# nikvaessen/w2v2-speaker

Measured on AMD Instinct MI355X. Metric: utterances/sec (w2v2-base + mean+std + AAM-softmax training step, 3 s clips), higher is better.
Workload: dtype f16; 1 GPU; wav2vec2-base + AAM-softmax(5994), mean+std pooling, 3 s synthetic audio, bs=66 per GPU, CNN frozen, fwd+bwd+all-reduce+Adam (BASELINE configs[1]); global_batch=66, samples_per_utt=48000, parallelism=dp1, regularisation=True

## Files before the change

### include/w2v2_hip.h

```cpp
#ifndef W2V2_HIP_H
#define W2V2_HIP_H

#include <stddef.h>
#include <stdint.h>

#ifdef __cplusplus
extern "C" {
#endif

#define W2V2_F32 0
#define W2V2_BF16 1
#define W2V2_F16 2

int w2v2_version(void);
const char* w2v2_last_error(void);

typedef struct {
  const void* ptr;
  int64_t ld;
  int64_t seg_len, seg_stride;
  int64_t stride0, stride1;
  int32_t trans;
  int32_t _pad;
} w2v2_operand;

enum {
  W2V2_EPI_NONE = 0,
  W2V2_EPI_BIAS = 1,
  W2V2_EPI_BIAS_GELU = 2,
  W2V2_EPI_GELU_BWD = 3,
  W2V2_EPI_ADD = 4,
  W2V2_EPI_SCALE_RC = 5,
  W2V2_EPI_BIAS_GELU_GRAD = 6,
  W2V2_EPI_MUL = 7
};

typedef struct {
  int32_t M, N, K;
  int32_t batch, batch_inner;
  int32_t dtype_ab;
  int32_t dtype_c;
  int32_t epilogue;
  w2v2_operand A, B;
  void* C;
  int64_t ldc, c_stride0, c_stride1;
  void* aux;
  int64_t ldaux, aux_stride0, aux_stride1;
  const float* bias;
  int64_t bias_stride1;
  const float* row_scale;
  const float* col_scale;
  float alpha;
  int32_t split_k;
  int32_t accumulate;
  int32_t _pad;
  int32_t k_ext, n_ext_from;
  int64_t b_lo_offset;
} w2v2_gemm_desc;

int w2v2_gemm(const w2v2_gemm_desc* d, void* stream);
int w2v2_gemm_timed(const w2v2_gemm_desc* d, void* stream, int slot);
int w2v2_timer_read(int first_slot, int n, float* ms_out);
int w2v2_gemm_kernel_of(const w2v2_gemm_desc* d);
int w2v2_tune_gemm_kernel(int family);
int w2v2_tune_gemm_debug(int bits);
int w2v2_tune_gemm_f32_tile(int tile);
int w2v2_tune_gemm_ring_debug(int bits);
int w2v2_gemm_f32_last_kernel(void);

typedef struct {
  const void* dY; int64_t ld_dy;
  const void* X;  int64_t ld_x;
  float* dW;      int64_t ld_dw;
  float* dbias;
  int32_t n_out, n_in;
} w2v2_wgrad_problem;
int w2v2_wgrad_grouped(const w2v2_wgrad_problem* problems, int n, int tokens, int tokens_padded,
                       int dtype , void* stream);
int w2v2_wgrad_kernel_of(const w2v2_wgrad_problem* problems, int n);
int w2v2_tune_wgrad_kernel(int family);

int w2v2_conv0_workspace_floats(int N, int C, int k, int stride);
int w2v2_conv0_stats(const float* wav, const float* w , float* partial, float* mean_rstd,
                     int B, int N, int C, int k, int stride, float eps, void* stream);
int w2v2_conv0_stats_mfma(const float* wav, const float* w, float* partial, float* mean_rstd,
                          int B, int N, int C, int k, int stride, float eps, void* stream);
int w2v2_conv0_stats_len(const float* wav, const float* w, float* partial, float* mean_rstd, const int* frames,
                         int B, int N, int C, int k, int stride, float eps, void* stream);
int w2v2_conv0_stats_mfma_len(const float* wav, const float* w, float* partial, float* mean_rstd, const int* frames,
                              int B, int N, int C, int k, int stride, float eps, void* stream);
int w2v2_conv0_apply(const float* wav, const float* w, const float* mean_rstd, const float* gamma,
                     const float* beta, void* y, int dtype, int B, int N, int C, int k, int stride,
                     void* stream);
int w2v2_conv0_layernorm_gelu(const float* wav, const float* w, const float* bias, const float* gamma, const float* beta,
                              void* out, int B, int N, int C, int k, int stride, float eps, int dtype, void* stream);
int w2v2_conv0_layernorm_gelu_bwd_workspace_floats(int B, int N, int C, int k, int stride);
int w2v2_conv0_layernorm_gelu_bwd(const float* wav, const float* w, const float* bias, const float* gamma, const float* beta,
                                  const void* dy, float* dw, float* dbias, float* dgamma, float* dbeta, float* workspace,
                                  int B, int N, int C, int k, int stride, float eps, int dtype, void* stream);
int w2v2_conv0_bwd(const float* wav, const float* w, const float* mean_rstd, const float* gamma,
                   const float* beta, const void* dz, float* sums, float* dw, float* dgamma, float* dbeta,
                   int dtype, int B, int N, int C, int k, int stride, void* stream);
int w2v2_col2im(const void* col, void* dx, int B, int Lin, int Lout, int Cin, int k, int stride, int dtype,
                void* stream);
int w2v2_unpack_conv_grad(const float* gp, float* g, int Cout, int Cin, int k, void* stream);
int w2v2_pack_conv_weight(const float* w, void* out, int dtype, int Cout, int Cin, int k, void* stream);

int w2v2_layernorm_fwd(const void* x, void* r_inout, const float* gamma, const float* beta, void* y,
                       float* mean, float* rstd, int M, int H, float eps, float drop_p,
                       uint64_t seed, int dtype, void* stream);
int w2v2_layernorm_gelu_fwd(const void* x, const float* gamma, const float* beta, void* y, int M, int H, float eps,
                            int dtype, void* stream);
int w2v2_layernorm_gelu_bwd_workspace_floats(int M, int H);
int w2v2_layernorm_gelu_bwd(const void* dy, const void* z, const float* gamma, const float* beta, void* dz, float* dgamma,
                            float* dbeta, float* dbias, float* workspace, int M, int H, float eps, int dtype, void* stream);
int w2v2_layernorm_bwd_workspace_floats(int H);
int w2v2_layernorm_bwd(const void* dy, const void* s, const float* mean, const float* rstd,
                       const float* gamma, void* ds, void* d_r, float* dgamma, float* dbeta,
                       float* workspace, int M, int H, float drop_p, uint64_t seed, int dtype,
                       void* stream);
typedef struct {
  const float* partial;
  float* dgamma;
  float* dbeta;
} w2v2_ln_fold;
int w2v2_layernorm_bwd_fold(const w2v2_ln_fold* entries, int n, int M, int H, void* stream);

int w2v2_dropout(const void* x, void* y, int64_t n, float p, uint64_t seed, int dtype, void* stream);
int w2v2_gelu_bwd(const void* dy, const void* pre, void* dx, int64_t n, int dtype, void* stream);
#define W2V2_PARTIAL_ROWS 256
int w2v2_gelu_bwd_colsum(const void* dy, const void* pre, void* dx, float* colsum, float* partial, int M, int N, int dtype,
                         void* stream);
int w2v2_add(const void* x, const void* a, void* y, int64_t n, int dtype, void* stream);
int w2v2_colsum(const void* x, int64_t ld, float* out, int M, int N, int dtype, void* stream);
int w2v2_zero_ranges(float* base, const int64_t* table, int n_ranges, int blocks_per_range, void* stream);
int w2v2_mean(const float* x, float* out, int n, void* stream);
int w2v2_cast(const float* x, void* y, int64_t n, int dtype, void* stream);
int w2v2_transpose_many(const void* src, void* dst, const int64_t* table, int n, int blocks_per_matrix,
                        int dtype, void* stream);
int w2v2_mask_fill(void* h, const uint8_t* mask, const float* embed, int M, int H, int dtype,
                   void* stream);
int w2v2_mask_feature(void* h, const uint8_t* mask, int B, int T, int H, int dtype, void* stream);
int w2v2_mask_fill_bwd(void* dh, const uint8_t* mask, float* d_embed, float* partial, int M, int H, int dtype,
                       void* stream);
int w2v2_prepend_token(const void* x, void* y, float c, int B, int T, int H, int dtype, void* stream);
int w2v2_pair_assemble(const void* feat, void* y, const int* left_row, const int* left_frames, const int* right_row,
                       const int* right_frames, float cls_c, float sep_c, int B, int T, int H, int dtype, void* stream);

int w2v2_posconv_regroup(const void* x, void* xg, int B, int T, int H, int G, int K, int pad_left,
                         int dtype, void* stream);
int w2v2_posconv_regroup_len(const void* x, void* xg, const int* lens, int B, int T, int H, int G, int K, int pad_left,
                             int dtype, void* stream);
int w2v2_posconv_wgrad(const void* dY, const void* xg, float* dwf, int B, int T, int H, int G, int K,
                       int dtype , void* stream);
int w2v2_posconv_direct(const void* xg, const void* w, void* out, void* aux, const float* bias, int B, int T, int G,
                        int Cg, int K, int64_t ldc, int mode, int dtype, void* stream);
int64_t w2v2_weightnorm_scratch_floats(int H, int G, int K);
int w2v2_weightnorm_pack(const float* g, const float* v, float* sumsq , void* wf,
                         void* wb, int H, int G, int K, int dtype, void* stream);
int w2v2_weightnorm_bwd(const float* g, const float* v, const float* sumsq, const float* dwf,
                        float* dot , float* dg, float* dv, int H, int G, int K,
                        void* stream);

int w2v2_softmax_fwd(const float* s, void* p, void* p_drop, int64_t rows, int T, int64_t ld,
                     float drop_p, uint64_t seed, int dtype, void* stream);
int w2v2_softmax_bwd(const float* dp_drop, const void* p, void* ds, int64_t rows, int T, int64_t ld,
                     float drop_p, uint64_t seed, int dtype, void* stream);
int w2v2_softmax_fwd_len(const float* s, void* p, const int* lens, int B, int heads, int T, int64_t ld, int dtype,
                         void* stream);
int w2v2_attention_fwd(const void* qkv, void* ctx, float* lse, int B, int T, int heads, int d,
                       float scale, float drop_p, uint64_t seed, int dtype, void* stream);
int w2v2_attention_bwd(const void* qkv, const void* ctx, const void* dctx, const float* lse,
                       void* dqkv, float* delta , int B, int T, int heads,
                       int d, float scale, float drop_p, uint64_t seed, int dtype, void* stream);
int w2v2_attention_fwd_len(const void* qkv, void* ctx, float* lse, const int* lens, int B, int T, int heads, int d,
                           float scale, int dtype, void* stream);

int w2v2_pool_fwd(const void* x, float* out, int B, int T, int H, int mode, int dtype, void* stream);
int w2v2_pool_fwd_len(const void* x, float* out, const int* lens, int B, int T, int H, int mode, int dtype,
                      void* stream);
int w2v2_pool_bwd(const void* x, const float* out, const float* dout, void* dx, int B, int T, int H,
                  int mode, int dtype, void* stream);

int w2v2_asp_context(const void* x, float* ctx, int B, int T, int C, int dtype, void* stream);
int w2v2_asp_context_len(const void* x, float* ctx, const int* lens, int B, int T, int C, int dtype, void* stream);
int w2v2_asp_context_bias(const float* ctx, const float* w1 , const float* b1, float* cb ,
                          int B, int A, int C, void* stream);
int w2v2_asp_bn_workspace_floats(int M, int A);
int w2v2_asp_bn_stats(const void* a_pre, float* workspace, float* mean_rstd, float* running, int M, int A,
                      float eps, float momentum, int dtype, void* stream);
int w2v2_asp_bn_eval_stats(const float* running, float* mean_rstd, int A, float eps, void* stream);
int w2v2_asp_bn_tanh(const void* a_pre, const float* mean_rstd, const float* gamma, const float* beta, void* h,
                     int M, int A, int dtype, void* stream);
int w2v2_asp_bn_bwd(const void* dh, const void* a_pre, const float* mean_rstd, const float* gamma,
                    const float* beta, float* workspace, float* dgamma, float* dbeta, void* da, int M, int A,
                    int dtype, void* stream);
int w2v2_asp_pool_fwd(const void* x, const void* s, float* out, float* stats, int B, int T, int C, int dtype,
                      void* stream);
int w2v2_asp_pool_fwd_len(const void* x, const void* s, float* out, float* stats, const int* lens, int B, int T, int C,
                          int dtype, void* stream);
int w2v2_asp_pool_bwd(const void* x, const void* s, const float* out, const float* stats, const float* dout,
                      void* ds, void* dx, int B, int T, int C, int dtype, void* stream);
int w2v2_asp_context_bwd(const void* x, const float* ctx, const void* da, const float* w1, float* dw1, void* dx,
                         float* scratch, int B, int T, int C, int A, int dtype, void* stream);

int w2v2_bce_head_fwd_bwd(const float* emb, const float* w, const float* b, const int64_t* label, float* prob,
                          float* loss_rows, float* dlogit, float* demb, float* dw, float* db, int B, int H,
                          const float* loss_scale, void* stream);

int w2v2_bn_workspace_floats(int M, int C);
int w2v2_bn_fwd(const void* a, int64_t lda, float* workspace, float* mean_rstd, float* running, const float* gamma,
                const float* beta, void* y, int64_t ldy, int M, int C, float eps, float momentum, int relu, int train,
                int dtype, void* stream);
int w2v2_bn_colsum_rows(int M, int C);
int w2v2_bn_bwd(const void* dy, int64_t lddy, const void* a, int64_t lda, const float* mean_rstd, const float* gamma,
                float* workspace, float* dgamma, float* dbeta, void* da, int64_t ldda, int M, int C, int relu,
                float* colsum_partial, int dtype, void* stream);
int w2v2_bn_bwd_sum(const void* dy, int64_t lddy, const void* dy2, int64_t lddy2, const void* a, int64_t lda,
                    const float* mean_rstd, const float* gamma, float* workspace, float* dgamma, float* dbeta, void* da,
                    int64_t ldda, int M, int C, int relu, float* colsum_partial, int dtype, void* stream);
int w2v2_im2col_reflect(const void* x, int64_t ldx, void* col, int B, int T, int Cin, int k, int dilation, int dtype,
                        void* stream);
int w2v2_im2col_reflect_sum(const void* x, int64_t ldx, const void* x2, int64_t ldx2, void* col, int B, int T, int Cin,
                            int k, int dilation, int dtype, void* stream);
int w2v2_im2col_reflect_len(const void* x, int64_t ldx, void* col, const int* lens, int B, int T, int Cin, int k,
                            int dilation, int dtype, void* stream);
int w2v2_im2col_reflect_sum_len(const void* x, int64_t ldx, const void* x2, int64_t ldx2, void* col, const int* lens,
                                int B, int T, int Cin, int k, int dilation, int dtype, void* stream);
int w2v2_col2im_reflect(const void* dcol, void* dx, int64_t lddx, int B, int T, int Cin, int k, int dilation,
                        int accumulate, int dtype, void* stream);
int w2v2_add_strided(const void* a, int64_t lda, const void* b, int64_t ldb, void* y, int64_t ldy, int M, int C,
                     int dtype, void* stream);
int w2v2_se_scale(const void* x, const float* g, void* y, int B, int T, int C, int dtype, void* stream);
int w2v2_se_bwd_gate(const void* dout, const void* x, float* dg, int B, int T, int C, int dtype, void* stream);
int w2v2_se_bwd_x(const void* dout, const float* g, const float* ds, void* dx, int B, int T, int C, int dtype,
                  void* stream);
int w2v2_act_fwd(const float* x, float* y, int64_t n, int mode, void* stream);
int w2v2_act_bwd(const float* dy, const float* y, float* dx, int64_t n, int mode, void* stream);

#define W2V2_FBANK_TILE_FRAMES 16
int w2v2_fbank_db(const float* wav, const int* lens, const float* window, const float* fbank, float* db_out,
                  float* partial_max, int B, int N, int T, int n_mels, void* stream);
int w2v2_fbank_normalize(const float* db, const float* partial_max, const int* lens, void* out, int64_t ldo, int dtype,
                         int B, int T, int n_mels, void* stream);

int w2v2_skinny_linear_fwd(const float* x, const float* W, const float* bias, float* y, int B, int N, int K, int act,
                           void* stream);
int w2v2_skinny_linear_bwd_x(const float* dy, const float* y, const float* W, float* dx, int B, int N, int K, int act,
                             void* stream);
int w2v2_skinny_linear_bwd_w(const float* dy, const float* y, const float* x, float* dW, float* dbias, int B, int N,
                             int K, int act, int accumulate, void* stream);

int w2v2_row_invnorm(const void* x, int64_t ld, float* inv, int rows, int cols, int dtype,
                     void* stream);
int w2v2_aam_softmax_fwd_bwd(const float* cos, const int64_t* label, float* softmax,
                             float* loss_rows, void* dcos_w, void* dcos_x, const float* inv_x,
                             const float* inv_w, float* rowdot, float* colprod, int B, int C,
                             int64_t ldc, float margin, float scale, const float* loss_scale,
                             float* correct_rows, int easy_margin , int dtype, void* stream);
int w2v2_normalize_bwd(const float* g, const void* x, int64_t ldx, const float* inv,
                       const float* dot, float* dx, int rows, int cols, int x_dtype, int add,
                       void* stream);
int w2v2_aam_dw(const void* dcos_x, int64_t ldc, const void* emb, const float* colprod, const float* W,
                const float* inv_w, float* dW, int B, int C, int E, int dtype, void* stream);

int w2v2_adam_step(float* p, const float* g, float* m, float* v, void* pb, int pb_dtype, int64_t n, float lr,
                   float beta1, float beta2, float eps, float bias_corr1, float bias_corr2,
                   float grad_scale, const float* scaler_state, int step, int skip_slot, void* stream);

#define W2V2_OPTIM_ADAM 0
#define W2V2_OPTIM_SGD 1
int w2v2_optim_step(int algo, float* p, const float* g, float* m, float* v, void* pb, int pb_dtype, int64_t n, float lr,
                    float beta1, float beta2, float eps, float bias_corr1, float bias_corr2, float grad_scale,
                    float weight_decay, float momentum, float dampening, int nesterov, const float* norm_state,
                    const float* scaler_state, int step, int skip_slot, void* stream);

int w2v2_grad_norm_partials(int64_t n);
int w2v2_grad_norm(const float* g, int64_t n, float grad_scale, float* scaler_state, float max_norm, double* partials,
                   int n_partials, float* norm_state, void* stream);

int w2v2_grad_accumulate(float* acc, const float* g, int64_t n, int first, void* stream);

int w2v2_weight_residual(const float* p, void* lo, const int64_t* table, int n_ranges, int dtype, void* stream);
int w2v2_grad_scaler_check(const float* g, int64_t n, float* state, void* stream);
int w2v2_grad_scaler_update(float* state, float growth, float backoff, int growth_interval, int skipped_ranges,
                            void* stream);

typedef struct w2v2_comm w2v2_comm;
int w2v2_comm_unique_id(void* id_host_128);
int w2v2_comm_init(w2v2_comm** comm, const void* id_host_128, int rank, int world, int device);
int w2v2_comm_init_loopback(w2v2_comm** comm, int world, int device);
int w2v2_allreduce_async(w2v2_comm* comm, float* buf, int64_t n, void* stream);
int w2v2_broadcast_async(w2v2_comm* comm, void* buf, int64_t nbytes, int root, void* stream);
int w2v2_comm_destroy(w2v2_comm* comm);
int w2v2_traffic_probe(float* buf, int64_t n, int channels, int lds_bytes, float gbps, void* stream);

#ifdef __cplusplus
}
#endif
#endif
```

### w2v2_speaker_amd/_lib.py

```python
from __future__ import annotations

import ctypes as C
import os

from . import _build

F32, BF16, F16 = 0, 1, 2
EPI_NONE, EPI_BIAS, EPI_BIAS_GELU, EPI_GELU_BWD, EPI_ADD, EPI_SCALE_RC, EPI_BIAS_GELU_GRAD, EPI_MUL = range(8)
OPTIM_ADAM, OPTIM_SGD = 0, 1

c_i32, c_i64, c_u64, c_f32, c_vp = C.c_int32, C.c_int64, C.c_uint64, C.c_float, C.c_void_p


class Operand(C.Structure):
    _fields_ = [("ptr", c_vp), ("ld", c_i64), ("seg_len", c_i64), ("seg_stride", c_i64),
                ("stride0", c_i64), ("stride1", c_i64), ("trans", c_i32), ("_pad", c_i32)]


class GemmDesc(C.Structure):
    _fields_ = [("M", c_i32), ("N", c_i32), ("K", c_i32), ("batch", c_i32), ("batch_inner", c_i32),
                ("dtype_ab", c_i32), ("dtype_c", c_i32), ("epilogue", c_i32),
                ("A", Operand), ("B", Operand),
                ("C", c_vp), ("ldc", c_i64), ("c_stride0", c_i64), ("c_stride1", c_i64),
                ("aux", c_vp), ("ldaux", c_i64), ("aux_stride0", c_i64), ("aux_stride1", c_i64),
                ("bias", c_vp), ("bias_stride1", c_i64), ("row_scale", c_vp), ("col_scale", c_vp),
                ("alpha", c_f32), ("split_k", c_i32), ("accumulate", c_i32), ("_pad", c_i32),
                ("k_ext", c_i32), ("n_ext_from", c_i32), ("b_lo_offset", c_i64)]


class LnFold(C.Structure):
    _fields_ = [("partial", c_vp), ("dgamma", c_vp), ("dbeta", c_vp)]


class WgradProblem(C.Structure):
    _fields_ = [("dY", c_vp), ("ld_dy", c_i64), ("X", c_vp), ("ld_x", c_i64), ("dW", c_vp), ("ld_dw", c_i64),
                ("dbias", c_vp), ("n_out", c_i32), ("n_in", c_i32)]


_SIGS = {
    "w2v2_version": (c_i32, []),
    "w2v2_last_error": (C.c_char_p, []),
    "w2v2_gemm": (c_i32, [C.POINTER(GemmDesc), c_vp]),
    "w2v2_gemm_kernel_of": (c_i32, [c_vp]),
    "w2v2_gemm_timed": (c_i32, [C.POINTER(GemmDesc), c_vp, c_i32]),
    "w2v2_timer_read": (c_i32, [c_i32, c_i32, c_vp]),
    "w2v2_tune_gemm_kernel": (c_i32, [c_i32]),
    "w2v2_tune_gemm_debug": (c_i32, [c_i32]),
    "w2v2_tune_gemm_f32_tile": (c_i32, [c_i32]),
    "w2v2_tune_gemm_ring_debug": (c_i32, [c_i32]),
    "w2v2_gemm_f32_last_kernel": (c_i32, []),
    "w2v2_zero_ranges": (c_i32, [c_vp, c_vp, c_i32, c_i32, c_vp]),
    "w2v2_mean": (c_i32, [c_vp, c_vp, c_i32, c_vp]),
    "w2v2_wgrad_grouped": (c_i32, [C.POINTER(WgradProblem), c_i32, c_i32, c_i32, c_i32, c_vp]),
    "w2v2_wgrad_kernel_of": (c_i32, [C.POINTER(WgradProblem), c_i32]),
    "w2v2_tune_wgrad_kernel": (c_i32, [c_i32]),
    "w2v2_conv0_workspace_floats": (c_i32, [c_i32, c_i32, c_i32, c_i32]),
    "w2v2_conv0_stats": (c_i32, [c_vp, c_vp, c_vp, c_vp, c_i32, c_i32, c_i32, c_i32, c_i32, c_f32, c_vp]),
    "w2v2_conv0_stats_mfma": (c_i32, [c_vp, c_vp, c_vp, c_vp, c_i32, c_i32, c_i32, c_i32, c_i32, c_f32, c_vp]),
    "w2v2_conv0_stats_len": (c_i32, [c_vp, c_vp, c_vp, c_vp, c_vp, c_i32, c_i32, c_i32, c_i32, c_i32, c_f32, c_vp]),
    "w2v2_conv0_stats_mfma_len": (c_i32, [c_vp, c_vp, c_vp, c_vp, c_vp, c_i32, c_i32, c_i32, c_i32, c_i32, c_f32,
                                          c_vp]),
    "w2v2_conv0_apply": (c_i32, [c_vp, c_vp, c_vp, c_vp, c_vp, c_vp, c_i32, c_i32, c_i32, c_i32, c_i32,
                                 c_i32, c_vp]),
    "w2v2_pack_conv_weight": (c_i32, [c_vp, c_vp, c_i32, c_i32, c_i32, c_i32, c_vp]),
    "w2v2_conv0_bwd": (c_i32, [c_vp] * 10 + [c_i32] * 6 + [c_vp]),
    "w2v2_col2im": (c_i32, [c_vp, c_vp, c_i32, c_i32, c_i32, c_i32, c_i32, c_i32, c_i32, c_vp]),
    "w2v2_unpack_conv_grad": (c_i32, [c_vp, c_vp, c_i32, c_i32, c_i32, c_vp]),
    "w2v2_conv0_layernorm_gelu": (c_i32, [c_vp, c_vp, c_vp, c_vp, c_vp, c_vp, c_i32, c_i32, c_i32, c_i32, c_i32, c_f32, c_i32, c_vp]),
    "w2v2_layernorm_gelu_fwd": (c_i32, [c_vp, c_vp, c_vp, c_vp, c_i32, c_i32, c_f32, c_i32, c_vp]),
    "w2v2_layernorm_gelu_bwd_workspace_floats": (c_i32, [c_i32, c_i32]),
    "w2v2_layernorm_gelu_bwd": (c_i32, [c_vp] * 9 + [c_i32, c_i32, c_f32, c_i32, c_vp]),
    "w2v2_conv0_layernorm_gelu_bwd_workspace_floats": (c_i32, [c_i32] * 5),
    "w2v2_conv0_layernorm_gelu_bwd": (c_i32, [c_vp] * 11 + [c_i32] * 5 + [c_f32, c_i32, c_vp]),
    "w2v2_layernorm_fwd": (c_i32, [c_vp, c_vp, c_vp, c_vp, c_vp, c_vp, c_vp, c_i32, c_i32, c_f32, c_f32,
                                   c_u64, c_i32, c_vp]),
    "w2v2_layernorm_bwd_workspace_floats": (c_i32, [c_i32]),
    "w2v2_layernorm_bwd": (c_i32, [c_vp, c_vp, c_vp, c_vp, c_vp, c_vp, c_vp, c_vp, c_vp, c_vp, c_i32, c_i32,
                                   c_f32, c_u64, c_i32, c_vp]),
    "w2v2_layernorm_bwd_fold": (c_i32, [C.POINTER(LnFold), c_i32, c_i32, c_i32, c_vp]),
    "w2v2_dropout": (c_i32, [c_vp, c_vp, c_i64, c_f32, c_u64, c_i32, c_vp]),
    "w2v2_gelu_bwd_colsum": (c_i32, [c_vp, c_vp, c_vp, c_vp, c_vp, c_i32, c_i32, c_i32, c_vp]),
    "w2v2_gelu_bwd": (c_i32, [c_vp, c_vp, c_vp, c_i64, c_i32, c_vp]),
    "w2v2_add": (c_i32, [c_vp, c_vp, c_vp, c_i64, c_i32, c_vp]),
    "w2v2_colsum": (c_i32, [c_vp, c_i64, c_vp, c_i32, c_i32, c_i32, c_vp]),
    "w2v2_cast": (c_i32, [c_vp, c_vp, c_i64, c_i32, c_vp]),
    "w2v2_transpose_many": (c_i32, [c_vp, c_vp, c_vp, c_i32, c_i32, c_i32, c_vp]),
    "w2v2_mask_feature": (c_i32, [c_vp, c_vp, c_i32, c_i32, c_i32, c_i32, c_vp]),
    "w2v2_mask_fill": (c_i32, [c_vp, c_vp, c_vp, c_i32, c_i32, c_i32, c_vp]),
    "w2v2_mask_fill_bwd": (c_i32, [c_vp, c_vp, c_vp, c_vp, c_i32, c_i32, c_i32, c_vp]),
    "w2v2_prepend_token": (c_i32, [c_vp, c_vp, c_f32, c_i32, c_i32, c_i32, c_i32, c_vp]),
    "w2v2_pair_assemble": (c_i32, [c_vp, c_vp, c_vp, c_vp, c_vp, c_vp, c_f32, c_f32, c_i32, c_i32, c_i32, c_i32, c_vp]),
    "w2v2_posconv_regroup": (c_i32, [c_vp, c_vp, c_i32, c_i32, c_i32, c_i32, c_i32, c_i32, c_i32, c_vp]),
    "w2v2_posconv_regroup_len": (c_i32, [c_vp, c_vp, c_vp, c_i32, c_i32, c_i32, c_i32, c_i32, c_i32, c_i32, c_vp]),
    "w2v2_posconv_direct": (c_i32, [c_vp, c_vp, c_vp, c_vp, c_vp, c_i32, c_i32, c_i32, c_i32, c_i32, c_i64, c_i32, c_i32, c_vp]),
    "w2v2_posconv_wgrad": (c_i32, [c_vp, c_vp, c_vp, c_i32, c_i32, c_i32, c_i32, c_i32, c_i32, c_vp]),
    "w2v2_weightnorm_scratch_floats": (c_i64, [c_i32, c_i32, c_i32]),
    "w2v2_weightnorm_pack": (c_i32, [c_vp, c_vp, c_vp, c_vp, c_vp, c_i32, c_i32, c_i32, c_i32, c_vp]),
    "w2v2_weightnorm_bwd": (c_i32, [c_vp, c_vp, c_vp, c_vp, c_vp, c_vp, c_vp, c_i32, c_i32, c_i32, c_vp]),
    "w2v2_softmax_fwd": (c_i32, [c_vp, c_vp, c_vp, c_i64, c_i32, c_i64, c_f32, c_u64, c_i32, c_vp]),
    "w2v2_softmax_bwd": (c_i32, [c_vp, c_vp, c_vp, c_i64, c_i32, c_i64, c_f32, c_u64, c_i32, c_vp]),
    "w2v2_softmax_fwd_len": (c_i32, [c_vp, c_vp, c_vp, c_i32, c_i32, c_i32, c_i64, c_i32, c_vp]),
    "w2v2_attention_fwd": (c_i32, [c_vp, c_vp, c_vp, c_i32, c_i32, c_i32, c_i32, c_f32, c_f32, c_u64,
                                   c_i32, c_vp]),
    "w2v2_attention_fwd_len": (c_i32, [c_vp, c_vp, c_vp, c_vp, c_i32, c_i32, c_i32, c_i32, c_f32, c_i32, c_vp]),
    "w2v2_attention_bwd": (c_i32, [c_vp, c_vp, c_vp, c_vp, c_vp, c_vp, c_i32, c_i32, c_i32, c_i32, c_f32,
                                   c_f32, c_u64, c_i32, c_vp]),
    "w2v2_pool_fwd": (c_i32, [c_vp, c_vp, c_i32, c_i32, c_i32, c_i32, c_i32, c_vp]),
    "w2v2_pool_fwd_len": (c_i32, [c_vp, c_vp, c_vp, c_i32, c_i32, c_i32, c_i32, c_i32, c_vp]),
    "w2v2_pool_bwd": (c_i32, [c_vp, c_vp, c_vp, c_vp, c_i32, c_i32, c_i32, c_i32, c_i32, c_vp]),
    "w2v2_bce_head_fwd_bwd": (c_i32, [c_vp] * 10 + [c_i32, c_i32, c_vp, c_vp]),
    "w2v2_bn_workspace_floats": (c_i32, [c_i32, c_i32]),
    "w2v2_bn_fwd": (c_i32, [c_vp, c_i64, c_vp, c_vp, c_vp, c_vp, c_vp, c_vp, c_i64, c_i32, c_i32, c_f32, c_f32, c_i32,
                            c_i32, c_i32, c_vp]),
    "w2v2_skinny_linear_fwd": (c_i32, [c_vp, c_vp, c_vp, c_vp, c_i32, c_i32, c_i32, c_i32, c_vp]),
    "w2v2_skinny_linear_bwd_x": (c_i32, [c_vp, c_vp, c_vp, c_vp, c_i32, c_i32, c_i32, c_i32, c_vp]),
    "w2v2_skinny_linear_bwd_w": (c_i32, [c_vp, c_vp, c_vp, c_vp, c_vp, c_i32, c_i32, c_i32, c_i32, c_i32, c_vp]),
    "w2v2_bn_bwd": (c_i32, [c_vp, c_i64, c_vp, c_i64, c_vp, c_vp, c_vp, c_vp, c_vp, c_vp, c_i64, c_i32, c_i32, c_i32,
                            c_vp, c_i32, c_vp]),
    "w2v2_bn_bwd_sum": (c_i32, [c_vp, c_i64, c_vp, c_i64, c_vp, c_i64, c_vp, c_vp, c_vp, c_vp, c_vp, c_vp, c_i64, c_i32,
                                c_i32, c_i32, c_vp, c_i32, c_vp]),
    "w2v2_bn_colsum_rows": (c_i32, [c_i32, c_i32]),
    "w2v2_im2col_reflect": (c_i32, [c_vp, c_i64, c_vp, c_i32, c_i32, c_i32, c_i32, c_i32, c_i32, c_vp]),
    "w2v2_im2col_reflect_sum": (c_i32, [c_vp, c_i64, c_vp, c_i64, c_vp, c_i32, c_i32, c_i32, c_i32, c_i32, c_i32, c_vp]),
    "w2v2_im2col_reflect_len": (c_i32, [c_vp, c_i64, c_vp, c_vp, c_i32, c_i32, c_i32, c_i32, c_i32, c_i32, c_vp]),
    "w2v2_im2col_reflect_sum_len": (c_i32, [c_vp, c_i64, c_vp, c_i64, c_vp, c_vp, c_i32, c_i32, c_i32, c_i32, c_i32, c_i32,
                                            c_vp]),
    "w2v2_col2im_reflect": (c_i32, [c_vp, c_vp, c_i64, c_i32, c_i32, c_i32, c_i32, c_i32, c_i32, c_i32, c_vp]),
    "w2v2_add_strided": (c_i32, [c_vp, c_i64, c_vp, c_i64, c_vp, c_i64, c_i32, c_i32, c_i32, c_vp]),
    "w2v2_se_scale": (c_i32, [c_vp, c_vp, c_vp, c_i32, c_i32, c_i32, c_i32, c_vp]),
    "w2v2_se_bwd_gate": (c_i32, [c_vp, c_vp, c_vp, c_i32, c_i32, c_i32, c_i32, c_vp]),
    "w2v2_se_bwd_x": (c_i32, [c_vp, c_vp, c_vp, c_vp, c_i32, c_i32, c_i32, c_i32, c_vp]),
    "w2v2_act_fwd": (c_i32, [c_vp, c_vp, c_i64, c_i32, c_vp]),
    "w2v2_act_bwd": (c_i32, [c_vp, c_vp, c_vp, c_i64, c_i32, c_vp]),
    "w2v2_fbank_db": (c_i32, [c_vp, c_vp, c_vp, c_vp, c_vp, c_vp, c_i32, c_i32, c_i32, c_i32, c_vp]),
    "w2v2_fbank_normalize": (c_i32, [c_vp, c_vp, c_vp, c_vp, c_i64, c_i32, c_i32, c_i32, c_i32, c_vp]),
    "w2v2_asp_context": (c_i32, [c_vp, c_vp, c_i32, c_i32, c_i32, c_i32, c_vp]),
    "w2v2_asp_context_len": (c_i32, [c_vp, c_vp, c_vp, c_i32, c_i32, c_i32, c_i32, c_vp]),
    "w2v2_asp_context_bias": (c_i32, [c_vp, c_vp, c_vp, c_vp, c_i32, c_i32, c_i32, c_vp]),
    "w2v2_asp_bn_workspace_floats": (c_i32, [c_i32, c_i32]),
    "w2v2_asp_bn_stats": (c_i32, [c_vp, c_vp, c_vp, c_vp, c_i32, c_i32, c_f32, c_f32, c_i32, c_vp]),
    "w2v2_asp_bn_eval_stats": (c_i32, [c_vp, c_vp, c_i32, c_f32, c_vp]),
    "w2v2_asp_bn_tanh": (c_i32, [c_vp, c_vp, c_vp, c_vp, c_vp, c_i32, c_i32, c_i32, c_vp]),
    "w2v2_asp_bn_bwd": (c_i32, [c_vp] * 9 + [c_i32, c_i32, c_i32, c_vp]),
    "w2v2_asp_pool_fwd": (c_i32, [c_vp, c_vp, c_vp, c_vp, c_i32, c_i32, c_i32, c_i32, c_vp]),
    "w2v2_asp_pool_fwd_len": (c_i32, [c_vp, c_vp, c_vp, c_vp, c_vp, c_i32, c_i32, c_i32, c_i32, c_vp]),
    "w2v2_asp_pool_bwd": (c_i32, [c_vp] * 7 + [c_i32, c_i32, c_i32, c_i32, c_vp]),
    "w2v2_asp_context_bwd": (c_i32, [c_vp] * 7 + [c_i32, c_i32, c_i32, c_i32, c_i32, c_vp]),
    "w2v2_row_invnorm": (c_i32, [c_vp, c_i64, c_vp, c_i32, c_i32, c_i32, c_vp]),
    "w2v2_aam_softmax_fwd_bwd": (c_i32, [c_vp, c_vp, c_vp, c_vp, c_vp, c_vp, c_vp, c_vp, c_vp, c_vp, c_i32,
                                         c_i32, c_i64, c_f32, c_f32, c_vp, c_vp, c_i32, c_i32, c_vp]),
    "w2v2_aam_dw": (c_i32, [c_vp, c_i64, c_vp, c_vp, c_vp, c_vp, c_vp, c_i32, c_i32, c_i32, c_i32, c_vp]),
    "w2v2_normalize_bwd": (c_i32, [c_vp, c_vp, c_i64, c_vp, c_vp, c_vp, c_i32, c_i32, c_i32, c_i32, c_vp]),
    "w2v2_adam_step": (c_i32, [c_vp, c_vp, c_vp, c_vp, c_vp, c_i32, c_i64, c_f32, c_f32, c_f32, c_f32, c_f32,
                               c_f32, c_f32, c_vp, c_i32, c_i32, c_vp]),
    "w2v2_optim_step": (c_i32, [c_i32, c_vp, c_vp, c_vp, c_vp, c_vp, c_i32, c_i64, c_f32, c_f32, c_f32, c_f32, c_f32,
                                c_f32, c_f32, c_f32, c_f32, c_f32, c_i32, c_vp, c_vp, c_i32, c_i32, c_vp]),
    "w2v2_grad_norm_partials": (c_i32, [c_i64]),
    "w2v2_grad_norm": (c_i32, [c_vp, c_i64, c_f32, c_vp, c_f32, c_vp, c_i32, c_vp, c_vp]),
    "w2v2_grad_accumulate": (c_i32, [c_vp, c_vp, c_i64, c_i32, c_vp]),
    "w2v2_weight_residual": (c_i32, [c_vp, c_vp, c_vp, c_i32, c_i32, c_vp]),
    "w2v2_comm_unique_id": (c_i32, [c_vp]),
    "w2v2_comm_init": (c_i32, [C.POINTER(c_vp), c_vp, c_i32, c_i32, c_i32]),
    "w2v2_comm_init_loopback": (c_i32, [C.POINTER(c_vp), c_i32, c_i32]),
    "w2v2_allreduce_async": (c_i32, [c_vp, c_vp, c_i64, c_vp]),
    "w2v2_broadcast_async": (c_i32, [c_vp, c_vp, c_i64, c_i32, c_vp]),
    "w2v2_comm_destroy": (c_i32, [c_vp]),
    "w2v2_traffic_probe": (c_i32, [c_vp, c_i64, c_i32, c_i32, c_f32, c_vp]),
    "w2v2_grad_scaler_check": (c_i32, [c_vp, c_i64, c_vp, c_vp]),
    "w2v2_grad_scaler_update": (c_i32, [c_vp, c_f32, c_f32, c_i32, c_i32, c_vp]),
}

EXPORTS = tuple(_SIGS)
_lib = None


def library_path() -> str:
    return _build.LIB


def load():
    global _lib
    if _lib is not None:
        return _lib
    path = _build.LIB
    alt = os.environ.get("W2V2_LIB_AB")
    if alt and os.path.exists(alt):
        path = alt
    elif _build.needs_build():
        try:
            _build.build_locked()
        except Exception as e:
            raise RuntimeError(f"libw2v2hip.so is missing or older than its sources and could not be built: {e}") from e
    lib = C.CDLL(path)
    for name, (res, args) in _SIGS.items():
        if path == alt and not hasattr(lib, name):
            continue
        fn = getattr(lib, name)
        fn.restype, fn.argtypes = res, args
    _lib = lib
    return lib


def check(rc: int, what: str = "") -> None:
    if rc != 0:
        msg = load().w2v2_last_error()
        raise RuntimeError(f"libw2v2hip {what} failed: {msg.decode() if msg else rc}")
```

### w2v2_speaker_amd/csrc/gemm.hip

```cpp
#include "gemm_common.h"

template <int R, bool TRANS>
struct Stager {
  static constexpr int NV = TRANS ? 4 : (R / 32);
  uint4 v[NV];

  __device__ __forceinline__ void load(const OpDev& o, const bf16_t* __restrict__ base, int r0,
                                       int rbound, int k0, int kend, int tid,
                                       const int64_t* __restrict__ rowoff) {
    if constexpr (!TRANS) {
#pragma unroll
      for (int j = 0; j < NV; ++j) {
        const int c = tid + 256 * j;
        const int row = c >> 3, kc = c & 7;
        const int k = k0 + kc * 8;
        uint4 val = make_uint4(0, 0, 0, 0);
        if (r0 + row < rbound && k < kend) {
          const bf16_t* p = base + rowoff[j] + k;
          if (o.vec_ok && k + 8 <= kend) {
            val = *reinterpret_cast<const uint4*>(p);
          } else {
            bf16_t t[8];
#pragma unroll
            for (int e = 0; e < 8; ++e) t[e] = (k + e < kend) ? p[e] : (bf16_t)0;
            val.x = t[0] | ((uint32_t)t[1] << 16); val.y = t[2] | ((uint32_t)t[3] << 16);
            val.z = t[4] | ((uint32_t)t[5] << 16); val.w = t[6] | ((uint32_t)t[7] << 16);
          }
        }
        v[j] = val;
      }
    } else {
      const int nblk = R * 2;
      const int mb = tid % (R / 8), kb = tid / (R / 8);
#pragma unroll
      for (int i = 0; i < 4; ++i) {
        uint4 val = make_uint4(0, 0, 0, 0);
        const int k = k0 + kb * 4 + i;
        const int in0 = r0 + mb * 8;
        if (tid < nblk && k < kend && in0 < rbound) {
          const bf16_t* p = base + outer_off(o, k) + in0;
          if (o.vec_ok && in0 + 8 <= rbound) {
            val = *reinterpret_cast<const uint4*>(p);
          } else {
            bf16_t t[8];
#pragma unroll
            for (int e = 0; e < 8; ++e) t[e] = (in0 + e < rbound) ? p[e] : (bf16_t)0;
            val.x = t[0] | ((uint32_t)t[1] << 16); val.y = t[2] | ((uint32_t)t[3] << 16);
            val.z = t[4] | ((uint32_t)t[5] << 16); val.w = t[6] | ((uint32_t)t[7] << 16);
          }
        }
        v[i] = val;
      }
    }
  }

  __device__ __forceinline__ void store(bf16_t* __restrict__ lds, int tid) const {
    if constexpr (!TRANS) {
#pragma unroll
      for (int j = 0; j < NV; ++j) {
        const int c = tid + 256 * j;
        const int row = c >> 3, kc = c & 7;
        *reinterpret_cast<uint4*>(lds + row * 64 + ((kc ^ swz_rs(row)) << 3)) = v[j];
      }
    } else {
      const int nblk = R * 2;
      if (tid >= nblk) return;
      const int mb = tid % (R / 8), kb = tid / (R / 8);
      const uint32_t w[4][4] = {{v[0].x, v[0].y, v[0].z, v[0].w},
                                {v[1].x, v[1].y, v[1].z, v[1].w},
                                {v[2].x, v[2].y, v[2].z, v[2].w},
                                {v[3].x, v[3].y, v[3].z, v[3].w}};
#pragma unroll
      for (int mi = 0; mi < 8; ++mi) {
        const int d = mi >> 1;
        uint2 o2;
        if (mi & 1) {
          o2.x = (w[0][d] >> 16) | (w[1][d] & 0xffff0000u);
          o2.y = (w[2][d] >> 16) | (w[3][d] & 0xffff0000u);
        } else {
          o2.x = (w[0][d] & 0xffffu) | (w[1][d] << 16);
          o2.y = (w[2][d] & 0xffffu) | (w[3][d] << 16);
        }
        const int row = mb * 8 + mi;
        const int chunk = kb >> 1, half = kb & 1;
        *reinterpret_cast<uint2*>(lds + row * 64 + ((chunk ^ swz_rs(row)) << 3) + half * 4) = o2;
      }
    }
  }
};

template <typename TE, int FM, int FN, bool TA, bool TB, typename TC>
__global__ __launch_bounds__(256) void gemm16_regstage_kernel(const GemmArgs g) {
  constexpr int BM = 32 * FM, BN = 32 * FN;
  extern __shared__ __attribute__((aligned(16))) char smem_raw[];
  bf16_t* As = reinterpret_cast<bf16_t*>(smem_raw);
  bf16_t* Bs = As + 2 * BM * 64;

  const int tid = threadIdx.x;
  const int lane = tid & 63, wave = tid >> 6;
  const int wm = wave >> 1, wn = wave & 1;

  const int ntile = g.tiles_m * g.tiles_n;
  const int tile = xcd_remap(blockIdx.x, ntile);
  const int tm = tile / g.tiles_n, tn = tile - tm * g.tiles_n;
  const int m0 = tm * BM, n0 = tn * BN;
  const int z = blockIdx.z;
  const int z0 = z / g.batch_inner, z1 = z - z0 * g.batch_inner;
  const int split = blockIdx.y;
  const int kbeg = split * g.k_per_split;
  const int kend = min(g.K, kbeg + g.k_per_split);

  const bf16_t* Ab = reinterpret_cast<const bf16_t*>(g.A.ptr) + z0 * g.a_s0 + z1 * g.a_s1;
  const bf16_t* Bb = reinterpret_cast<const bf16_t*>(g.B.ptr) + z0 * g.b_s0 + z1 * g.b_s1;

  int64_t arow[TA ? 1 : (BM / 32)], brow[TB ? 1 : (BN / 32)];
  if constexpr (!TA) {
#pragma unroll
    for (int j = 0; j < BM / 32; ++j) {
      const int row = (tid + 256 * j) >> 3;
      arow[j] = (m0 + row < g.M) ? outer_off(g.A, m0 + row) : 0;
    }
  }
  if constexpr (!TB) {
#pragma unroll
    for (int j = 0; j < BN / 32; ++j) {
      const int row = (tid + 256 * j) >> 3;
      brow[j] = (n0 + row < g.N) ? outer_off(g.B, n0 + row) : 0;
    }
  }

  f32x4 acc[FM][FN];
#pragma unroll
  for (int i = 0; i < FM; ++i)
#pragma unroll
    for (int j = 0; j < FN; ++j) acc[i][j] = f32x4{0.f, 0.f, 0.f, 0.f};

  Stager<BM, TA> sa;
  Stager<BN, TB> sb;
  const int nk = (kend - kbeg + 63) / 64;
  if (nk > 0) {
    sa.load(g.A, Ab, m0, g.M, kbeg, kend, tid, arow);
    sb.load(g.B, Bb, n0, g.N, kbeg, kend, tid, brow);
    sa.store(As, tid);
    sb.store(Bs, tid);
  }
  __syncthreads();

  const int frow = lane & 15, fk = lane >> 4;
  for (int kt = 0; kt < nk; ++kt) {
    const int cur = kt & 1;
    if (kt + 1 < nk) {
      const int k0 = kbeg + (kt + 1) * 64;
      sa.load(g.A, Ab, m0, g.M, k0, kend, tid, arow);
      sb.load(g.B, Bb, n0, g.N, k0, kend, tid, brow);
    }
    const bf16_t* Ac = As + cur * BM * 64;
    const bf16_t* Bc = Bs + cur * BN * 64;
#pragma unroll
    for (int kk = 0; kk < 2; ++kk) {
      frag8_t af[FM], bfr[FN];
#pragma unroll
      for (int i = 0; i < FM; ++i) {
        const int row = wm * (16 * FM) + i * 16 + frow;
        af[i] = *reinterpret_cast<const frag8_t*>(Ac + row * 64 + (((kk * 4 + fk) ^ swz_rs(row)) << 3));
      }
#pragma unroll
      for (int j = 0; j < FN; ++j) {
        const int row = wn * (16 * FN) + j * 16 + frow;
        bfr[j] = *reinterpret_cast<const frag8_t*>(Bc + row * 64 + (((kk * 4 + fk) ^ swz_rs(row)) << 3));
      }
#pragma unroll
      for (int i = 0; i < FM; ++i)
#pragma unroll
        for (int j = 0; j < FN; ++j)
          acc[i][j] = mfma16<TE>(bfr[j], af[i], acc[i][j]);
    }
    if (kt + 1 < nk) {
      sa.store(As + (cur ^ 1) * BM * 64, tid);
      sb.store(Bs + (cur ^ 1) * BN * 64, tid);
    }
    __syncthreads();
  }

  tile_epilogue<TC, FM, FN>(g, acc, reinterpret_cast<float*>(smem_raw), m0, n0, wm, wn, z0, z1, split);
}


template <typename TE, int FM, int FN, typename TC>
__global__ __launch_bounds__(256) void gemm16_dma_128_kernel(const GemmArgs g) {
  constexpr int BM = 32 * FM, BN = 32 * FN;
  constexpr int NA = BM / 32, NB = BN / 32;
  extern __shared__ __attribute__((aligned(16))) char smem_raw[];
  bf16_t* As = reinterpret_cast<bf16_t*>(smem_raw);
  bf16_t* Bs = As + 2 * BM * 64;

  const int tid = threadIdx.x;
  const int lane = tid & 63;
  const int wave = __builtin_amdgcn_readfirstlane(tid >> 6);
  const int wm = wave >> 1, wn = wave & 1;

  const int ntile = g.tiles_m * g.tiles_n;
  const int tile = xcd_remap(blockIdx.x, ntile);
  const int tm = tile / g.tiles_n, tn = tile - tm * g.tiles_n;
  const int m0 = tm * BM, n0 = tn * BN;
  const int z = blockIdx.z;
  const int z0 = z / g.batch_inner, z1 = z - z0 * g.batch_inner;
  const int split = blockIdx.y;
  const int kbeg = split * g.k_per_split;
  const int kend = min(g.K, kbeg + g.k_per_split);
  const int nk = (kend - kbeg) >> 6;

  const bf16_t* Ab = reinterpret_cast<const bf16_t*>(g.A.ptr) + z0 * g.a_s0 + z1 * g.a_s1;
  const bf16_t* Bb = reinterpret_cast<const bf16_t*>(g.B.ptr) + z0 * g.b_s0 + z1 * g.b_s1;

  const int c8 = lane & 7, r8 = lane >> 3;
  const bf16_t* ap[NA];
  const bf16_t* bp[NB];
#pragma unroll
  for (int j = 0; j < NA; ++j) {
    const int row = (wave * NA + j) * 8 + r8;
    const int grow = min(m0 + row, g.M - 1);
    ap[j] = Ab + outer_off(g.A, grow) + kbeg + ((c8 ^ swz(row)) << 3);
  }
#pragma unroll
  for (int j = 0; j < NB; ++j) {
    const int row = (wave * NB + j) * 8 + r8;
    const int grow = min(n0 + row, g.N - 1);
    bp[j] = Bb + outer_off(g.B, grow) + kbeg + ((c8 ^ swz(row)) << 3);
  }

  f32x4 acc[FM][FN];
#pragma unroll
  for (int i = 0; i < FM; ++i)
#pragma unroll
    for (int j = 0; j < FN; ++j) acc[i][j] = f32x4{0.f, 0.f, 0.f, 0.f};

  auto stage = [&](int buf, int kt) {
    bf16_t* ad = As + buf * BM * 64 + wave * NA * 8 * 64;
    bf16_t* bd = Bs + buf * BN * 64 + wave * NB * 8 * 64;
#pragma unroll
    for (int j = 0; j < NA; ++j) w2v2_dma16(ap[j] + kt * 64, ad + j * 8 * 64);
#pragma unroll
    for (int j = 0; j < NB; ++j) w2v2_dma16(bp[j] + kt * 64, bd + j * 8 * 64);
  };
  auto landed = [&]() {
    asm volatile("s_waitcnt vmcnt(0)" ::: "memory");
    __syncthreads();
  };
  const int frow = lane & 15, fk = lane >> 4;
  auto compute = [&](int buf) {
    const bf16_t* Ac = As + buf * BM * 64;
    const bf16_t* Bc = Bs + buf * BN * 64;
#pragma unroll
    for (int kk = 0; kk < 2; ++kk) {
      frag8_t af[FM], bfr[FN];
#pragma unroll
      for (int i = 0; i < FM; ++i) {
        const int row = wm * (16 * FM) + i * 16 + frow;
        af[i] = *reinterpret_cast<const frag8_t*>(Ac + row * 64 + (((kk * 4 + fk) ^ swz(row)) << 3));
      }
#pragma unroll
      for (int j = 0; j < FN; ++j) {
        const int row = wn * (16 * FN) + j * 16 + frow;
        bfr[j] = *reinterpret_cast<const frag8_t*>(Bc + row * 64 + (((kk * 4 + fk) ^ swz(row)) << 3));
      }
#pragma unroll
      for (int i = 0; i < FM; ++i)
#pragma unroll
        for (int j = 0; j < FN; ++j)
          acc[i][j] = mfma16<TE>(bfr[j], af[i], acc[i][j]);
    }
  };

  if (nk > 0) stage(0, 0);
  w2v2_vmcnt0_visible();
  __syncthreads();
  for (int kt = 0; kt < nk; kt += 2) {
    if (kt + 1 < nk) stage(1, kt + 1);
    compute(0);
    landed();
    if (kt + 1 < nk) {
      if (kt + 2 < nk) stage(0, kt + 2);
      compute(1);
      landed();
    }
  }

  tile_epilogue<TC, FM, FN>(g, acc, reinterpret_cast<float*>(smem_raw), m0, n0, wm, wn, z0, z1, split);
}

const W2v2Switches& w2v2_switches() {
  static const W2v2Switches sw = [] {
    W2v2Switches s;
    auto env_int = [](const char* name, int dflt) { const char* e = getenv(name); return e ? atoi(e) : dflt; };
    auto env_on = [](const char* name, bool dflt) { const char* e = getenv(name); return e ? e[0] != '0' : dflt; };
    s.no_glds = getenv("W2V2_NO_GLDS") != nullptr;
    s.glds3 = getenv("W2V2_NO_GLDS3") == nullptr;
    s.tile256 = getenv("W2V2_NO_GEMM_PH") == nullptr;
    s.persistent = getenv("W2V2_G3_NONPERSISTENT") == nullptr;
    s.g3n = env_int("W2V2_G3N", 512);
    s.defer = getenv("W2V2_NO_DEFER") == nullptr;
    s.wt_stores = env_on("W2V2_EPI_WT", true);
    s.late_dma = env_on("W2V2_PH_LATE", false);
    s.reserve_cus = env_int("W2V2_RESERVE_CUS", 0);
    s.f32_no_dma = env_on("W2V2_F32_NO_DMA", false);
    s.wgrad_ring = getenv("W2V2_WGRAD_V1") == nullptr;
    s.wgrad_ring4 = getenv("W2V2_NO_WGRAD4") == nullptr;
    s.wgrad_phased = getenv("W2V2_NO_WGRAD_PH") == nullptr;
    return s;
  }();
  return sw;
}

int w2v2_device_cus() {
  static const int ncu = [] {
    int dev = 0, v = 0;
    (void)hipGetDevice(&dev);
    return (hipDeviceGetAttribute(&v, hipDeviceAttributeMultiprocessorCount, dev) == hipSuccess && v > 0) ? v : 256;
  }();
  return ncu;
}
int w2v2_gemm_device_cus() {
  const int ncu = w2v2_device_cus(), r = w2v2_switches().reserve_cus;
  return (r > 0 && r < ncu) ? ncu - r : ncu;
}

static int g_w2v2_force = 0;
extern "C" int w2v2_tune_gemm_kernel(int family) {
  const int old = g_w2v2_force;
  if (family == 0 || family == 1 || family == 2 || family == 4) g_w2v2_force = family;
  return old;
}

struct GemmRoute {
  int family;
  bool narrow;
  dim3 grid;
  int f32_rows;
};

static bool aligned16(const void* p) { return (reinterpret_cast<uintptr_t>(p) & 15) == 0; }

static int gemm_route(const w2v2_gemm_desc* d, int force, GemmArgs& a, GemmRoute& r) {
  W2V2_REQUIRE(d != nullptr, "w2v2_gemm: null descriptor");
  W2V2_REQUIRE(d->M > 0 && d->N > 0 && d->K >= 0 && d->batch > 0, "w2v2_gemm: bad shape M=%d N=%d K=%d batch=%d",
               d->M, d->N, d->K, d->batch);
  W2V2_REQUIRE(d->A.ptr && d->B.ptr && d->C, "w2v2_gemm: null operand");
  W2V2_REQUIRE(d->dtype_ab == W2V2_F32 || d->dtype_ab == W2V2_BF16 || d->dtype_ab == W2V2_F16,
               "w2v2_gemm: bad dtype_ab %d", d->dtype_ab);
  W2V2_REQUIRE(d->dtype_c == W2V2_F32 || d->dtype_c == d->dtype_ab, "w2v2_gemm: dtype_c %d must be f32 or dtype_ab (%d)",
               d->dtype_c, d->dtype_ab);
  W2V2_REQUIRE(d->epilogue >= 0 && d->epilogue <= W2V2_EPI_MUL, "w2v2_gemm: bad epilogue %d", d->epilogue);
  const int split = d->split_k > 1 ? d->split_k : 1;
  const int atomic = (split > 1 || d->accumulate) ? 1 : 0;
  if (atomic) {
    W2V2_REQUIRE(d->dtype_c == W2V2_F32, "w2v2_gemm: split_k/accumulate need an f32 C");
    W2V2_REQUIRE(d->epilogue == W2V2_EPI_NONE || (split == 1) || d->epilogue == W2V2_EPI_BIAS,
                 "w2v2_gemm: split_k supports EPI_NONE/EPI_BIAS only");
  }
  if (d->epilogue == W2V2_EPI_BIAS || d->epilogue == W2V2_EPI_BIAS_GELU || d->epilogue == W2V2_EPI_BIAS_GELU_GRAD)
    W2V2_REQUIRE(d->bias != nullptr, "w2v2_gemm: bias epilogue without bias");
  if (d->epilogue == W2V2_EPI_GELU_BWD || d->epilogue == W2V2_EPI_ADD || d->epilogue == W2V2_EPI_MUL ||
      d->epilogue == W2V2_EPI_BIAS_GELU_GRAD)
    W2V2_REQUIRE(d->aux != nullptr, "w2v2_gemm: epilogue %d needs aux", d->epilogue);
  if (d->epilogue == W2V2_EPI_SCALE_RC)
    W2V2_REQUIRE(d->row_scale && d->col_scale, "w2v2_gemm: EPI_SCALE_RC needs row/col scales");

  const bool f32 = d->dtype_ab == W2V2_F32;
  const int oal = f32 ? 4 : 8;
  a.M = d->M; a.N = d->N; a.K = d->K;
  a.epilogue = d->epilogue; a.split_k = split; a.atomic = atomic;
  a.tiles_m = a.tiles_n = 0;
  a.batch_inner = d->batch_inner > 0 ? d->batch_inner : 1;
  auto cvt = [&](const w2v2_operand& o) {
    OpDev v;
    v.ptr = o.ptr; v.ld = o.ld; v.seg_len = o.seg_len; v.seg_stride = o.seg_stride; v.trans = o.trans ? 1 : 0;
    v.vec_ok = aligned16(o.ptr) && (o.ld % oal == 0) && (o.seg_stride % oal == 0) && (o.stride0 % oal == 0) &&
               (o.stride1 % oal == 0);
    return v;
  };
  a.A = cvt(d->A);
  a.B = cvt(d->B);
  a.a_s0 = d->A.stride0; a.a_s1 = d->A.stride1; a.b_s0 = d->B.stride0; a.b_s1 = d->B.stride1;
  a.C = d->C; a.ldc = d->ldc; a.c_s0 = d->c_stride0; a.c_s1 = d->c_stride1;
  a.aux = d->aux; a.ldaux = d->ldaux; a.aux_s0 = d->aux_stride0; a.aux_s1 = d->aux_stride1;
  a.bias = d->bias; a.bias_s1 = d->bias_stride1;
  a.row_scale = d->row_scale; a.col_scale = d->col_scale;
  a.alpha = d->alpha;
  a.k_ext = d->k_ext; a.n_ext_from = d->n_ext_from; a.b_lo_off = d->b_lo_offset;
  a.defer_ok = 0;
  a.wt_stores = 1;
  a.late_dma = 0;
  a.xcd_tiles = 0;
  a.dbg_bits = 0;
  const int cal = d->dtype_c == W2V2_F32 ? 4 : 8;
  a.c_vec_ok = aligned16(d->C) && (d->ldc % cal == 0) && (d->c_stride0 % cal == 0) && (d->c_stride1 % cal == 0);
  a.aux_vec_ok = d->aux && aligned16(d->aux) && (d->ldaux % cal == 0) && (d->aux_stride0 % cal == 0) &&
                 (d->aux_stride1 % cal == 0);
  r.family = 0; r.narrow = false; r.grid = dim3(1); r.f32_rows = 0;

  const int bk = f32 ? 32 : 64;
  a.k_per_split = (int)(cdiv(cdiv(d->K, split), bk) * bk);
  if (a.k_per_split == 0) a.k_per_split = bk;
  if (f32) {
    r.f32_rows = w2v2_gemm_f32_dma_rows(a, d->M, d->N, d->K, split, d->batch);
    r.family = r.f32_rows > 0 ? 10 : 9;
    return 0;
  }

  const W2v2Switches& sw = w2v2_switches();
  const int64_t ncu = w2v2_gemm_device_cus();
  const bool glds = !a.A.trans && !a.B.trans && a.A.vec_ok && a.B.vec_ok && (d->K % 64 == 0) && d->K >= 64 && !sw.no_glds;
  r.narrow = d->N <= 64 || (glds && cdiv(d->M, 128) * cdiv(d->N, 128) * split * d->batch * 2 <= ncu);
  a.tiles_m = (int)cdiv(d->M, 128); a.tiles_n = (int)cdiv(d->N, r.narrow ? 64 : 128);
  r.grid = dim3(a.tiles_m * a.tiles_n, split, d->batch);

  const bool ring_ok = glds && split == 1 && !atomic;
  auto extent = [](const w2v2_operand& o, int64_t rows, int64_t K) -> int64_t {
    return (o.seg_len > 0 ? (rows / o.seg_len + 1) * o.seg_stride + o.seg_len * o.ld : rows * o.ld) + K;
  };
  const bool fits32 = extent(d->A, d->M, d->K) < (int64_t(1) << 31) && extent(d->B, d->N, d->K) < (int64_t(1) << 31);
  const bool phased_ok = ring_ok && d->k_ext == 0 && d->batch == 1 && fits32 && (d->dtype_c == W2V2_F32 || lines_ok(a));
  bool ring, phased;
  if (force != 0 && ring_ok && d->k_ext == 0 && d->batch == 1) {
    ring = force >= 2;
    phased = force == 4 && phased_ok;
  } else {
    ring = ring_ok && (d->k_ext != 0 || (d->N >= sw.g3n && d->M >= 1024 && sw.glds3));
    phased = false;
    if (ring && phased_ok && d->N >= 512 && sw.tile256) {
      const int64_t t4 = cdiv(d->M, 256) * cdiv(d->N, 256), t3 = cdiv(d->M, 256) * cdiv(d->N, 128);
      const double fill4 = (double)t4 / (double)(cdiv(t4, ncu) * ncu), fill3 = (double)t3 / (double)(cdiv(t3, ncu) * ncu);
      phased = fill4 * 1.25 >= fill3 && t4 * 2 >= ncu && (double)d->N / (double)(cdiv(d->N, 256) * 256) >= 0.9;
    }
  }
  if (d->k_ext != 0)
    W2V2_REQUIRE(ring && d->k_ext == d->K && d->n_ext_from >= 0 && d->n_ext_from % 128 == 0 && d->b_lo_offset % 8 == 0,
                 "w2v2_gemm: two-term weights (k_ext) need k_ext == K, n_ext_from %% 128 == 0 and K-contiguous 16-byte "
                 "aligned operands with K %% 64 == 0 (M=%d N=%d K=%d)", d->M, d->N, d->K);
  r.family = phased ? 4 : ring ? 2 : glds ? 1 : 3;
  a.wt_stores = sw.wt_stores;
  a.late_dma = sw.late_dma;
  if (r.family == 2)
    a.defer_ok = sw.defer && d->dtype_c != W2V2_F32 && lines_ok(a) && (d->N % 128 == 0) &&
                 d->epilogue != W2V2_EPI_BIAS_GELU && d->epilogue != W2V2_EPI_BIAS_GELU_GRAD;
  return 0;
}

extern "C" int w2v2_gemm_kernel_of(const w2v2_gemm_desc* d) {
  GemmArgs a;
  GemmRoute r;
  return gemm_route(d, g_w2v2_force, a, r) != 0 ? -1 : r.family;
}

template <typename TE, int FM, int FN, typename TC>
static int launch_glds(const GemmArgs& a, dim3 grid, hipStream_t st) {
  constexpr size_t lds = (size_t)2 * (32 * FM + 32 * FN) * 64 * sizeof(bf16_t);
  return w2v2_launch_lds<&gemm16_dma_128_kernel<TE, FM, FN, TC>>("gemm16_dma_128_kernel", grid, dim3(256), lds, st, a);
}

template <typename TE, int FM, int FN, typename TC>
static int launch_regstage(const GemmArgs& a, dim3 grid, hipStream_t st) {
  constexpr size_t lds = (size_t)2 * (32 * FM + 32 * FN) * 64 * sizeof(bf16_t);
#define W2V2_LAUNCH(TA_, TB_) \
  return w2v2_launch_lds<&gemm16_regstage_kernel<TE, FM, FN, TA_, TB_, TC>>("gemm16_regstage_kernel", grid, dim3(256), lds, st, a)
  if (!a.A.trans && !a.B.trans) W2V2_LAUNCH(false, false);
  else if (!a.A.trans && a.B.trans) W2V2_LAUNCH(false, true);
  else if (a.A.trans && !a.B.trans) W2V2_LAUNCH(true, false);
  else W2V2_LAUNCH(true, true);
#undef W2V2_LAUNCH
}

template <typename TE, typename TC>
static int launch_128(const GemmArgs& a, const GemmRoute& r, hipStream_t st) {
  if (r.family == 1) return r.narrow ? launch_glds<TE, 4, 2, TC>(a, r.grid, st) : launch_glds<TE, 4, 4, TC>(a, r.grid, st);
  return r.narrow ? launch_regstage<TE, 4, 2, TC>(a, r.grid, st) : launch_regstage<TE, 4, 4, TC>(a, r.grid, st);
}

extern "C" int w2v2_gemm(const w2v2_gemm_desc* d, void* stream) {
  GemmArgs a;
  GemmRoute r;
  if (gemm_route(d, g_w2v2_force, a, r) != 0) return -1;
  hipStream_t st = as_stream(stream);
  const bool c32 = d->dtype_c == W2V2_F32;
  int rc;
  switch (r.family) {
    case 4: rc = w2v2_launch_phased_256x256(a, d->dtype_ab, d->dtype_c, d->M, d->N, d->batch, st); break;
    case 2: rc = w2v2_launch_ring_256x128(a, d->dtype_ab, d->dtype_c, d->M, d->N, d->batch, w2v2_switches().persistent, st); break;
    case 9: case 10: rc = w2v2_launch_gemm_f32(a, d->M, d->N, d->K, a.split_k, d->batch, r.f32_rows, st); break;
    default:
      if (d->dtype_ab == W2V2_BF16) rc = c32 ? launch_128<bf16_t, float>(a, r, st) : launch_128<bf16_t, bf16_t>(a, r, st);
      else rc = c32 ? launch_128<f16_t, float>(a, r, st) : launch_128<f16_t, f16_t>(a, r, st);
      break;
  }
  if (rc != 0) return rc;
  W2V2_CHECK_LAUNCH("w2v2_gemm");
  return 0;
}

#include <vector>
W2v2PendingTimer& w2v2_pending_timer() {
  static thread_local W2v2PendingTimer t = {nullptr, nullptr, false};
  return t;
}
static std::vector<std::pair<hipEvent_t, hipEvent_t>> g_timer_slots;
extern "C" int w2v2_gemm_timed(const w2v2_gemm_desc* d, void* stream, int slot) {
  W2V2_REQUIRE(slot >= 0 && slot < (1 << 16), "w2v2_gemm_timed: slot %d out of range", slot);
  while ((int)g_timer_slots.size() <= slot) {
    hipEvent_t a, b;
    if (hipEventCreate(&a) != hipSuccess || hipEventCreate(&b) != hipSuccess) W2V2_FAIL("w2v2_gemm_timed: hipEventCreate failed");
    g_timer_slots.push_back({a, b});
  }
  W2v2PendingTimer& pt = w2v2_pending_timer();
  pt.start = g_timer_slots[slot].first;
  pt.stop = g_timer_slots[slot].second;
  pt.armed = true;
  const int rc = w2v2_gemm(d, stream);
  const bool unused = pt.armed;
  pt.armed = false;
  if (rc != 0) return rc;
  if (unused)
    W2V2_FAIL("w2v2_gemm_timed: this product does not run on the 256x128 ring or the phased 256x256 kernel");
  return 0;
}
extern "C" int w2v2_timer_read(int first_slot, int n, float* ms_out) {
  W2V2_REQUIRE(first_slot >= 0 && n >= 0 && first_slot + n <= (int)g_timer_slots.size() && ms_out, "w2v2_timer_read: bad range");
  for (int i = 0; i < n; ++i) {
    auto& e = g_timer_slots[first_slot + i];
    if (hipEventSynchronize(e.second) != hipSuccess || hipEventElapsedTime(ms_out + i, e.first, e.second) != hipSuccess)
      W2V2_FAIL("w2v2_timer_read: slot %d was never launched", first_slot + i);
  }
  return 0;
}
```

### w2v2_speaker_amd/csrc/gemm_common.h

```cpp
#pragma once
#include "common.h"
#include <hip/hip_ext.h>
#include <type_traits>
#include <stdlib.h>

typedef __attribute__((ext_vector_type(4))) float f32x4;

struct OpDev {
  const void* ptr;
  int64_t ld, seg_len, seg_stride;
  int trans;
  int vec_ok;
};

struct GemmArgs {
  int M, N, K;
  int epilogue, split_k, atomic;
  int tiles_m, tiles_n;
  int k_per_split;
  OpDev A, B;
  int64_t a_s0, a_s1, b_s0, b_s1;
  int batch_inner;
  void* C;
  int64_t ldc, c_s0, c_s1;
  void* aux;
  int64_t ldaux, aux_s0, aux_s1;
  const float* bias;
  int64_t bias_s1;
  const float* row_scale;
  const float* col_scale;
  float alpha;
  int c_vec_ok;
  int aux_vec_ok;
  int defer_ok;
  int wt_stores;
  int late_dma;
  int k_ext, n_ext_from;
  int64_t b_lo_off;
  int xcd_tiles;
  int dbg_bits;
};

__device__ __forceinline__ int64_t outer_off(const OpDev& o, int64_t idx) {
  if (o.seg_len > 0) {
    const int64_t q = idx / o.seg_len;
    return q * o.seg_stride + (idx - q * o.seg_len) * o.ld;
  }
  return idx * o.ld;
}

__device__ __forceinline__ int swz(int row) { return ((row ^ (row >> 1)) & 3) | (row & 4); }
__device__ __forceinline__ int swz_b(int row) { return swz((((row >> 4) & 3) << 2) | (row & 3)); }
__device__ __forceinline__ int swz_rs(int row) { return (row & 7) ^ ((row >> 3) & 1); }

template <typename TC>
__device__ __forceinline__ void epilogue_store4(const GemmArgs& g, TC* __restrict__ C,
                                                const TC* __restrict__ aux_in, TC* __restrict__ aux_out,
                                                const float* __restrict__ bias, int m, int n0,
                                                const float acc[4], bool lead) {
  if (m >= g.M) return;
  const float rs = (g.epilogue == W2V2_EPI_SCALE_RC) ? g.row_scale[m] : 1.0f;
  float out[4];
  float pre[4];
#pragma unroll
  for (int j = 0; j < 4; ++j) {
    const int n = n0 + j;
    float v = acc[j] * g.alpha;
    pre[j] = 0.f;
    if (n < g.N) {
      switch (g.epilogue) {
        case W2V2_EPI_BIAS:
          if (lead) v += bias[n];
          break;
        case W2V2_EPI_BIAS_GELU:
          v += bias[n];
          pre[j] = v;
          v = gelu_f(v);
          break;
        case W2V2_EPI_BIAS_GELU_GRAD:
          v += bias[n];
          gelu_both_f(v, v, pre[j]);
          break;
        case W2V2_EPI_GELU_BWD:
          v *= gelu_grad_f(to_f32<TC>(aux_in[(int64_t)m * g.ldaux + n]));
          break;
        case W2V2_EPI_MUL:
          v *= to_f32<TC>(aux_in[(int64_t)m * g.ldaux + n]);
          break;
        case W2V2_EPI_ADD:
          v += to_f32<TC>(aux_in[(int64_t)m * g.ldaux + n]);
          break;
        case W2V2_EPI_SCALE_RC:
          v *= rs * g.col_scale[n];
          break;
        default:
          break;
      }
    }
    out[j] = v;
  }
  TC* crow = C + (int64_t)m * g.ldc;
  if (g.atomic) {
    if constexpr (sizeof(TC) == 4) {
#pragma unroll
      for (int j = 0; j < 4; ++j)
        if (n0 + j < g.N) unsafeAtomicAdd(reinterpret_cast<float*>(crow) + n0 + j, out[j]);
    }
    return;
  }
  if (g.c_vec_ok && n0 + 4 <= g.N) {
    if constexpr (sizeof(TC) == 4) {
      *reinterpret_cast<float4*>(crow + n0) = make_float4(out[0], out[1], out[2], out[3]);
    } else {
      uint2 w;
      w.x = pack2<TC>(out[0], out[1]);
      w.y = pack2<TC>(out[2], out[3]);
      *reinterpret_cast<uint2*>(crow + n0) = w;
    }
  } else {
#pragma unroll
    for (int j = 0; j < 4; ++j)
      if (n0 + j < g.N) crow[n0 + j] = from_f32<TC>(out[j]);
  }
  if ((g.epilogue == W2V2_EPI_BIAS_GELU || g.epilogue == W2V2_EPI_BIAS_GELU_GRAD) && aux_out != nullptr) {
    TC* arow = aux_out + (int64_t)m * g.ldaux;
#pragma unroll
    for (int j = 0; j < 4; ++j)
      if (n0 + j < g.N) arow[n0 + j] = from_f32<TC>(pre[j]);
  }
}

template <typename TC, int EPI, bool DEFER = false>
__device__ __forceinline__ void epilogue_row8_impl(const GemmArgs& g, TC* __restrict__ Cz, TC* __restrict__ auxz,
                                                   int m, int n, float (&v)[8], const float (&cv)[8],
                                                   const float (&ax)[8], bool lead, uint4* dout = nullptr) {
  const bool full = n + 8 <= g.N;
  float pre[8];
  float rs = 1.0f;
  if constexpr (EPI == W2V2_EPI_SCALE_RC) rs = g.row_scale[m];
#pragma unroll
  for (int e = 0; e < 8; ++e) {
    float x = v[e] * g.alpha;
    if constexpr (EPI == W2V2_EPI_BIAS) { if (lead) x += cv[e]; }
    if constexpr (EPI == W2V2_EPI_BIAS_GELU) { x += cv[e]; pre[e] = x; x = gelu_f(x); }
    if constexpr (EPI == W2V2_EPI_BIAS_GELU_GRAD) { x += cv[e]; gelu_both_f(x, x, pre[e]); }
    if constexpr (EPI == W2V2_EPI_GELU_BWD) x *= gelu_grad_f(ax[e]);
    if constexpr (EPI == W2V2_EPI_MUL) x *= ax[e];
    if constexpr (EPI == W2V2_EPI_ADD) x += ax[e];
    if constexpr (EPI == W2V2_EPI_SCALE_RC) x *= rs * cv[e];
    v[e] = x;
  }
  TC* cp = Cz + (int64_t)m * g.ldc + n;
  if constexpr (DEFER) {
    if constexpr (sizeof(TC) == 2)
      *dout = make_uint4(pack2<TC>(v[0], v[1]), pack2<TC>(v[2], v[3]), pack2<TC>(v[4], v[5]), pack2<TC>(v[6], v[7]));
    return;
  }
  if (g.atomic) {
    if constexpr (sizeof(TC) == 4) {
#pragma unroll
      for (int e = 0; e < 8; ++e) if (n + e < g.N) unsafeAtomicAdd(reinterpret_cast<float*>(cp) + e, v[e]);
    }
  } else if (full && g.c_vec_ok) {
    Vec8<TC> t;
#pragma unroll
    for (int e = 0; e < 8; ++e) t.v[e] = v[e];
    t.store(cp);
  } else {
#pragma unroll
    for (int e = 0; e < 8; ++e) if (n + e < g.N) cp[e] = from_f32<TC>(v[e]);
  }
  if constexpr (EPI == W2V2_EPI_BIAS_GELU || EPI == W2V2_EPI_BIAS_GELU_GRAD) {
    if (auxz != nullptr) {
      TC* ap = auxz + (int64_t)m * g.ldaux + n;
      if (full && g.aux_vec_ok) {
        Vec8<TC> t;
#pragma unroll
        for (int e = 0; e < 8; ++e) t.v[e] = pre[e];
        t.store(ap);
      } else {
#pragma unroll
        for (int e = 0; e < 8; ++e) if (n + e < g.N) ap[e] = from_f32<TC>(pre[e]);
      }
    }
  }
}

template <typename TC, int EPI, int NIT, int NTHREADS, int BN>
__device__ __forceinline__ void epilogue_pass(const GemmArgs& g, const float* __restrict__ stage,
                                              TC* __restrict__ Cz, TC* __restrict__ auxz, int mbase, int n0,
                                              const float (&cv)[8], bool lead) {
  constexpr int PITCH = BN + 4, CPR = BN / 8;
  const int tid = threadIdx.x;
  const int ch = tid % CPR;
  const int n = n0 + ch * 8;
  if (n >= g.N) return;
  float ax[NIT][8];
  if constexpr (EPI == W2V2_EPI_GELU_BWD || EPI == W2V2_EPI_ADD || EPI == W2V2_EPI_MUL) {
#pragma unroll
    for (int it = 0; it < NIT; ++it) {
      const int r = (tid + NTHREADS * it) / CPR;
      const int m = mbase + r;
#pragma unroll
      for (int e = 0; e < 8; ++e) ax[it][e] = 0.f;
      if (m < g.M) {
        const TC* ap = auxz + (int64_t)m * g.ldaux + n;
        if (n + 8 <= g.N && g.aux_vec_ok) {
          Vec8<TC> t;
          t.load(ap);
#pragma unroll
          for (int e = 0; e < 8; ++e) ax[it][e] = t.v[e];
        } else {
#pragma unroll
          for (int e = 0; e < 8; ++e) if (n + e < g.N) ax[it][e] = to_f32<TC>(ap[e]);
        }
      }
    }
  }
#pragma unroll
  for (int it = 0; it < NIT; ++it) {
    const int r = (tid + NTHREADS * it) / CPR;
    const int m = mbase + r;
    if (m >= g.M) continue;
    const float4 lo = *reinterpret_cast<const float4*>(stage + r * PITCH + ch * 8);
    const float4 hi = *reinterpret_cast<const float4*>(stage + r * PITCH + ch * 8 + 4);
    float v[8] = {lo.x, lo.y, lo.z, lo.w, hi.x, hi.y, hi.z, hi.w};
    if constexpr (EPI == W2V2_EPI_GELU_BWD || EPI == W2V2_EPI_ADD || EPI == W2V2_EPI_MUL)
      epilogue_row8_impl<TC, EPI>(g, Cz, auxz, m, n, v, cv, ax[it], lead);
    else
      epilogue_row8_impl<TC, EPI>(g, Cz, auxz, m, n, v, cv, cv, lead);
  }
}

__device__ __forceinline__ void load_col8(const GemmArgs& g, const float* __restrict__ bias, int n, float (&cv)[8]) {
  const float* src = (g.epilogue == W2V2_EPI_SCALE_RC) ? g.col_scale : bias;
#pragma unroll
  for (int e = 0; e < 8; ++e) cv[e] = 0.f;
  if (src == nullptr || n >= g.N) return;
  if (n + 8 <= g.N && ((reinterpret_cast<uintptr_t>(src + n) & 15) == 0)) {
    const float4 a = *reinterpret_cast<const float4*>(src + n), b = *reinterpret_cast<const float4*>(src + n + 4);
    cv[0] = a.x; cv[1] = a.y; cv[2] = a.z; cv[3] = a.w; cv[4] = b.x; cv[5] = b.y; cv[6] = b.z; cv[7] = b.w;
  } else {
#pragma unroll
    for (int e = 0; e < 8; ++e) if (n + e < g.N) cv[e] = src[n + e];
  }
}

template <typename TC, int EPI, int FM, int I0, bool DEFER = false, int NR = 4>
__device__ __forceinline__ void epilogue_direct4(const GemmArgs& g, TC* __restrict__ Cz, TC* __restrict__ auxz,
                                                 f32x4 (&acc)[FM][4], int m, int n, const float (&cv0)[8],
                                                 const float (&cv1)[8], uint4 (&pend)[8]) {
  float ax[NR][16];
  if constexpr (EPI == W2V2_EPI_GELU_BWD || EPI == W2V2_EPI_ADD || EPI == W2V2_EPI_MUL) {
#pragma unroll
    for (int i = 0; i < NR; ++i) {
      const int mi = m + 16 * (I0 + i);
#pragma unroll
      for (int e = 0; e < 16; ++e) ax[i][e] = 0.f;
      if (mi < g.M) {
        const TC* ap = auxz + (int64_t)mi * g.ldaux + n;
#pragma unroll
        for (int h = 0; h < 2; ++h) {
          if (n + 8 * h + 8 <= g.N && g.aux_vec_ok) {
            Vec8<TC> t;
            t.load(ap + 8 * h);
#pragma unroll
            for (int e = 0; e < 8; ++e) ax[i][8 * h + e] = t.v[e];
          } else {
#pragma unroll
            for (int e = 0; e < 8; ++e) if (n + 8 * h + e < g.N) ax[i][8 * h + e] = to_f32<TC>(ap[8 * h + e]);
          }
        }
      }
    }
  }
#pragma unroll
  for (int i = 0; i < NR; ++i) {
    const int mi = m + 16 * (I0 + i);
    if (mi >= g.M) continue;
#pragma unroll
    for (int h = 0; h < 2; ++h) {
      if (n + 8 * h >= g.N) continue;
      float v[8];
#pragma unroll
      for (int e = 0; e < 8; ++e) v[e] = acc[I0 + i][2 * h + (e >> 2)][e & 3];
      float a8[8];
#pragma unroll
      for (int e = 0; e < 8; ++e) a8[e] = (EPI == W2V2_EPI_GELU_BWD || EPI == W2V2_EPI_ADD || EPI == W2V2_EPI_MUL) ? ax[i][8 * h + e] : 0.f;
      if constexpr (DEFER && FM == 4)
        epilogue_row8_impl<TC, EPI, true>(g, Cz, auxz, mi, n + 8 * h, v, h ? cv1 : cv0, a8, true, &pend[i * 2 + h]);
      else
        epilogue_row8_impl<TC, EPI>(g, Cz, auxz, mi, n + 8 * h, v, h ? cv1 : cv0, a8, true);
    }
  }
}
template <typename TC, int EPI, int FM, int NR = 4>
__device__ __forceinline__ void epilogue_direct(const GemmArgs& g, TC* __restrict__ Cz, TC* __restrict__ auxz,
                                                f32x4 (&acc)[FM][4], int m, int n, const float (&cv0)[8],
                                                const float (&cv1)[8]) {
  if (n >= g.N) return;
  uint4 unused[8];
  if constexpr (NR == 4) {
    epilogue_direct4<TC, EPI, FM, 0>(g, Cz, auxz, acc, m, n, cv0, cv1, unused);
    if constexpr (FM > 4) epilogue_direct4<TC, EPI, FM, 4>(g, Cz, auxz, acc, m, n, cv0, cv1, unused);
  } else {
    static_assert(NR == 2 && FM == 8, "two-row batches are wired for the 128-row wave tiles");
    epilogue_direct4<TC, EPI, FM, 0, false, 2>(g, Cz, auxz, acc, m, n, cv0, cv1, unused);
    epilogue_direct4<TC, EPI, FM, 2, false, 2>(g, Cz, auxz, acc, m, n, cv0, cv1, unused);
    epilogue_direct4<TC, EPI, FM, 4, false, 2>(g, Cz, auxz, acc, m, n, cv0, cv1, unused);
    epilogue_direct4<TC, EPI, FM, 6, false, 2>(g, Cz, auxz, acc, m, n, cv0, cv1, unused);
  }
}

__host__ __device__ __forceinline__ bool lines_ok(const GemmArgs& g) {
  return g.c_vec_ok && !g.atomic && (g.N & 63) == 0 && (g.aux == nullptr || g.aux_vec_ok);
}

template <typename TC, int EPI, int FM, bool DEFER = false>
__device__ __forceinline__ void epilogue_lines(const GemmArgs& g, TC* __restrict__ Cz, TC* __restrict__ auxz,
                                               f32x4 (&acc)[FM][4], int mw, int nc, int lane, const float (&cv0)[8],
                                               const float (&cv1)[8], uint4* __restrict__ pend) {
  static_assert(sizeof(TC) == 2, "16-bit outputs only");
  constexpr bool READS_AUX = EPI == W2V2_EPI_GELU_BWD || EPI == W2V2_EPI_ADD || EPI == W2V2_EPI_MUL;
  constexpr bool WRITES_AUX = EPI == W2V2_EPI_BIAS_GELU || EPI == W2V2_EPI_BIAS_GELU_GRAD;
  if constexpr (!DEFER) {
    if (nc >= g.N) return;
  }
  const bool wt = g.wt_stores != 0;
  auto st16 = [wt](TC* p, uint4 v) {
    if (wt) store16_wt(p, v); else *reinterpret_cast<uint4*>(p) = v;
  };
  const int c = lane & 15;
  const bool lo = c < 8;
  const int ra = mw + (c & 7);
  const int ncs = nc + (lo ? 0 : 8);
  const int mo = mw + c;
#pragma unroll
  for (int i0 = 0; i0 < FM; i0 += 4) {
    uint4 la[4], lb[4];
    if constexpr (READS_AUX) {
#pragma unroll
      for (int i = 0; i < 4; ++i) {
        const int r = ra + 16 * (i0 + i);
        la[i] = lb[i] = make_uint4(0, 0, 0, 0);
        if (r < g.M) la[i] = *reinterpret_cast<const uint4*>(auxz + (int64_t)r * g.ldaux + ncs);
        if (r + 8 < g.M) lb[i] = *reinterpret_cast<const uint4*>(auxz + (int64_t)(r + 8) * g.ldaux + ncs);
      }
    }
#pragma unroll
    for (int i = 0; i < 4; ++i) {
      float ax[16];
      if constexpr (READS_AUX) {
        uint4 a0, a1;
        lines_to_halves(lo, la[i], lb[i], a0, a1);
        unpack8<TC>(a0, ax);
        unpack8<TC>(a1, ax + 8);
      }
      float rs = 1.0f;
      if constexpr (EPI == W2V2_EPI_SCALE_RC) rs = (mo + 16 * (i0 + i) < g.M) ? g.row_scale[mo + 16 * (i0 + i)] : 0.f;
      float v[16], pre[16];
#pragma unroll
      for (int e = 0; e < 16; ++e) {
        float x = acc[i0 + i][e >> 2][e & 3] * g.alpha;
        const float cve = e < 8 ? cv0[e] : cv1[e - 8];
        if constexpr (EPI == W2V2_EPI_BIAS) x += cve;
        if constexpr (EPI == W2V2_EPI_BIAS_GELU) { x += cve; pre[e] = x; x = gelu_f(x); }
        if constexpr (EPI == W2V2_EPI_BIAS_GELU_GRAD) { x += cve; gelu_both_f(x, x, pre[e]); }
        if constexpr (EPI == W2V2_EPI_GELU_BWD) x *= gelu_grad_f(ax[e]);
        if constexpr (EPI == W2V2_EPI_MUL) x *= ax[e];
        if constexpr (EPI == W2V2_EPI_ADD) x += ax[e];
        if constexpr (EPI == W2V2_EPI_SCALE_RC) x *= rs * cve;
        v[e] = x;
      }
      uint4 da, db;
      halves_to_lines(lo, pack8<TC>(v), pack8<TC>(v + 8), da, db);
      const int r = ra + 16 * (i0 + i);
      if constexpr (DEFER) {
        pend[2 * (i0 + i)] = da;
        pend[2 * (i0 + i) + 1] = db;
      } else {
        if (r < g.M) st16(Cz + (int64_t)r * g.ldc + ncs, da);
        if (r + 8 < g.M) st16(Cz + (int64_t)(r + 8) * g.ldc + ncs, db);
      }
      if constexpr (WRITES_AUX) {
        if (auxz != nullptr) {
          uint4 xa, xb;
          halves_to_lines(lo, pack8<TC>(pre), pack8<TC>(pre + 8), xa, xb);
          if (r < g.M) st16(auxz + (int64_t)r * g.ldaux + ncs, xa);
          if (r + 8 < g.M) st16(auxz + (int64_t)(r + 8) * g.ldaux + ncs, xb);
        }
      }
    }
  }
}

#define W2V2_EPI_DISPATCH(CALL)                                              \
  switch (g.epilogue) {                                                      \
    case W2V2_EPI_BIAS: { constexpr int EPI = W2V2_EPI_BIAS; CALL; } break;  \
    case W2V2_EPI_BIAS_GELU: { constexpr int EPI = W2V2_EPI_BIAS_GELU; CALL; } break; \
    case W2V2_EPI_GELU_BWD: { constexpr int EPI = W2V2_EPI_GELU_BWD; CALL; } break;   \
    case W2V2_EPI_ADD: { constexpr int EPI = W2V2_EPI_ADD; CALL; } break;    \
    case W2V2_EPI_SCALE_RC: { constexpr int EPI = W2V2_EPI_SCALE_RC; CALL; } break;   \
    case W2V2_EPI_BIAS_GELU_GRAD: { constexpr int EPI = W2V2_EPI_BIAS_GELU_GRAD; CALL; } break; \
    case W2V2_EPI_MUL: { constexpr int EPI = W2V2_EPI_MUL; CALL; } break;    \
    default: { constexpr int EPI = W2V2_EPI_NONE; CALL; } break;             \
  }

template <typename TC, int FM, int FN>
__device__ __forceinline__ void tile_epilogue(const GemmArgs& g, f32x4 (&acc)[FM][FN], float* __restrict__ stage,
                                              int m0, int n0, int wm, int wn, int z0, int z1, int split) {
  constexpr int BN = 32 * FN, ROWS = 16 * FM, PITCH = BN + 4, CPR = BN / 8;
  const int tid = threadIdx.x, lane = tid & 63;
  const int frow = lane & 15, fk = lane >> 4;
  TC* Cz = reinterpret_cast<TC*>(g.C) + z0 * g.c_s0 + z1 * g.c_s1;
  TC* auxz = g.aux ? reinterpret_cast<TC*>(g.aux) + z0 * g.aux_s0 + z1 * g.aux_s1 : nullptr;
  const float* bias = g.bias ? g.bias + z1 * g.bias_s1 : nullptr;
  float cv[8];
  load_col8(g, bias, n0 + (tid % CPR) * 8, cv);
#pragma unroll 1
  for (int pass = 0; pass < 2; ++pass) {
    __syncthreads();
    if (wm == pass) {
#pragma unroll
      for (int i = 0; i < FM; ++i)
#pragma unroll
        for (int j = 0; j < FN; ++j)
          *reinterpret_cast<float4*>(stage + (i * 16 + frow) * PITCH + wn * (16 * FN) + j * 16 + fk * 4) =
              make_float4(acc[i][j][0], acc[i][j][1], acc[i][j][2], acc[i][j][3]);
    }
    __syncthreads();
    W2V2_EPI_DISPATCH((epilogue_pass<TC, EPI, (ROWS * CPR) / 256, 256, BN>(g, stage, Cz, auxz, m0 + pass * ROWS, n0, cv,
                                                                        split == 0)));
  }
}

template <int NP>
__device__ __forceinline__ void tile_ptrs(const OpDev& o, const bf16_t* base, int t0, int TR, int bound, int row0,
                                          int step, const int* col, const bf16_t** out) {
  bool fast = t0 + TR <= bound;
  int64_t seg_base = 0;
  int first = t0;
  if (o.seg_len > 0) {
    const int sl = (int)o.seg_len;
    const int q0 = t0 / sl, q1 = (t0 + TR - 1) / sl;
    fast = fast && q0 == q1;
    seg_base = (int64_t)q0 * o.seg_stride;
    first = t0 - q0 * sl;
  }
  if (fast) {
    const bf16_t* p0 = base + seg_base + (int64_t)(first + row0) * o.ld;
#pragma unroll
    for (int j = 0; j < NP; ++j) out[j] = p0 + (int64_t)(j * step) * o.ld + col[j];
  } else {
#pragma unroll
    for (int j = 0; j < NP; ++j) out[j] = base + outer_off(o, min(t0 + row0 + j * step, bound - 1)) + col[j];
  }
}

__device__ __forceinline__ int xcd_remap(int bid, int nwg) {
  const int q = nwg >> 3, r = nwg & 7, xcd = bid & 7, loc = bid >> 3;
  return (xcd < r ? xcd * (q + 1) : r * (q + 1) + (xcd - r) * q) + loc;
}


typedef __attribute__((address_space(1))) const void gvoid_t;
typedef __attribute__((address_space(3))) void lvoid_t;

template <int N> __device__ __forceinline__ void wait_vmcnt() {
  static_assert(N >= 0 && N < 64, "vmcnt is a 6-bit counter");
  asm volatile("s_waitcnt vmcnt(%0)" ::"n"(N) : "memory");
}

int w2v2_gemm_device_cus();
int w2v2_launch_ring_256x128(const GemmArgs& a, int dtype_ab, int dtype_c, int M, int N, int batch, bool persistent,
                             hipStream_t st);
int w2v2_launch_phased_256x256(const GemmArgs& a, int dtype_ab, int dtype_c, int M, int N, int batch, hipStream_t st);
int w2v2_launch_gemm_f32(GemmArgs a, int M, int N, int K, int split, int batch, int dma_rows, hipStream_t st);
int w2v2_gemm_f32_dma_rows(const GemmArgs& a, int M, int N, int K, int split, int batch);
int w2v2_launch_gemm_f32_dma(const GemmArgs& a, int M, int N, int split, int batch, int fi, int nst, hipStream_t st);
bool w2v2_gemm_f32_dma_has_dbg(const GemmArgs& a, int fi);
```

### w2v2_speaker_amd/csrc/heads.hip

```cpp
#include "common.h"
#include <stdlib.h>

template <typename T>
__global__ __launch_bounds__(256) void row_invnorm_kernel(const T* __restrict__ x, int64_t ld, float* __restrict__ inv,
                                                          int rows, int cols) {
  const int lane = threadIdx.x & 63;
  const int row = blockIdx.x * 4 + (threadIdx.x >> 6);
  if (row >= rows) return;
  const T* xr = x + (int64_t)row * ld;
  float s = 0.f;
  if constexpr (sizeof(T) == 4) {
    if ((cols & 3) == 0 && (ld & 3) == 0 && (reinterpret_cast<uintptr_t>(x) & 15) == 0) {
      const float4* x4 = reinterpret_cast<const float4*>(xr);
      float s1 = 0.f, s2 = 0.f, s3 = 0.f;
      for (int c = lane; c < (cols >> 2); c += 64) {
        const float4 v = x4[c];
        s = fmaf(v.x, v.x, s); s1 = fmaf(v.y, v.y, s1); s2 = fmaf(v.z, v.z, s2); s3 = fmaf(v.w, v.w, s3);
      }
      s = (s + s1) + (s2 + s3);
    } else {
      for (int c = lane; c < cols; c += 64) { const float v = to_f32<T>(xr[c]); s = fmaf(v, v, s); }
    }
  } else {
    for (int c = lane; c < cols; c += 64) { const float v = to_f32<T>(xr[c]); s = fmaf(v, v, s); }
  }
  s = wave_sum(s);
  if (lane == 0) inv[row] = 1.0f / fmaxf(sqrtf(s), 1e-12f);
}

extern "C" int w2v2_row_invnorm(const void* x, int64_t ld, float* inv, int rows, int cols, int dtype, void* stream) {
  W2V2_REQUIRE(x && inv && rows > 0 && cols > 0 && ld >= cols, "row_invnorm: bad arguments");
  dim3 grid((unsigned)cdiv(rows, 4));
  W2V2_DISPATCH_ACT(dtype, "row_invnorm",
    hipLaunchKernelGGL(row_invnorm_kernel<AT>, grid, dim3(256), 0, as_stream(stream), (const AT*)x, ld, inv, rows, cols););
  W2V2_CHECK_LAUNCH("row_invnorm");
  return 0;
}

__device__ __forceinline__ float block_reduce(float v, float* sh, bool is_max) {
  v = is_max ? wave_max(v) : wave_sum(v);
  const int lane = threadIdx.x & 63, wave = threadIdx.x >> 6;
  __syncthreads();
  if (lane == 0) sh[wave] = v;
  __syncthreads();
  const float a = sh[0], b = sh[1], c = sh[2], d = sh[3];
  return is_max ? fmaxf(fmaxf(a, b), fmaxf(c, d)) : (a + b + c + d);
}

template <int NW>
__device__ __forceinline__ float block_reduce_n(float v, float* sh, bool is_max) {
  v = is_max ? wave_max(v) : wave_sum(v);
  const int lane = threadIdx.x & 63, wave = threadIdx.x >> 6;
  __syncthreads();
  if (lane == 0) sh[wave] = v;
  __syncthreads();
  float r = sh[0];
#pragma unroll
  for (int w = 1; w < NW; ++w) r = is_max ? fmaxf(r, sh[w]) : r + sh[w];
  return r;
}

template <int NW>
__device__ __forceinline__ void block_reduce_sum2(float& a, float& b, float* sha, float* shb) {
  a = wave_sum(a);
  b = wave_sum(b);
  const int lane = threadIdx.x & 63, wave = threadIdx.x >> 6;
  __syncthreads();
  if (lane == 0) { sha[wave] = a; shb[wave] = b; }
  __syncthreads();
  float ra = sha[0], rb = shb[0];
#pragma unroll
  for (int w = 1; w < NW; ++w) { ra += sha[w]; rb += shb[w]; }
  a = ra;
  b = rb;
}

constexpr int AAM_ROW_THREADS = 1024;
template <typename T>
__global__ __launch_bounds__(AAM_ROW_THREADS) void aam_row_kernel(const float* __restrict__ cosv, const int64_t* __restrict__ label,
                                                      float* __restrict__ softmax, float* __restrict__ loss_rows,
                                                      T* __restrict__ dcos_w, T* __restrict__ dcos_x,
                                                      const float* __restrict__ inv_x,
                                                      const float* __restrict__ inv_w, float* __restrict__ rowdot,
                                                      float* __restrict__ colprod, int B, int C, int64_t ldc,
                                                      float margin, float scale, const float* __restrict__ loss_scale,
                                                      float* __restrict__ correct_rows, int easy_margin) {
  constexpr int NT = AAM_ROW_THREADS, NW = NT / 64;
  __shared__ float sh[NW], sh2[NW];
  __shared__ int shi[NW];
  const int b = blockIdx.x;
  const int64_t yl = label[b];
  const bool bad_label = yl < 0 || yl >= C;
  const int y = bad_label ? 0 : (int)yl;
  const float* cr = cosv + (int64_t)b * ldc;
  const bool plain = margin < 0.f;
  float zy, dphi = 1.0f, sc = plain ? 1.0f : scale;
  {
    const float cy = cr[y];
    if (plain) {
      zy = cy;
    } else {
      const float cos_m = cosf(margin), sin_m = sinf(margin);
      const float th = cosf(3.14159265358979323846f - margin);
      const float mm = sinf(3.14159265358979323846f - margin) * margin;
      const float sine = sqrtf(fminf(fmaxf(1.0f - cy * cy, 0.f), 1.f));
      float phi = cy * cos_m - sine * sin_m;
      if (easy_margin ? (cy > 0.f) : (cy - th > 0.f)) {
        dphi = cos_m + sin_m * cy / fmaxf(sine, 1e-12f);
      } else {
        phi = easy_margin ? cy : cy - mm;
        dphi = 1.0f;
      }
      zy = phi * scale;
    }
  }
  float mx = -INFINITY;
  int amax = 0;
  for (int c = threadIdx.x; c < C; c += NT) {
    const float z = c == y ? zy : cr[c] * sc;
    if (z > mx) { mx = z; amax = c; }
  }
  const float mine = mx;
  mx = block_reduce_n<NW>(mx, sh, true);
  if (correct_rows != nullptr) {
    int cand = (mine == mx) ? amax : 0x7fffffff;
#pragma unroll
    for (int o = 32; o > 0; o >>= 1) cand = min(cand, __shfl_xor(cand, o, 64));
    __syncthreads();
    if ((threadIdx.x & 63) == 0) shi[threadIdx.x >> 6] = cand;
    __syncthreads();
    if (threadIdx.x == 0) {
      int best = shi[0];
#pragma unroll
      for (int w = 1; w < NW; ++w) best = min(best, shi[w]);
      correct_rows[b] = (!bad_label && best == y) ? 1.0f : 0.0f;
    }
  }
  float sum = 0.f, sum_off = 0.f;
  for (int c = threadIdx.x; c < C; c += NT) {
    const float e = __expf((c == y ? zy : cr[c] * sc) - mx);
    sum += e;
    if (c != y) sum_off += e;
  }
  block_reduce_sum2<NW>(sum, sum_off, sh, sh2);
  const float inv = 1.0f / sum;
  if (threadIdx.x == 0) loss_rows[b] = bad_label ? __builtin_nanf("") : (mx + __logf(sum)) - zy;
  const float invB = bad_label ? 0.f : (loss_scale ? loss_scale[0] : 1.0f) / (float)B;
  float rd = 0.f;
  for (int c = threadIdx.x; c < C; c += NT) {
    const float cv = cr[c];
    const float p = __expf((c == y ? zy : cv * sc) - mx) * inv;
    softmax[(int64_t)b * ldc + c] = p;
    if (dcos_w != nullptr) {
      float g = (p - (c == y ? 1.0f : 0.0f)) * invB * sc;
      if (c == y) {
        if (p > 0.5f) g = -(sum_off * inv) * invB * sc;
        g *= dphi;
      }
      dcos_w[(int64_t)b * ldc + c] = from_f32<T>(inv_w ? g * inv_w[c] : g);
      if (dcos_x != nullptr) dcos_x[(int64_t)b * ldc + c] = from_f32<T>(inv_x ? g * inv_x[b] : g);
      if (colprod != nullptr) {
        rd = fmaf(g, cv, rd);
        colprod[(int64_t)b * C + c] = g * cv;
      }
    }
  }
  if (rowdot != nullptr && dcos_w != nullptr) {
    rd = block_reduce_n<NW>(rd, sh, false);
    if (threadIdx.x == 0) rowdot[b] = rd;
  }
}

extern "C" int w2v2_aam_softmax_fwd_bwd(const float* cos, const int64_t* label, float* softmax, float* loss_rows,
                                        void* dcos_w, void* dcos_x, const float* inv_x, const float* inv_w,
                                        float* rowdot, float* colprod, int B, int C, int64_t ldc, float margin,
                                        float scale, const float* loss_scale, float* correct_rows, int easy_margin,
                                        int dtype, void* stream) {
  W2V2_REQUIRE(cos && label && softmax && loss_rows && B > 0 && C > 0 && ldc >= C, "aam_softmax: bad arguments");
  W2V2_DISPATCH_ACT(dtype, "aam_softmax",
    hipLaunchKernelGGL(aam_row_kernel<AT>, dim3(B), dim3(AAM_ROW_THREADS), 0, as_stream(stream), cos, label, softmax,
                       loss_rows, (AT*)dcos_w, (AT*)dcos_x, inv_x, inv_w, rowdot, colprod, B, C, ldc, margin,
                       scale, loss_scale, correct_rows, easy_margin););
  W2V2_CHECK_LAUNCH("aam_softmax");
  return 0;
}

template <typename TX>
__global__ void normalize_bwd_kernel(const float* __restrict__ g, const TX* __restrict__ x, int64_t ldx,
                                     const float* __restrict__ inv, const float* __restrict__ dot,
                                     float* __restrict__ dx, int rows, int cols, int add) {
  const int64_t total = (int64_t)rows * cols;
  for (int64_t i = blockIdx.x * (int64_t)blockDim.x + threadIdx.x; i < total; i += (int64_t)gridDim.x * blockDim.x) {
    const int r = (int)(i / cols), c = (int)(i - (int64_t)r * cols);
    const float iv = inv[r];
    const float v = iv * (g[i] - to_f32<TX>(x[(int64_t)r * ldx + c]) * iv * dot[r]);
    dx[i] = add ? dx[i] + v : v;
  }
}

extern "C" int w2v2_normalize_bwd(const float* g, const void* x, int64_t ldx, const float* inv, const float* dot,
                                  float* dx, int rows, int cols, int x_dtype, int add, void* stream) {
  W2V2_REQUIRE(g && x && inv && dot && dx && rows > 0 && cols > 0 && ldx >= cols, "normalize_bwd: bad arguments");
  const int64_t total = (int64_t)rows * cols;
  int nb = (int)(cdiv(total, 256) > 4096 ? 4096 : cdiv(total, 256));
  W2V2_DISPATCH_ACT(x_dtype, "normalize_bwd",
    hipLaunchKernelGGL(normalize_bwd_kernel<AT>, dim3(nb), dim3(256), 0, as_stream(stream), g, (const AT*)x,
                       ldx, inv, dot, dx, rows, cols, add););
  W2V2_CHECK_LAUNCH("normalize_bwd");
  return 0;
}

constexpr int ADW_CB = 16, ADW_EC = 512, ADW_BC = 36;
typedef __attribute__((ext_vector_type(2))) float f32x2_t;
template <typename T>
__global__ __launch_bounds__(256) void aam_dw_kernel(const T* __restrict__ dcos_x, int64_t ldc, const T* __restrict__ emb,
                                                     const float* __restrict__ colprod, const float* __restrict__ W,
                                                     const float* __restrict__ inv_w, float* __restrict__ dW, int B,
                                                     int Cn, int E, int chunk) {
  extern __shared__ __attribute__((aligned(16))) char adw_raw[];
  T* es = reinterpret_cast<T*>(adw_raw);
  float* dc = reinterpret_cast<float*>(adw_raw + (size_t)ADW_BC * ADW_EC * sizeof(T));
  float* cdp = dc + ADW_BC * ADW_CB;
  float* cd = cdp + 16 * ADW_CB;
  const int c0 = blockIdx.x * ADW_CB, ecol0 = blockIdx.y * ADW_EC, tid = threadIdx.x;
  const int q = tid & 127, h = tid >> 7;
  const int e0 = ecol0 + 4 * q;
  f32x2_t acc[4][4];
#pragma unroll
  for (int j = 0; j < 4; ++j)
#pragma unroll
    for (int k = 0; k < 4; ++k) acc[j][k] = f32x2_t{0.f, 0.f};
  {
    const int k = tid % ADW_CB, bl = tid / ADW_CB;
    float s = 0.f;
    if (c0 + k < Cn)
      for (int b = bl; b < B; b += 256 / ADW_CB) s += colprod[(int64_t)b * Cn + c0 + k];
    cdp[bl * ADW_CB + k] = s;
  }
  constexpr int VPR = ADW_EC * sizeof(T) / 16;
  constexpr int EPV = 16 / sizeof(T);
  for (int b0 = 0; b0 < B; b0 += chunk) {
    const int nb = min(chunk, B - b0);
    __syncthreads();
    for (int i0 = tid; i0 < nb * VPR; i0 += 256 * 8) {
      uint4 v[8];
#pragma unroll
      for (int u = 0; u < 8; ++u) {
        const int i = i0 + 256 * u, r = i / VPR, vcol = i - r * VPR;
        v[u] = make_uint4(0, 0, 0, 0);
        if (i < nb * VPR && ecol0 + vcol * EPV < E)
          v[u] = *reinterpret_cast<const uint4*>(emb + (int64_t)(b0 + r) * E + ecol0 + vcol * EPV);
      }
#pragma unroll
      for (int u = 0; u < 8; ++u) {
        const int i = i0 + 256 * u, r = i / VPR, vcol = i - r * VPR;
        if (i < nb * VPR) *reinterpret_cast<uint4*>(es + (int64_t)r * ADW_EC + vcol * EPV) = v[u];
      }
    }
    {
      constexpr int NDV = (ADW_BC * ADW_CB + 255) / 256;
      float dv[NDV];
#pragma unroll
      for (int u = 0; u < NDV; ++u) {
        const int i = tid + 256 * u, r = i / ADW_CB, k = i - r * ADW_CB;
        dv[u] = (r < nb && c0 + k < Cn) ? to_f32<T>(dcos_x[(int64_t)(b0 + r) * ldc + c0 + k]) : 0.f;
      }
#pragma unroll
      for (int u = 0; u < NDV; ++u)
        if (tid + 256 * u < ADW_BC * ADW_CB) dc[tid + 256 * u] = dv[u];
    }
    __syncthreads();
#pragma unroll 4
    for (int r = 0; r < nb; ++r) {
      float x[4];
      if constexpr (sizeof(T) == 2) {
        const uint2 w = *reinterpret_cast<const uint2*>(es + r * ADW_EC + 4 * q);
        unpack2<T>(w.x, x[0], x[1]);
        unpack2<T>(w.y, x[2], x[3]);
      } else {
        const float4 w = *reinterpret_cast<const float4*>(es + r * ADW_EC + 4 * q);
        x[0] = w.x; x[1] = w.y; x[2] = w.z; x[3] = w.w;
      }
      const float4 d0 = *reinterpret_cast<const float4*>(dc + r * ADW_CB + h * 8);
      const float4 d1 = *reinterpret_cast<const float4*>(dc + r * ADW_CB + h * 8 + 4);
      const f32x2_t d[4] = {{d0.x, d0.y}, {d0.z, d0.w}, {d1.x, d1.y}, {d1.z, d1.w}};
#pragma unroll
      for (int j = 0; j < 4; ++j)
#pragma unroll
        for (int k = 0; k < 4; ++k) acc[j][k] = __builtin_elementwise_fma(d[k], f32x2_t{x[j], x[j]}, acc[j][k]);
    }
  }
  __syncthreads();
  if (tid < ADW_CB) {
    float s = 0.f;
    for (int l = 0; l < 256 / ADW_CB; ++l) s += cdp[l * ADW_CB + tid];
    cd[tid] = s;
  }
  __syncthreads();
  if (e0 >= E) return;
  float4 wv[8];
  float ivv[8];
#pragma unroll
  for (int k = 0; k < 8; ++k) {
    const int c = min(c0 + h * 8 + k, Cn - 1);
    wv[k] = *reinterpret_cast<const float4*>(W + (int64_t)c * E + e0);
    ivv[k] = inv_w[c];
  }
#pragma unroll
  for (int k = 0; k < 8; ++k) {
    const int c = c0 + h * 8 + k;
    const float iv = ivv[k], sc = iv * cd[h * 8 + k];
    const float w4[4] = {wv[k].x, wv[k].y, wv[k].z, wv[k].w};
    float o[4];
#pragma unroll
    for (int j = 0; j < 4; ++j) o[j] = iv * (acc[j][k >> 1][k & 1] - w4[j] * sc);
    if (c < Cn) *reinterpret_cast<float4*>(dW + (int64_t)c * E + e0) = make_float4(o[0], o[1], o[2], o[3]);
  }
}

extern "C" int w2v2_aam_dw(const void* dcos_x, int64_t ldc, const void* emb, const float* colprod, const float* W,
                           const float* inv_w, float* dW, int B, int Cn, int E, int dtype, void* stream) {
  W2V2_REQUIRE(dcos_x && emb && colprod && W && inv_w && dW && B > 0 && Cn > 0 && E > 0 && ldc >= Cn, "aam_dw: bad arguments");
  W2V2_REQUIRE(E % 8 == 0 && ((uintptr_t)emb | (uintptr_t)W | (uintptr_t)dW) % 16 == 0,
               "aam_dw: embedding dim %d must be a multiple of 8 and the operands 16-byte aligned (else: the GEMM path)", E);
  dim3 grid((unsigned)cdiv(Cn, ADW_CB), (unsigned)cdiv(E, ADW_EC));
  hipStream_t st = as_stream(stream);
  W2V2_DISPATCH_ACT(dtype, "aam_dw", {
    const size_t lds = (size_t)ADW_BC * ADW_EC * sizeof(AT) + (size_t)(ADW_BC * ADW_CB + 16 * ADW_CB + ADW_CB) * sizeof(float);
    const int nchunk = (int)cdiv(B, ADW_BC), chunk = (int)cdiv(B, nchunk);
    if (w2v2_launch_lds<&aam_dw_kernel<AT>>("aam_dw_kernel", grid, dim3(256), lds, st, (const AT*)dcos_x, ldc, (const AT*)emb,
                                            colprod, W, inv_w, dW, B, Cn, E, chunk) != 0)
      return -1;
  });
  W2V2_CHECK_LAUNCH("aam_dw");
  return 0;
}

__global__ __launch_bounds__(64) void bce_row_kernel(const float* __restrict__ emb, const float* __restrict__ w,
                                                     const float* __restrict__ b, const int64_t* __restrict__ label,
                                                     float* __restrict__ prob, float* __restrict__ loss_rows,
                                                     float* __restrict__ dlogit, float* __restrict__ demb, int B,
                                                     int H, const float* __restrict__ loss_scale) {
  const int row = blockIdx.x, lane = threadIdx.x;
  const float* e = emb + (int64_t)row * H;
  float s = 0.f;
  for (int h = lane; h < H; h += 64) s = fmaf(e[h], w[h], s);
  s = wave_sum(s) + b[0];
  const int64_t yl = label[row];
  const bool bad_label = yl != 0 && yl != 1;
  const float y = (float)yl;
  const float p = 1.0f / (1.0f + __expf(-s));
  const float l = fmaxf(s, 0.f) - s * y + log1pf(__expf(-fabsf(s)));
  const float dl = bad_label ? 0.f : (p - y) * (loss_scale ? loss_scale[0] : 1.0f) / (float)B;
  if (lane == 0) {
    prob[row] = p;
    loss_rows[row] = bad_label ? __builtin_nanf("") : l;
    if (dlogit != nullptr) dlogit[row] = dl;
  }
  if (demb != nullptr)
    for (int h = lane; h < H; h += 64) demb[(int64_t)row * H + h] = dl * w[h];
}
__global__ void bce_wgrad_kernel(const float* __restrict__ emb, const float* __restrict__ dlogit,
                                 float* __restrict__ dw, float* __restrict__ db, int B, int H) {
  const int h = blockIdx.x * blockDim.x + threadIdx.x;
  if (h < H) {
    float s = 0.f;
    for (int r = 0; r < B; ++r) s = fmaf(dlogit[r], emb[(int64_t)r * H + h], s);
    dw[h] = s;
  }
  if (h == 0) {
    float s = 0.f;
    for (int r = 0; r < B; ++r) s += dlogit[r];
    db[0] = s;
  }
}

extern "C" int w2v2_bce_head_fwd_bwd(const float* emb, const float* w, const float* b, const int64_t* label, float* prob,
                                     float* loss_rows, float* dlogit, float* demb, float* dw, float* db, int B, int H,
                                     const float* loss_scale, void* stream) {
  W2V2_REQUIRE(emb && w && b && label && prob && loss_rows && B > 0 && H > 0, "bce_head: bad arguments");
  W2V2_REQUIRE((dlogit == nullptr) == (demb == nullptr) && (demb == nullptr) == (dw == nullptr) &&
                   (dw == nullptr) == (db == nullptr),
               "bce_head: gradient outputs come together");
  hipStream_t st = as_stream(stream);
  hipLaunchKernelGGL(bce_row_kernel, dim3(B), dim3(64), 0, st, emb, w, b, label, prob, loss_rows, dlogit, demb, B, H,
                     loss_scale);
  if (dw != nullptr)
    hipLaunchKernelGGL(bce_wgrad_kernel, dim3((unsigned)cdiv(H, 256)), dim3(256), 0, st, emb, dlogit, dw, db, B, H);
  W2V2_CHECK_LAUNCH("bce_head");
  return 0;
}
```

### w2v2_speaker_amd/heads.py

```python
from __future__ import annotations

from typing import Optional

import torch

from . import ops
from .ops import EPI_BIAS, EPI_SCALE_RC, Gemm


class ClassifierHead:
    def __init__(self, kind: str, batch: int, embed_dim: int, classes: int, *, w_master: torch.Tensor,
                 w_operand: torch.Tensor, w_grad: Optional[torch.Tensor], bias: Optional[torch.Tensor] = None,
                 bias_grad: Optional[torch.Tensor] = None, emb: torch.Tensor, act_dtype: torch.dtype,
                 train: bool, margin: float = 0.2, scale: float = 30.0, loss_scale: Optional[torch.Tensor] = None,
                 easy_margin: bool = False):
        assert kind in ("aam", "ce")
        self.loss_scale = loss_scale
        self.kind, self.B, self.E, self.C, self.train = kind, batch, embed_dim, classes, train
        self.margin, self.scale, self.easy_margin = margin, scale, bool(easy_margin)
        self.w_master, self.w_grad, self.bias, self.bias_grad, self.emb = w_master, w_grad, bias, bias_grad, emb
        dev, f32 = emb.device, torch.float32
        B, E, Cn = batch, embed_dim, classes
        self.ldc = (Cn + 7) // 8 * 8
        self.emb_lp = torch.empty(B, E, dtype=act_dtype, device=dev) if act_dtype != f32 else emb
        self.logits = torch.zeros(B, self.ldc, dtype=f32, device=dev)
        self.softmax = torch.zeros(B, self.ldc, dtype=f32, device=dev)
        self.loss_rows = torch.empty(B, dtype=f32, device=dev)
        self.correct = torch.zeros(B, dtype=f32, device=dev)
        aam = kind == "aam"
        if aam:
            self.inv_x, self.inv_w = torch.empty(B, dtype=f32, device=dev), torch.empty(Cn, dtype=f32, device=dev)
            self.g_fwd = Gemm(B, Cn, E, self.emb_lp, w_operand, self.logits, lda=E, ldb=E, ldc=self.ldc,
                              epilogue=EPI_SCALE_RC, row_scale=self.inv_x, col_scale=self.inv_w)
        else:
            self.g_fwd = Gemm(B, Cn, E, self.emb_lp, w_operand, self.logits, lda=E, ldb=E, ldc=self.ldc,
                              epilogue=EPI_BIAS, bias=bias)
        if train:
            self.dcos_w = torch.zeros(B, self.ldc, dtype=act_dtype, device=dev)
            self.dcos_x = torch.zeros(B, self.ldc, dtype=act_dtype, device=dev) if aam else self.dcos_w
            self.rowdot = torch.empty(B, dtype=f32, device=dev)
            self._zbuf = torch.empty(Cn + B * E, dtype=f32, device=dev)
            self._ztab = torch.tensor([[0, Cn + B * E]], dtype=torch.int64, device=dev)
            self.coldot = self._zbuf[:Cn]
            self.G1 = self._zbuf[Cn:].view(B, E)
            self.colprod = torch.empty(B, Cn, dtype=f32, device=dev) if aam else None
            self.demb = torch.empty(B, E, dtype=f32, device=dev)
            S = max(1, min(16, Cn // 256))
            Kc = (Cn // S) // 8 * 8 if S > 1 else Cn
            rest = Cn - S * Kc
            self.dx_parts = torch.empty(S + (1 if rest else 0), B, E, dtype=f32, device=dev)
            self.g_dx = [Gemm(B, E, Kc, self.dcos_w, w_operand, self.dx_parts, lda=self.ldc, ldb=E, ldc=E, transB=True,
                              batch=S, batch_inner=S, a_strides=(0, Kc), b_strides=(0, Kc * E), c_strides=(0, B * E))]
            if rest:
                self.g_dx.append(Gemm(B, E, rest, self.dcos_w.view(-1)[S * Kc:], w_operand.view(-1)[S * Kc * E:],
                                      self.dx_parts[S], lda=self.ldc, ldb=E, ldc=E, transB=True))
            self.fused_dw = aam and E % 8 == 0
            if aam and not self.fused_dw:
                self.H1 = torch.empty(Cn, E, dtype=f32, device=dev)
                self.g_dw = Gemm(Cn, E, B, self.dcos_x, self.emb_lp, self.H1, lda=self.ldc, ldb=E, ldc=E,
                                 transA=True, transB=True)
            elif not aam:
                self.g_dw = Gemm(Cn, E, B, self.dcos_x, self.emb_lp, w_grad, lda=self.ldc, ldb=E, ldc=E,
                                 transA=True, transB=True, accumulate=True)

    def forward_backward(self, label: torch.Tensor):
        B, E, Cn = self.B, self.E, self.C
        assert label.dtype == torch.int64 and label.is_cuda and label.shape == (B,)
        aam, tr = self.kind == "aam", self.train
        if self.emb_lp is not self.emb:
            ops.cast(self.emb, self.emb_lp)
        if aam:
            ops.row_invnorm(self.emb, self.inv_x, B, E)
            ops.row_invnorm(self.w_master, self.inv_w, Cn, E)
        self.g_fwd()
        if tr:
            ops.zero_ranges(self._zbuf, self._ztab, blocks_per_range=16)
        ops.aam_softmax_fwd_bwd(self.logits, label, self.softmax, self.loss_rows,
                                self.dcos_w if tr else None, (self.dcos_x if aam else None) if tr else None,
                                self.inv_x if aam else None, self.inv_w if aam else None,
                                self.rowdot if (tr and aam) else None, self.colprod if (tr and aam) else None,
                                B, Cn, self.ldc, self.margin if aam else -1.0, self.scale, self.loss_scale if tr else None,
                                self.correct, easy_margin=self.easy_margin)
        loss = torch.empty((), dtype=torch.float32, device=self.loss_rows.device)
        ops.mean(self.loss_rows, loss)
        if tr:
            for g in self.g_dx:
                g()
            ops.colsum(self.dx_parts, self.G1.view(-1), self.dx_parts.shape[0], B * E)
            if aam:
                ops.normalize_bwd(self.G1, self.emb, self.inv_x, self.rowdot, self.demb, B, E)
                if self.fused_dw:
                    ops.aam_dw(self.dcos_x, self.emb_lp, self.colprod, self.w_master, self.inv_w, self.w_grad, B, Cn, E,
                               self.ldc)
                else:
                    self.g_dw()
                    ops.colsum(self.colprod, self.coldot, B, Cn)
                    ops.normalize_bwd(self.H1, self.w_master, self.inv_w, self.coldot, self.w_grad, Cn, E)
            else:
                self.demb.copy_(self.G1)
                self.g_dw()
                ops.colsum(self.dcos_w, self.bias_grad, B, Cn, self.ldc)
        return loss, self.softmax[:, :Cn]


class BceHead:

    def __init__(self, batch: int, embed_dim: int, *, w: torch.Tensor, b: torch.Tensor,
                 w_grad: Optional[torch.Tensor], b_grad: Optional[torch.Tensor], emb: torch.Tensor, train: bool,
                 loss_scale: Optional[torch.Tensor] = None):
        dev, f32 = emb.device, torch.float32
        self.loss_scale = loss_scale
        self.B, self.E, self.w, self.b, self.w_grad, self.b_grad, self.emb, self.train = (batch, embed_dim, w, b, w_grad,
                                                                                          b_grad, emb, train)
        self.prob = torch.empty(batch, dtype=f32, device=dev)
        self.loss_rows = torch.empty(batch, dtype=f32, device=dev)
        self.dlogit = torch.empty(batch, dtype=f32, device=dev) if train else None
        self.demb = torch.empty(batch, embed_dim, dtype=f32, device=dev) if train else None

    def forward_backward(self, label: torch.Tensor):
        assert label.dtype == torch.int64 and label.is_cuda and label.shape == (self.B,)
        tr = self.train
        ops.bce_head_fwd_bwd(self.emb, self.w.view(-1), self.b, label, self.prob, self.loss_rows,
                             self.dlogit if tr else None, self.demb if tr else None,
                             self.w_grad.view(-1) if tr else None, self.b_grad if tr else None, self.B, self.E,
                             self.loss_scale if tr else None)
        loss = torch.empty((), dtype=torch.float32, device=self.loss_rows.device)
        ops.mean(self.loss_rows, loss)
        return loss, self.prob



class FcStack:

    def __init__(self, store, batch: int, in_dim: int, hidden, x0: torch.Tensor, train: bool):
        dev, f32 = x0.device, torch.float32
        self.B, self.dims, self.train = batch, [in_dim] + list(hidden), train
        self.x = [x0] + [torch.empty(batch, h, dtype=f32, device=dev) for h in hidden]
        self.w = [store.p(f"fc_list.{i}.0.weight") for i in range(len(hidden))]
        self.b = [store.p(f"fc_list.{i}.0.bias") for i in range(len(hidden))]
        if train:
            self.dw = [store.g(f"fc_list.{i}.0.weight") for i in range(len(hidden))]
            self.db = [store.g(f"fc_list.{i}.0.bias") for i in range(len(hidden))]
            self.dx = [torch.empty(batch, d, dtype=f32, device=dev) for d in self.dims]

    def forward(self, upto: Optional[int] = None) -> torch.Tensor:
        n = len(self.w) if upto is None else upto + 1
        for i in range(n):
            ops.skinny_linear_fwd(self.x[i], self.w[i], self.b[i], self.x[i + 1], ops.ACT_RELU)
        return self.x[n]

    def backward(self, dout: torch.Tensor) -> torch.Tensor:
        n = len(self.w)
        self.dx[n].copy_(dout)
        for i in reversed(range(n)):
            ops.skinny_linear_bwd_w(self.dx[i + 1], self.x[i + 1], self.x[i], self.dw[i], self.db[i], ops.ACT_RELU, True)
            ops.skinny_linear_bwd_x(self.dx[i + 1], self.x[i + 1], self.w[i], self.dx[i], ops.ACT_RELU)
        return self.dx[0]
```

### w2v2_speaker_amd/ops.py

```python
from __future__ import annotations

import ctypes as C
from typing import Optional, Tuple

import torch

from . import _lib
from ._lib import (BF16, EPI_ADD, EPI_BIAS, EPI_BIAS_GELU, EPI_BIAS_GELU_GRAD, EPI_GELU_BWD, EPI_MUL, EPI_NONE, EPI_SCALE_RC, F16, F32,
                   GemmDesc)

POOL_MODES = {"mean+std": 0, "mean": 1, "max": 2, "first": 3, "first+cls": 3, "last": 4, "middle": 4, "quantile": 5}
POOL_WIDTH = {0: 2, 5: 5}
POOL_INDEX_BASE = 16


def lib():
    return _lib.load()


def dt(t: torch.Tensor) -> int:
    if t.dtype == torch.bfloat16:
        return BF16
    if t.dtype == torch.float16:
        return F16
    if t.dtype == torch.float32:
        return F32
    raise TypeError(f"unsupported dtype {t.dtype}")


def is16(dtype: torch.dtype) -> bool:
    return dtype in (torch.bfloat16, torch.float16)


def stream() -> int:
    return torch.cuda.current_stream().cuda_stream


def _p(t: Optional[torch.Tensor]):
    return None if t is None else t.data_ptr()


def _dev(*ts):
    for t in ts:
        if t is not None and not t.is_cuda:
            raise RuntimeError("w2v2_speaker_amd ops need tensors on the GPU (no CPU fallback exists)")


class Gemm:

    def __init__(self, M: int, N: int, K: int, A: torch.Tensor, B: torch.Tensor, Cmat: torch.Tensor, *,
                 lda: int, ldb: int, ldc: int, transA: bool = False, transB: bool = False,
                 batch: int = 1, batch_inner: int = 1,
                 a_strides: Tuple[int, int] = (0, 0), b_strides: Tuple[int, int] = (0, 0),
                 c_strides: Tuple[int, int] = (0, 0),
                 a_seg: Tuple[int, int] = (0, 0), b_seg: Tuple[int, int] = (0, 0),
                 epilogue: int = EPI_NONE, bias: Optional[torch.Tensor] = None, bias_stride1: int = 0,
                 aux: Optional[torch.Tensor] = None, ldaux: int = 0, aux_strides: Tuple[int, int] = (0, 0),
                 row_scale: Optional[torch.Tensor] = None, col_scale: Optional[torch.Tensor] = None,
                 alpha: float = 1.0, split_k: int = 1, accumulate: bool = False,
                 b_lo: Optional[torch.Tensor] = None, n_ext_from: int = 0):
        _dev(A, B, Cmat, bias, aux, row_scale, col_scale, b_lo)
        if dt(A) != dt(B):
            raise TypeError("GEMM operands must share a dtype")
        if aux is not None and aux.dtype != Cmat.dtype:
            raise TypeError("aux must have the dtype of C")
        for t in (bias, row_scale, col_scale):
            if t is not None and t.dtype != torch.float32:
                raise TypeError("bias / scales are f32")
        d = GemmDesc()
        d.M, d.N, d.K = M, N, K
        d.batch, d.batch_inner = batch, max(1, batch_inner)
        d.dtype_ab, d.dtype_c, d.epilogue = dt(A), dt(Cmat), epilogue
        d.A.ptr, d.A.ld, d.A.trans = A.data_ptr(), lda, int(transA)
        d.A.seg_len, d.A.seg_stride = a_seg
        d.A.stride0, d.A.stride1 = a_strides
        d.B.ptr, d.B.ld, d.B.trans = B.data_ptr(), ldb, int(transB)
        d.B.seg_len, d.B.seg_stride = b_seg
        d.B.stride0, d.B.stride1 = b_strides
        d.C, d.ldc = Cmat.data_ptr(), ldc
        d.c_stride0, d.c_stride1 = c_strides
        d.aux, d.ldaux = _p(aux), ldaux
        d.aux_stride0, d.aux_stride1 = aux_strides
        d.bias, d.bias_stride1 = _p(bias), bias_stride1
        d.row_scale, d.col_scale = _p(row_scale), _p(col_scale)
        d.alpha, d.split_k, d.accumulate = alpha, split_k, int(accumulate)
        d.k_ext, d.n_ext_from, d.b_lo_offset = 0, 0, 0
        if b_lo is not None:
            assert b_lo.dtype == B.dtype and (b_lo.data_ptr() - B.data_ptr()) % B.element_size() == 0
            d.k_ext, d.n_ext_from = K, n_ext_from
            d.b_lo_offset = (b_lo.data_ptr() - B.data_ptr()) // B.element_size()
        self.desc = d
        self._ref = C.byref(d)
        self._keep = (A, B, Cmat, bias, aux, row_scale, col_scale, b_lo)
        self._fn = lib().w2v2_gemm
        self.flops = 2.0 * M * N * K * batch
        esz = A.element_size()
        self.bytes = float(batch) * ((M * K + N * K) * esz + M * N * Cmat.element_size() * (2 if aux is not None else 1))
        lp = dt(A) != F32
        self.kernel_class = ("mfma16" if lp else "f32") + "_" + ("t" if transA else "n") + ("n" if transB else "t")
        self.narrow = N <= 64
        self.out_is_act = is16(Cmat.dtype)
        fam = lib().w2v2_gemm_kernel_of(self._ref)
        self.kernel_name = {4: "gemm16_phased_256x256_kernel", 2: "gemm16_ring_256x128_kernel", 1: "gemm16_dma_128_kernel",
                            3: "gemm16_regstage_kernel", 9: "gemm_f32_mfma_kernel",
                            10: "gemm_f32_dma_kernel"}.get(fam, "gemm16_regstage_kernel" if lp
                                                                                       else "gemm_f32_mfma_kernel")

    _prof = None
    _TIMED_KERNELS = ("gemm16_ring_256x128_kernel", "gemm16_phased_256x256_kernel")
    _log = None

    def key(self) -> dict:
        d = self.desc
        return {"kind": "gemm", "M": d.M, "N": d.N, "K": d.K, "batch": d.batch, "epi": d.epilogue,
                "two_term": int(d.k_ext != 0), "n_ext_from": d.n_ext_from, "aux": int(bool(d.aux)),
                "kernel": self.kernel_name, "flops": self.flops + 2.0 * d.M * max(0, d.N - d.n_ext_from) * d.k_ext,
                "alg_flops": self.flops, "bytes": self.bytes}

    @classmethod
    def profile_begin(cls, select) -> None:
        cls._prof = {"select": select, "events": [], "slots": []}

    @classmethod
    def profile_end(cls) -> dict:
        prof, cls._prof = cls._prof, None
        if not prof or not (prof["events"] or prof["slots"]):
            return {"launches": 0, "ms": 0.0, "flops": 0.0, "bytes": 0.0, "by_kernel": {}}
        torch.cuda.synchronize()
        out = {"launches": 0, "ms": 0.0, "flops": 0.0, "bytes": 0.0, "by_kernel": {}}
        timed = []
        if prof["slots"]:
            import ctypes
            buf = (ctypes.c_float * len(prof["slots"]))()
            _lib.check(lib().w2v2_timer_read(0, len(prof["slots"]), ctypes.cast(buf, ctypes.c_void_p)), "timer_read")
            timed = [(float(buf[i]),) + prof["slots"][i] for i in range(len(prof["slots"]))]
        for ms, f, nb, name in [(a.elapsed_time(b), f, nb, name) for a, b, f, nb, name in prof["events"]] + timed:
            k = out["by_kernel"].setdefault(name, {"launches": 0, "ms": 0.0, "flops": 0.0, "bytes": 0.0})
            for d in (out, k):
                d["launches"] += 1
                d["ms"] += ms
                d["flops"] += f
                d["bytes"] += nb
        return out

    def __call__(self) -> None:
        prof = Gemm._prof
        if Gemm._log is not None:
            Gemm._log.append(self.key())
        if (prof is not None and prof["select"](self) and self.kernel_name in Gemm._TIMED_KERNELS
                and hasattr(lib(), "w2v2_gemm_timed")):
            rc = lib().w2v2_gemm_timed(self._ref, stream(), len(prof["slots"]))
            prof["slots"].append((self.flops, self.bytes, self.kernel_name))
        elif prof is not None and prof["select"](self):
            e0, e1 = torch.cuda.Event(enable_timing=True), torch.cuda.Event(enable_timing=True)
            e0.record()
            rc = self._fn(self._ref, stream())
            e1.record()
            prof["events"].append((e0, e1, self.flops, self.bytes, self.kernel_name))
        else:
            rc = self._fn(self._ref, stream())
        if rc:
            _lib.check(rc, "gemm")


def gemm(*args, **kw) -> None:
    Gemm(*args, **kw)()


class WgradGroup:

    def __init__(self, problems, tokens: int, tokens_padded: int):
        n = len(problems)
        arr = (_lib.WgradProblem * n)()
        keep = []
        self.flops = 0.0
        for i, (dY, X, dW, db) in enumerate(problems):
            _dev(dY, X, dW, db)
            assert is16(dY.dtype) and X.dtype == dY.dtype and dW.dtype == torch.float32
            assert i == 0 or dY.dtype == problems[0][0].dtype, "one element type per grouped launch"
            assert dY.shape[0] >= tokens_padded and X.shape[0] >= tokens_padded
            q = arr[i]
            q.dY, q.ld_dy = dY.data_ptr(), dY.stride(0)
            q.X, q.ld_x = X.data_ptr(), X.stride(0)
            q.dW, q.ld_dw = dW.data_ptr(), dW.stride(0)
            q.dbias = _p(db)
            q.n_out, q.n_in = dW.shape
            keep.append((dY, X, dW, db))
            self.flops += 2.0 * tokens * dW.shape[0] * dW.shape[1]
        self._arr, self._keep, self._n = arr, keep, n
        self._tokens, self._tpad = tokens, tokens_padded
        self._dt = dt(problems[0][0])
        self._fn = lib().w2v2_wgrad_grouped
        self.kernel_name = self._KERNELS.get(lib().w2v2_wgrad_kernel_of(arr, n), "rejected")

    _KERNELS = {1: "wgrad_grouped_kernel", 2: "wgrad_grouped_ring_kernel", 3: "wgrad_grouped_ring4_kernel",
                4: "wgrad_grouped_phased_kernel"}

    def __call__(self) -> None:
        if Gemm._log is not None:
            Gemm._log.append({"kind": "wgrad", "problems": self._n, "tokens": self._tokens, "flops": self.flops,
                              "alg_flops": self.flops,
                              "kernel": self.kernel_name})
        rc = self._fn(self._arr, self._n, self._tokens, self._tpad, self._dt, stream())
        if rc:
            _lib.check(rc, "wgrad_grouped")


def conv0_workspace(B: int, N: int, C: int, k: int, stride: int, device) -> torch.Tensor:
    n = lib().w2v2_conv0_workspace_floats(N, C, k, stride)
    return torch.empty(B * n + B * C * 2, dtype=torch.float32, device=device)


def conv0_groupnorm_gelu(wav: torch.Tensor, w: torch.Tensor, gamma: torch.Tensor, beta: torch.Tensor,
                         out: torch.Tensor, work: torch.Tensor, k: int, stride: int, eps: float = 1e-5) -> None:
    _dev(wav, w, gamma, beta, out, work)
    B, N = wav.shape
    Cc = w.shape[0]
    mr = work[work.numel() - B * Cc * 2:]
    L = lib()
    stats = L.w2v2_conv0_stats_mfma if is16(out.dtype) else L.w2v2_conv0_stats
    _lib.check(stats(wav.data_ptr(), w.data_ptr(), work.data_ptr(), mr.data_ptr(), B, N, Cc, k, stride,
                     eps, stream()), "conv0_stats")
    _lib.check(L.w2v2_conv0_apply(wav.data_ptr(), w.data_ptr(), mr.data_ptr(), gamma.data_ptr(), beta.data_ptr(),
                                  out.data_ptr(), dt(out), B, N, Cc, k, stride, stream()), "conv0_apply")


def conv0_stats_len(wav, w, work, frames, k: int, stride: int, mfma: bool, eps: float = 1e-5) -> torch.Tensor:
    _dev(wav, w, work, frames)
    assert frames.dtype == torch.int32
    B, N = wav.shape
    Cc = w.shape[0]
    mr = work[work.numel() - B * Cc * 2:]
    fn = lib().w2v2_conv0_stats_mfma_len if mfma else lib().w2v2_conv0_stats_len
    _lib.check(fn(wav.data_ptr(), w.data_ptr(), work.data_ptr(), mr.data_ptr(), frames.data_ptr(), B, N, Cc, k, stride,
                  eps, stream()), "conv0_stats_len")
    return mr.view(B, Cc, 2)


def conv0_groupnorm_gelu_len(wav, w, gamma, beta, out, work, frames, k: int, stride: int, eps: float = 1e-5) -> None:
    _dev(wav, w, gamma, beta, out, work, frames)
    B, N = wav.shape
    Cc = w.shape[0]
    mr = conv0_stats_len(wav, w, work, frames, k, stride, is16(out.dtype), eps)
    _lib.check(lib().w2v2_conv0_apply(wav.data_ptr(), w.data_ptr(), mr.data_ptr(), gamma.data_ptr(), beta.data_ptr(),
                                      out.data_ptr(), dt(out), B, N, Cc, k, stride, stream()), "conv0_apply")


def conv0_layernorm_gelu(wav, w, bias, gamma, beta, out, k: int, stride: int, eps: float = 1e-5) -> None:
    _dev(wav, w, bias, gamma, beta, out)
    B, N = wav.shape
    _lib.check(lib().w2v2_conv0_layernorm_gelu(wav.data_ptr(), w.data_ptr(), _p(bias), gamma.data_ptr(), beta.data_ptr(),
                                               out.data_ptr(), B, N, out.shape[-1], k, stride, eps, dt(out), stream()),
               "conv0_layernorm_gelu")


def conv0_layernorm_gelu_bwd_workspace(B: int, N: int, C: int, k: int, stride: int, device) -> torch.Tensor:
    n = lib().w2v2_conv0_layernorm_gelu_bwd_workspace_floats(B, N, C, k, stride)
    return torch.empty(max(n, 1), dtype=torch.float32, device=device)


def conv0_layernorm_gelu_bwd(wav, w, bias, gamma, beta, dy, dw, dbias, dgamma, dbeta, work, k: int, stride: int,
                             eps: float = 1e-5) -> None:
    _dev(wav, w, bias, gamma, beta, dy, dw, dbias, dgamma, dbeta, work)
    B, N = wav.shape
    Cc = dy.shape[-1]
    if work.numel() < lib().w2v2_conv0_layernorm_gelu_bwd_workspace_floats(B, N, Cc, k, stride):
        raise ValueError("conv0_layernorm_gelu_bwd: workspace too small")
    _lib.check(lib().w2v2_conv0_layernorm_gelu_bwd(wav.data_ptr(), w.data_ptr(), _p(bias), gamma.data_ptr(), beta.data_ptr(),
                                                   dy.data_ptr(), dw.data_ptr(), _p(dbias), dgamma.data_ptr(),
                                                   dbeta.data_ptr(), work.data_ptr(), B, N, Cc, k, stride, eps, dt(dy),
                                                   stream()), "conv0_layernorm_gelu_bwd")


def conv0_bwd(wav, w, work, gamma, beta, dz, sums, dw, dgamma, dbeta, k: int, stride: int) -> None:
    _dev(wav, w, work, gamma, beta, dz, sums, dw, dgamma, dbeta)
    B, N = wav.shape
    Cc = w.shape[0]
    mr = work[work.numel() - B * Cc * 2:]
    _lib.check(lib().w2v2_conv0_bwd(wav.data_ptr(), w.data_ptr(), mr.data_ptr(), gamma.data_ptr(), beta.data_ptr(),
                                    dz.data_ptr(), sums.data_ptr(), dw.data_ptr(), dgamma.data_ptr(), dbeta.data_ptr(),
                                    dt(dz), B, N, Cc, k, stride, stream()), "conv0_bwd")


def col2im(col, dx, B: int, Lin: int, Lout: int, Cin: int, k: int, stride: int) -> None:
    _dev(col, dx)
    _lib.check(lib().w2v2_col2im(col.data_ptr(), dx.data_ptr(), B, Lin, Lout, Cin, k, stride, dt(col), stream()),
               "col2im")


def unpack_conv_grad(gp, g) -> None:
    _dev(gp, g)
    co, ci, k = g.shape
    _lib.check(lib().w2v2_unpack_conv_grad(gp.data_ptr(), g.data_ptr(), co, ci, k, stream()), "unpack_conv_grad")


def pack_conv_weight(w: torch.Tensor, out: torch.Tensor) -> None:
    _dev(w, out)
    co, ci, k = w.shape
    _lib.check(lib().w2v2_pack_conv_weight(w.data_ptr(), out.data_ptr(), dt(out), co, ci, k, stream()), "pack_conv")


def layernorm_fwd(x, r, gamma, beta, y, mean, rstd, eps: float, drop_p: float = 0.0, seed: int = 0) -> None:
    _dev(x, r, gamma, beta, y, mean, rstd)
    H = x.shape[-1]
    M = x.numel() // H
    _lib.check(lib().w2v2_layernorm_fwd(x.data_ptr(), _p(r), gamma.data_ptr(), beta.data_ptr(), y.data_ptr(),
                                        mean.data_ptr(), rstd.data_ptr(), M, H, eps, drop_p, seed, dt(x), stream()),
               "layernorm_fwd")


def layernorm_gelu_fwd(x, gamma, beta, y, eps: float) -> None:
    _dev(x, gamma, beta, y)
    H = x.shape[-1]
    _lib.check(lib().w2v2_layernorm_gelu_fwd(x.data_ptr(), gamma.data_ptr(), beta.data_ptr(), y.data_ptr(), x.numel() // H, H,
                                             eps, dt(x), stream()), "layernorm_gelu_fwd")


def layernorm_gelu_bwd_workspace(M: int, H: int, device) -> torch.Tensor:
    return torch.empty(max(lib().w2v2_layernorm_gelu_bwd_workspace_floats(M, H), 1), dtype=torch.float32, device=device)


def layernorm_gelu_bwd(dy, z, gamma, beta, dz, dgamma, dbeta, dbias, work, eps: float = 1e-5) -> None:
    _dev(dy, z, gamma, beta, dz, dgamma, dbeta, dbias, work)
    H = dy.shape[-1]
    M = dy.numel() // H
    if work.numel() < lib().w2v2_layernorm_gelu_bwd_workspace_floats(M, H):
        raise ValueError("layernorm_gelu_bwd: workspace too small")
    _lib.check(lib().w2v2_layernorm_gelu_bwd(dy.data_ptr(), z.data_ptr(), gamma.data_ptr(), beta.data_ptr(), dz.data_ptr(),
                                             dgamma.data_ptr(), dbeta.data_ptr(), _p(dbias), work.data_ptr(), M, H, eps,
                                             dt(dy), stream()), "layernorm_gelu_bwd")


_LN_WS = {}


def _ln_workspace(H: int, device) -> torch.Tensor:
    key = (H, str(device))
    if key not in _LN_WS:
        _LN_WS[key] = torch.empty(lib().w2v2_layernorm_bwd_workspace_floats(H), dtype=torch.float32, device=device)
    return _LN_WS[key]


def layernorm_bwd(dy, s, mean, rstd, gamma, ds, d_r, dgamma, dbeta, drop_p: float = 0.0, seed: int = 0,
                  defer_to: Optional["LnFoldGroup"] = None) -> None:
    _dev(dy, s, mean, rstd, gamma, ds, d_r, dgamma, dbeta)
    H = dy.shape[-1]
    M = dy.numel() // H
    if defer_to is not None and dgamma is not None:
        ws = defer_to.add(dgamma, dbeta, M, H)
        _lib.check(lib().w2v2_layernorm_bwd(dy.data_ptr(), s.data_ptr(), mean.data_ptr(), rstd.data_ptr(),
                                            gamma.data_ptr(), ds.data_ptr(), _p(d_r), None, None, ws.data_ptr(), M, H,
                                            drop_p, seed, dt(dy), stream()), "layernorm_bwd")
        return
    ws = _ln_workspace(H, dy.device) if dgamma is not None else None
    _lib.check(lib().w2v2_layernorm_bwd(dy.data_ptr(), s.data_ptr(), mean.data_ptr(), rstd.data_ptr(),
                                        gamma.data_ptr(), ds.data_ptr(), _p(d_r), _p(dgamma), _p(dbeta), _p(ws), M, H,
                                        drop_p, seed, dt(dy), stream()), "layernorm_bwd")


class LnFoldGroup:

    def __init__(self, H: int, device, slots: int = 8):
        n = lib().w2v2_layernorm_bwd_workspace_floats(H)
        self._ws = torch.empty(slots, n, dtype=torch.float32, device=device)
        self._arr = (_lib.LnFold * slots)()
        self._n, self._M, self._H, self._keep = 0, 0, H, []

    def add(self, dgamma, dbeta, M: int, H: int) -> torch.Tensor:
        if self._n == len(self._arr):
            self.fold()
        assert H == self._H and (self._n == 0 or M == self._M)
        e = self._arr[self._n]
        e.partial, e.dgamma, e.dbeta = self._ws[self._n].data_ptr(), dgamma.data_ptr(), dbeta.data_ptr()
        self._keep.append((dgamma, dbeta))
        self._M = M
        self._n += 1
        return self._ws[self._n - 1]

    def fold(self) -> None:
        if self._n:
            _lib.check(lib().w2v2_layernorm_bwd_fold(self._arr, self._n, self._M, self._H, stream()),
                       "layernorm_bwd_fold")
        self._n, self._keep = 0, []


def dropout_(x: torch.Tensor, p: float, seed: int) -> None:
    _dev(x)
    _lib.check(lib().w2v2_dropout(x.data_ptr(), x.data_ptr(), x.numel(), p, seed, dt(x), stream()), "dropout")


def gelu_bwd(dy, pre, dx) -> None:
    _dev(dy, pre, dx)
    _lib.check(lib().w2v2_gelu_bwd(dy.data_ptr(), pre.data_ptr(), dx.data_ptr(), dy.numel(), dt(dy), stream()),
               "gelu_bwd")


PARTIAL_ROWS = 256
_PARTIAL_WS = {}


def _partial_workspace(N: int, device, st: int) -> torch.Tensor:
    key = (N, str(device), st)
    if key not in _PARTIAL_WS:
        _PARTIAL_WS[key] = torch.empty(PARTIAL_ROWS * N, dtype=torch.float32, device=device)
    return _PARTIAL_WS[key]


def gelu_bwd_colsum(dy, pre, dx, colsum_out, M: int, N: int) -> None:
    _dev(dy, pre, dx, colsum_out)
    st = stream()
    ws = _partial_workspace(N, dy.device, st)
    _lib.check(lib().w2v2_gelu_bwd_colsum(dy.data_ptr(), pre.data_ptr(), dx.data_ptr(), colsum_out.data_ptr(),
                                          ws.data_ptr(), M, N, dt(dy), st), "gelu_bwd_colsum")


def add(x, a, y) -> None:
    _dev(x, a, y)
    _lib.check(lib().w2v2_add(x.data_ptr(), a.data_ptr(), y.data_ptr(), x.numel(), dt(x), stream()), "add")


def colsum(x: torch.Tensor, out: torch.Tensor, M: int, N: int, ld: Optional[int] = None) -> None:
    _dev(x, out)
    _lib.check(lib().w2v2_colsum(x.data_ptr(), ld if ld is not None else N, out.data_ptr(), M, N, dt(x), stream()),
               "colsum")


def zero_ranges(base: torch.Tensor, table: torch.Tensor, blocks_per_range: int = 8) -> None:
    _dev(base, table)
    assert base.dtype == torch.float32 and table.dtype == torch.int64
    _lib.check(lib().w2v2_zero_ranges(base.data_ptr(), table.data_ptr(), table.shape[0], blocks_per_range, stream()),
               "zero_ranges")


def mean(x: torch.Tensor, out: torch.Tensor) -> None:
    _dev(x, out)
    assert x.dtype == torch.float32 and out.dtype == torch.float32
    _lib.check(lib().w2v2_mean(x.data_ptr(), out.data_ptr(), x.numel(), stream()), "mean")


def cast(x: torch.Tensor, y: torch.Tensor) -> None:
    _dev(x, y)
    _lib.check(lib().w2v2_cast(x.data_ptr(), y.data_ptr(), x.numel(), dt(y), stream()), "cast")


def transpose_many(src, dst, table, n: int, blocks_per_matrix: int = 64) -> None:
    _dev(src, dst, table)
    _lib.check(lib().w2v2_transpose_many(src.data_ptr(), dst.data_ptr(), table.data_ptr(), n, blocks_per_matrix,
                                         dt(src), stream()), "transpose_many")


def mask_fill(h, mask_u8, embed) -> None:
    _dev(h, mask_u8, embed)
    H = h.shape[-1]
    _lib.check(lib().w2v2_mask_fill(h.data_ptr(), mask_u8.data_ptr(), embed.data_ptr(), h.numel() // H, H, dt(h),
                                    stream()), "mask_fill")


def mask_feature(h, mask_u8, B: int, T: int) -> None:
    _dev(h, mask_u8)
    H = h.shape[-1]
    assert mask_u8.dtype == torch.uint8 and mask_u8.numel() == B * H
    _lib.check(lib().w2v2_mask_feature(h.data_ptr(), mask_u8.data_ptr(), B, T, H, dt(h), stream()), "mask_feature")


def mask_fill_bwd(dh, mask_u8, d_embed) -> None:
    _dev(dh, mask_u8, d_embed)
    H = dh.shape[-1]
    st = stream()
    ws = _partial_workspace(H, dh.device, st)
    _lib.check(lib().w2v2_mask_fill_bwd(dh.data_ptr(), mask_u8.data_ptr(), d_embed.data_ptr(), ws.data_ptr(),
                                        dh.numel() // H, H, dt(dh), st), "mask_fill_bwd")


def prepend_token(x, y, c: float) -> None:
    _dev(x, y)
    B, T, H = x.shape
    _lib.check(lib().w2v2_prepend_token(x.data_ptr(), y.data_ptr(), c, B, T, H, dt(x), stream()), "prepend_token")


def pair_tables(left_row, left_frames, right_row, right_frames, rows: int, T: int) -> torch.Tensor:
    as_list = lambda x: x.reshape(-1).tolist() if isinstance(x, torch.Tensor) else list(x)
    cols = [[int(v) for v in as_list(x)] for x in (left_row, left_frames, right_row, right_frames)]
    if len({len(c) for c in cols}) != 1 or not cols[0]:
        raise ValueError("pair_assemble: the four tables need one entry per pair (at least one pair)")
    for b, (lr, ta, rr, tb) in enumerate(zip(*cols)):
        if ta < 1 or tb < 1:
            raise ValueError(f"pair_assemble: pair {b} has an empty side ({ta} + {tb} frames)")
        if ta + tb + 3 > T:
            raise ValueError(f"pair_assemble: pair {b} needs {ta + tb + 3} frames, the sequence has {T}")
        if lr < 0 or rr < 0 or lr + ta > rows or rr + tb > rows:
            raise ValueError(f"pair_assemble: pair {b} reads rows [{lr}, {lr + ta}) and [{rr}, {rr + tb}) of a feature "
                             f"matrix of {rows}")
    return torch.tensor(cols, dtype=torch.int32)


def pair_assemble(feat, y, left_row, left_frames, right_row, right_frames, cls_c: float, sep_c: float,
                  table: Optional[torch.Tensor] = None) -> torch.Tensor:
    _dev(feat, y)
    B, T, H = y.shape
    assert feat.dim() == 2 and feat.shape[1] == H and feat.dtype == y.dtype and feat.is_contiguous() and y.is_contiguous()
    host = pair_tables(left_row, left_frames, right_row, right_frames, feat.shape[0], T)
    if host.shape[1] != B:
        raise ValueError(f"pair_assemble: {host.shape[1]} pairs for a batch of {B}")
    if table is None:
        table = torch.empty(4, B, dtype=torch.int32, device=y.device)
    assert table.shape == (4, B) and table.dtype == torch.int32 and table.is_cuda and table.is_contiguous()
    table.copy_(host)
    _lib.check(lib().w2v2_pair_assemble(feat.data_ptr(), y.data_ptr(), table[0].data_ptr(), table[1].data_ptr(),
                                        table[2].data_ptr(), table[3].data_ptr(), cls_c, sep_c, B, T, H, dt(y), stream()),
               "pair_assemble")
    return host


def posconv_wgrad(dY, xg, dwf, B: int, T: int, H: int, G: int, K: int) -> None:
    _dev(dY, xg, dwf)
    assert is16(dY.dtype) and xg.dtype == dY.dtype and dwf.dtype == torch.float32
    _lib.check(lib().w2v2_posconv_wgrad(dY.data_ptr(), xg.data_ptr(), dwf.data_ptr(), B, T, H, G, K, dt(dY), stream()),
               "posconv_wgrad")


def posconv_direct(xg, w, out, aux, bias, B: int, T: int, G: int, Cg: int, K: int, ldc: int, mode: int) -> None:
    _dev(xg, w, out, aux, bias)
    assert is16(xg.dtype) and w.dtype == xg.dtype and out.dtype == xg.dtype
    _lib.check(lib().w2v2_posconv_direct(xg.data_ptr(), w.data_ptr(), out.data_ptr(), _p(aux), _p(bias), B, T, G, Cg, K,
                                         ldc, mode, dt(xg), stream()), "posconv_direct")
    if Gemm._log is not None:
        Gemm._log.append({"kind": "posconv", "flops": 2.0 * B * T * G * Cg * K * Cg, "alg_flops": 2.0 * B * T * G * Cg * K * Cg,
                          "kernel": "posconv_direct_kernel", "M": B * T, "N": Cg, "K": K * Cg, "mode": mode})


def posconv_regroup(x, xg, B: int, T: int, H: int, G: int, K: int, pad_left: int) -> None:
    _dev(x, xg)
    _lib.check(lib().w2v2_posconv_regroup(x.data_ptr(), xg.data_ptr(), B, T, H, G, K, pad_left, dt(x), stream()),
               "posconv_regroup")


def posconv_regroup_len(x, xg, lens, B: int, T: int, H: int, G: int, K: int, pad_left: int) -> None:
    _dev(x, xg, lens)
    _lib.check(lib().w2v2_posconv_regroup_len(x.data_ptr(), xg.data_ptr(), lens.data_ptr(), B, T, H, G, K, pad_left,
                                              dt(x), stream()), "posconv_regroup_len")


def weightnorm_scratch(H: int, G: int, K: int, device) -> torch.Tensor:
    return torch.empty(int(lib().w2v2_weightnorm_scratch_floats(H, G, K)), dtype=torch.float32, device=device)


def weightnorm_pack(g, v, sumsq, wf, wb, H: int, G: int, K: int) -> None:
    _dev(g, v, sumsq, wf, wb)
    _lib.check(lib().w2v2_weightnorm_pack(g.data_ptr(), v.data_ptr(), sumsq.data_ptr(), wf.data_ptr(),
                                          wb.data_ptr(), H, G, K, dt(wf), stream()), "weightnorm_pack")


def weightnorm_bwd(g, v, sumsq, dwf, dot, dg, dv, H: int, G: int, K: int) -> None:
    _dev(g, v, sumsq, dwf, dot, dg, dv)
    _lib.check(lib().w2v2_weightnorm_bwd(g.data_ptr(), v.data_ptr(), sumsq.data_ptr(), dwf.data_ptr(),
                                         dot.data_ptr(), dg.data_ptr(), dv.data_ptr(), H, G, K, stream()),
               "weightnorm_bwd")


def softmax_fwd(s, p, p_drop, rows: int, T: int, ld: int, drop_p: float, seed: int) -> None:
    _dev(s, p, p_drop)
    _lib.check(lib().w2v2_softmax_fwd(s.data_ptr(), p.data_ptr(), _p(p_drop), rows, T, ld, drop_p, seed, dt(p),
                                      stream()), "softmax_fwd")


def softmax_fwd_len(s, p, lens, B: int, heads: int, T: int, ld: int) -> None:
    _dev(s, p, lens)
    _lib.check(lib().w2v2_softmax_fwd_len(s.data_ptr(), p.data_ptr(), lens.data_ptr(), B, heads, T, ld, dt(p),
                                          stream()), "softmax_fwd_len")


def softmax_bwd(dp_drop, p, ds, rows: int, T: int, ld: int, drop_p: float, seed: int) -> None:
    _dev(dp_drop, p, ds)
    _lib.check(lib().w2v2_softmax_bwd(dp_drop.data_ptr(), p.data_ptr(), ds.data_ptr(), rows, T, ld, drop_p, seed,
                                      dt(p), stream()), "softmax_bwd")


def attention_fwd(qkv, ctx, lse, B: int, T: int, heads: int, d: int, scale: float, drop_p: float, seed: int) -> None:
    _dev(qkv, ctx, lse)
    _lib.check(lib().w2v2_attention_fwd(qkv.data_ptr(), ctx.data_ptr(), lse.data_ptr(), B, T, heads, d, scale,
                                        drop_p, seed, dt(qkv), stream()), "attention_fwd")


def attention_fwd_len(qkv, ctx, lse, lens, B: int, T: int, heads: int, d: int, scale: float) -> None:
    _dev(qkv, ctx, lse, lens)
    _lib.check(lib().w2v2_attention_fwd_len(qkv.data_ptr(), ctx.data_ptr(), lse.data_ptr(), lens.data_ptr(), B, T, heads,
                                            d, scale, dt(qkv), stream()), "attention_fwd_len")


def attention_bwd(qkv, ctx, dctx, lse, dqkv, delta, B: int, T: int, heads: int, d: int, scale: float,
                  drop_p: float, seed: int) -> None:
    _dev(qkv, ctx, dctx, lse, dqkv, delta)
    _lib.check(lib().w2v2_attention_bwd(qkv.data_ptr(), ctx.data_ptr(), dctx.data_ptr(), lse.data_ptr(),
                                        dqkv.data_ptr(), delta.data_ptr(), B, T, heads, d, scale, drop_p, seed,
                                        dt(qkv), stream()), "attention_bwd")


def pool_fwd(x, out, mode: int) -> None:
    _dev(x, out)
    B, T, H = x.shape
    _lib.check(lib().w2v2_pool_fwd(x.data_ptr(), out.data_ptr(), B, T, H, mode, dt(x), stream()), "pool_fwd")


def pool_fwd_len(x, out, lens, mode: int) -> None:
    _dev(x, out, lens)
    B, T, H = x.shape
    _lib.check(lib().w2v2_pool_fwd_len(x.data_ptr(), out.data_ptr(), lens.data_ptr(), B, T, H, mode, dt(x), stream()),
               "pool_fwd_len")


def pool_bwd(x, out, dout, dx, mode: int) -> None:
    _dev(x, out, dout, dx)
    B, T, H = x.shape
    _lib.check(lib().w2v2_pool_bwd(x.data_ptr(), out.data_ptr(), dout.data_ptr(), dx.data_ptr(), B, T, H, mode,
                                   dt(x), stream()), "pool_bwd")


def row_invnorm(x, inv, rows: int, cols: int, ld: Optional[int] = None) -> None:
    _dev(x, inv)
    _lib.check(lib().w2v2_row_invnorm(x.data_ptr(), ld if ld is not None else cols, inv.data_ptr(), rows, cols,
                                      dt(x), stream()), "row_invnorm")


def aam_softmax_fwd_bwd(cos, label, softmax, loss_rows, dcos_w, dcos_x, inv_x, inv_w, rowdot, colprod, B: int,
                        Cn: int, ldc: int, margin: float, scale: float, loss_scale=None, correct_rows=None,
                        easy_margin: bool = False) -> None:
    _dev(cos, label, softmax, loss_rows, dcos_w, dcos_x, inv_x, inv_w, rowdot, colprod, loss_scale, correct_rows)
    dty = dt(dcos_w) if dcos_w is not None else F32
    _lib.check(lib().w2v2_aam_softmax_fwd_bwd(cos.data_ptr(), label.data_ptr(), softmax.data_ptr(),
                                              loss_rows.data_ptr(), _p(dcos_w), _p(dcos_x), _p(inv_x), _p(inv_w),
                                              _p(rowdot), _p(colprod), B, Cn, ldc, margin, scale, _p(loss_scale),
                                              _p(correct_rows), int(easy_margin), dty, stream()),
               "aam_softmax")


def normalize_bwd(g, x, inv, dot, dx, rows: int, cols: int, ldx: Optional[int] = None, add_to: bool = False) -> None:
    _dev(g, x, inv, dot, dx)
    _lib.check(lib().w2v2_normalize_bwd(g.data_ptr(), x.data_ptr(), ldx if ldx is not None else cols, inv.data_ptr(),
                                        dot.data_ptr(), dx.data_ptr(), rows, cols, dt(x), int(add_to), stream()),
               "normalize_bwd")


def aam_dw(dcos_x, emb, colprod, w_master, inv_w, dw, B: int, Cn: int, E: int, ldc: int) -> None:
    _dev(dcos_x, emb, colprod, w_master, inv_w, dw)
    assert emb.dtype == dcos_x.dtype and dw.dtype == torch.float32 and w_master.dtype == torch.float32
    _lib.check(lib().w2v2_aam_dw(dcos_x.data_ptr(), ldc, emb.data_ptr(), colprod.data_ptr(), w_master.data_ptr(),
                                 inv_w.data_ptr(), dw.data_ptr(), B, Cn, E, dt(emb), stream()), "aam_dw")


def adam_step(p, g, m, v, pb, n: int, lr: float, beta1: float, beta2: float, eps: float, step: int,
              grad_scale: float = 1.0, scaler=None, skip_slot: int = 0) -> None:
    _dev(p, g, m, v, pb, scaler)
    bc1 = 1.0 - beta1 ** step
    bc2 = 1.0 - beta2 ** step
    _lib.check(lib().w2v2_adam_step(p.data_ptr(), g.data_ptr(), m.data_ptr(), v.data_ptr(), _p(pb),
                                    dt(pb) if pb is not None else BF16, n, lr, beta1, beta2, eps, bc1, bc2, grad_scale,
                                    _p(scaler), step, skip_slot, stream()), "adam_step")


def optim_step(algo: str, p, g, m, v, pb, n: int, lr: float, beta1: float = 0.9, beta2: float = 0.999, eps: float = 1e-8,
               step: int = 1, grad_scale: float = 1.0, scaler=None, skip_slot: int = 0, weight_decay: float = 0.0,
               momentum: float = 0.0, dampening: float = 0.0, nesterov: bool = False, norm_state=None) -> None:
    if algo not in ("adam", "sgd"):
        raise ValueError(f"optim_step: algo must be 'adam' or 'sgd', got {algo!r}")
    _dev(p, g, m, v, pb, scaler, norm_state)
    adam = algo == "adam"
    bc1 = 1.0 - beta1 ** step if adam else 1.0
    bc2 = 1.0 - beta2 ** step if adam else 1.0
    _lib.check(lib().w2v2_optim_step(_lib.OPTIM_ADAM if adam else _lib.OPTIM_SGD, p.data_ptr(), g.data_ptr(), _p(m), _p(v),
                                     _p(pb), dt(pb) if pb is not None else BF16, n, lr, beta1, beta2, eps, bc1, bc2,
                                     grad_scale, weight_decay, momentum, dampening, int(bool(nesterov)), _p(norm_state),
                                     _p(scaler), step, skip_slot, stream()), "optim_step")


def grad_norm_partials(n: int) -> int:
    return int(lib().w2v2_grad_norm_partials(n))


def grad_norm(g, n: int, norm_state, partials, grad_scale: float = 1.0, scaler=None, max_norm: float = 0.0) -> None:
    _dev(g, norm_state, partials, scaler)
    assert partials.dtype == torch.float64 and norm_state.dtype == torch.float32 and norm_state.numel() >= 2
    _lib.check(lib().w2v2_grad_norm(g.data_ptr(), n, grad_scale, _p(scaler), max_norm, partials.data_ptr(),
                                    partials.numel(), norm_state.data_ptr(), stream()), "grad_norm")


def grad_accumulate(acc, g, n: int, first: bool) -> None:
    _dev(acc, g)
    assert acc.dtype == torch.float32 and g.dtype == torch.float32 and acc.numel() >= n and g.numel() >= n
    _lib.check(lib().w2v2_grad_accumulate(acc.data_ptr(), g.data_ptr(), n, int(bool(first)), stream()), "grad_accumulate")


def weight_residual(p, lo, table) -> None:
    _dev(p, lo, table)
    _lib.check(lib().w2v2_weight_residual(p.data_ptr(), lo.data_ptr(), table.data_ptr(), table.shape[0], dt(lo), stream()),
               "weight_residual")


def grad_scaler_check(g, n: int, state) -> None:
    _dev(g, state)
    _lib.check(lib().w2v2_grad_scaler_check(g.data_ptr(), n, state.data_ptr(), stream()), "grad_scaler_check")


def grad_scaler_update(state, growth: float = 2.0, backoff: float = 0.5, growth_interval: int = 2000,
                       skipped_ranges: int = 0) -> None:
    _dev(state)
    assert skipped_ranges == 0 or state.numel() >= 8
    _lib.check(lib().w2v2_grad_scaler_update(state.data_ptr(), growth, backoff, growth_interval, skipped_ranges, stream()),
               "grad_scaler_update")


def asp_context(x, ctx, B: int, T: int, C: int) -> None:
    _dev(x, ctx)
    _lib.check(lib().w2v2_asp_context(x.data_ptr(), ctx.data_ptr(), B, T, C, dt(x), stream()), "asp_context")


def asp_context_len(x, ctx, lens, B: int, T: int, C: int) -> None:
    _dev(x, ctx, lens)
    _lib.check(lib().w2v2_asp_context_len(x.data_ptr(), ctx.data_ptr(), lens.data_ptr(), B, T, C, dt(x), stream()),
               "asp_context_len")


def asp_context_bias(ctx, w1, b1, cb, B: int, A: int, C: int) -> None:
    _dev(ctx, w1, b1, cb)
    _lib.check(lib().w2v2_asp_context_bias(ctx.data_ptr(), w1.data_ptr(), b1.data_ptr(), cb.data_ptr(), B, A, C,
                                           stream()), "asp_context_bias")


def asp_bn_workspace(M: int, A: int, device) -> torch.Tensor:
    return torch.empty(lib().w2v2_asp_bn_workspace_floats(M, A), dtype=torch.float32, device=device)


def asp_bn_stats(a_pre, work, mean_rstd, running, M: int, A: int, eps: float, momentum: float) -> None:
    _dev(a_pre, work, mean_rstd, running)
    _lib.check(lib().w2v2_asp_bn_stats(a_pre.data_ptr(), work.data_ptr(), mean_rstd.data_ptr(), _p(running), M, A, eps,
                                       momentum, dt(a_pre), stream()), "asp_bn_stats")


def asp_bn_eval_stats(running, mean_rstd, A: int, eps: float) -> None:
    _dev(running, mean_rstd)
    _lib.check(lib().w2v2_asp_bn_eval_stats(running.data_ptr(), mean_rstd.data_ptr(), A, eps, stream()),
               "asp_bn_eval_stats")


def asp_bn_tanh(a_pre, mean_rstd, gamma, beta, h, M: int, A: int) -> None:
    _dev(a_pre, mean_rstd, gamma, beta, h)
    _lib.check(lib().w2v2_asp_bn_tanh(a_pre.data_ptr(), mean_rstd.data_ptr(), gamma.data_ptr(), beta.data_ptr(),
                                      h.data_ptr(), M, A, dt(a_pre), stream()), "asp_bn_tanh")


def asp_bn_bwd(dh, a_pre, mean_rstd, gamma, beta, work, dgamma, dbeta, da, M: int, A: int) -> None:
    _dev(dh, a_pre, mean_rstd, gamma, beta, work, dgamma, dbeta, da)
    _lib.check(lib().w2v2_asp_bn_bwd(dh.data_ptr(), a_pre.data_ptr(), mean_rstd.data_ptr(),
                                     gamma.data_ptr(), beta.data_ptr(), work.data_ptr(), dgamma.data_ptr(), dbeta.data_ptr(),
                                     da.data_ptr(), M, A, dt(dh), stream()), "asp_bn_bwd")


def asp_pool_fwd(x, s, out, stats, B: int, T: int, C: int) -> None:
    _dev(x, s, out, stats)
    _lib.check(lib().w2v2_asp_pool_fwd(x.data_ptr(), s.data_ptr(), out.data_ptr(), stats.data_ptr(), B, T, C, dt(x),
                                       stream()), "asp_pool_fwd")


def asp_pool_fwd_len(x, s, out, stats, lens, B: int, T: int, C: int) -> None:
    _dev(x, s, out, stats, lens)
    _lib.check(lib().w2v2_asp_pool_fwd_len(x.data_ptr(), s.data_ptr(), out.data_ptr(), stats.data_ptr(), lens.data_ptr(),
                                           B, T, C, dt(x), stream()), "asp_pool_fwd_len")


def asp_pool_bwd(x, s, out, stats, dout, ds, dx, B: int, T: int, C: int) -> None:
    _dev(x, s, out, stats, dout, ds, dx)
    _lib.check(lib().w2v2_asp_pool_bwd(x.data_ptr(), s.data_ptr(), out.data_ptr(), stats.data_ptr(), dout.data_ptr(),
                                       ds.data_ptr(), dx.data_ptr(), B, T, C, dt(x), stream()), "asp_pool_bwd")


def asp_context_bwd(x, ctx, da, w1, dw1, dx, scratch, B: int, T: int, C: int, A: int) -> None:
    _dev(x, ctx, da, w1, dw1, dx, scratch)
    _lib.check(lib().w2v2_asp_context_bwd(x.data_ptr(), ctx.data_ptr(), da.data_ptr(), w1.data_ptr(), dw1.data_ptr(),
                                          dx.data_ptr(), scratch.data_ptr(), B, T, C, A, dt(x), stream()),
               "asp_context_bwd")


def bn_workspace(M: int, C: int, device) -> torch.Tensor:
    return torch.empty(lib().w2v2_bn_workspace_floats(M, C), dtype=torch.float32, device=device)


def bn_fwd(a, lda: int, work, mean_rstd, running, gamma, beta, y, ldy: int, M: int, C: int, eps: float,
           momentum: float, relu: bool, train: bool) -> None:
    _dev(a, work, mean_rstd, running, gamma, beta, y)
    _lib.check(lib().w2v2_bn_fwd(a.data_ptr(), lda, _p(work), mean_rstd.data_ptr(), _p(running), gamma.data_ptr(),
                                 beta.data_ptr(), y.data_ptr(), ldy, M, C, eps, momentum, int(relu), int(train), dt(a),
                                 stream()), "bn_fwd")


def bn_colsum_rows(M: int, C: int) -> int:
    return int(lib().w2v2_bn_colsum_rows(M, C))


def bn_bwd(dy, lddy: int, a, lda: int, mean_rstd, gamma, work, dgamma, dbeta, da, ldda: int, M: int, C: int,
           relu: bool, colsum_partial=None, dy2=None, lddy2: int = 0) -> None:
    _dev(dy, a, mean_rstd, gamma, work, dgamma, dbeta, da, colsum_partial, dy2)
    if dy2 is None:
        _lib.check(lib().w2v2_bn_bwd(dy.data_ptr(), lddy, a.data_ptr(), lda, mean_rstd.data_ptr(), gamma.data_ptr(),
                                     work.data_ptr(), dgamma.data_ptr(), dbeta.data_ptr(), da.data_ptr(), ldda, M, C,
                                     int(relu), _p(colsum_partial), dt(a), stream()), "bn_bwd")
    else:
        _lib.check(lib().w2v2_bn_bwd_sum(dy.data_ptr(), lddy, dy2.data_ptr(), lddy2, a.data_ptr(), lda,
                                         mean_rstd.data_ptr(), gamma.data_ptr(), work.data_ptr(), dgamma.data_ptr(),
                                         dbeta.data_ptr(), da.data_ptr(), ldda, M, C, int(relu), _p(colsum_partial),
                                         dt(a), stream()), "bn_bwd_sum")


def im2col_reflect(x, ldx: int, col, B: int, T: int, Cin: int, k: int, dilation: int, x2=None, ldx2: int = 0) -> None:
    _dev(x, col, x2)
    if x2 is None:
        _lib.check(lib().w2v2_im2col_reflect(x.data_ptr(), ldx, col.data_ptr(), B, T, Cin, k, dilation, dt(x), stream()),
                   "im2col_reflect")
    else:
        _lib.check(lib().w2v2_im2col_reflect_sum(x.data_ptr(), ldx, x2.data_ptr(), ldx2, col.data_ptr(), B, T, Cin, k,
                                                 dilation, dt(x), stream()), "im2col_reflect_sum")


def im2col_reflect_len(x, ldx: int, col, lens, B: int, T: int, Cin: int, k: int, dilation: int, x2=None,
                       ldx2: int = 0) -> None:
    _dev(x, col, lens, x2)
    if x2 is None:
        _lib.check(lib().w2v2_im2col_reflect_len(x.data_ptr(), ldx, col.data_ptr(), lens.data_ptr(), B, T, Cin, k,
                                                 dilation, dt(x), stream()), "im2col_reflect_len")
    else:
        _lib.check(lib().w2v2_im2col_reflect_sum_len(x.data_ptr(), ldx, x2.data_ptr(), ldx2, col.data_ptr(),
                                                     lens.data_ptr(), B, T, Cin, k, dilation, dt(x), stream()),
                   "im2col_reflect_sum_len")


def col2im_reflect(dcol, dx, lddx: int, B: int, T: int, Cin: int, k: int, dilation: int, accumulate: bool) -> None:
    _dev(dcol, dx)
    _lib.check(lib().w2v2_col2im_reflect(dcol.data_ptr(), dx.data_ptr(), lddx, B, T, Cin, k, dilation,
                                         int(accumulate), dt(dcol), stream()), "col2im_reflect")


def add_strided(a, lda: int, b, ldb: int, y, ldy: int, M: int, C: int) -> None:
    _dev(a, b, y)
    _lib.check(lib().w2v2_add_strided(a.data_ptr(), lda, _p(b), ldb, y.data_ptr(), ldy, M, C, dt(a), stream()),
               "add_strided")


def copy_strided(a, lda: int, y, ldy: int, M: int, C: int) -> None:
    add_strided(a, lda, None, 0, y, ldy, M, C)


FBANK_HOP, FBANK_WIN, FBANK_TILE_FRAMES = 160, 400, 16


def fbank_partial_max(B: int, T: int, device) -> torch.Tensor:
    return torch.empty(B, -(-T // FBANK_TILE_FRAMES), dtype=torch.float32, device=device)


def _fbank_f32(*ts) -> None:
    for t in ts:
        if t.dtype != torch.float32 or not t.is_contiguous():
            raise ValueError("fbank: wav, window, fbank, db and partial_max are contiguous f32 tensors")


def fbank_db(wav, lens, window, fbank, db, partial_max) -> None:
    _dev(wav, lens, window, fbank, db, partial_max)
    _fbank_f32(wav, window, fbank, db, partial_max)
    B, N = wav.shape
    T, n_mels = 1 + N // FBANK_HOP, fbank.shape[1]
    if (window.numel() != FBANK_WIN or fbank.shape[0] != FBANK_WIN // 2 + 1 or tuple(db.shape) != (B, T, n_mels)
            or partial_max.numel() < B * -(-T // FBANK_TILE_FRAMES)
            or (lens is not None and (lens.dtype != torch.int32 or lens.numel() != B))):
        raise ValueError(f"fbank_db: shapes wav {tuple(wav.shape)}, window {tuple(window.shape)}, fbank "
                         f"{tuple(fbank.shape)}, db {tuple(db.shape)}, partial_max {tuple(partial_max.shape)}")
    _lib.check(lib().w2v2_fbank_db(wav.data_ptr(), _p(lens), window.data_ptr(), fbank.data_ptr(), db.data_ptr(),
                                   partial_max.data_ptr(), B, N, T, n_mels, stream()), "fbank_db")


def fbank_normalize(db, partial_max, lens, out, ldo: int) -> None:
    _dev(db, partial_max, lens, out)
    _fbank_f32(db, partial_max)
    B, T, n_mels = db.shape
    if (out.dtype not in (torch.float32, torch.bfloat16) or ldo < n_mels or out.stride(-1) != 1
            or partial_max.numel() < B * -(-T // FBANK_TILE_FRAMES)
            or out.untyped_storage().nbytes() // out.element_size() - out.storage_offset() < (B * T - 1) * ldo + n_mels
            or (lens is not None and (lens.dtype != torch.int32 or lens.numel() != B))):
        raise ValueError(f"fbank_normalize: db {tuple(db.shape)}, out {tuple(out.shape)} {out.dtype} with row stride {ldo}")
    _lib.check(lib().w2v2_fbank_normalize(db.data_ptr(), partial_max.data_ptr(), _p(lens), out.data_ptr(), ldo, dt(out),
                                          B, T, n_mels, stream()), "fbank_normalize")


def se_scale(x, g, y, B: int, T: int, C: int) -> None:
    _dev(x, g, y)
    _lib.check(lib().w2v2_se_scale(x.data_ptr(), g.data_ptr(), y.data_ptr(), B, T, C, dt(x), stream()), "se_scale")


def se_bwd_gate(dout, x, dg, B: int, T: int, C: int) -> None:
    _dev(dout, x, dg)
    _lib.check(lib().w2v2_se_bwd_gate(dout.data_ptr(), x.data_ptr(), dg.data_ptr(), B, T, C, dt(x), stream()),
               "se_bwd_gate")


def se_bwd_x(dout, g, ds, dx, B: int, T: int, C: int) -> None:
    _dev(dout, g, ds, dx)
    _lib.check(lib().w2v2_se_bwd_x(dout.data_ptr(), g.data_ptr(), ds.data_ptr(), dx.data_ptr(), B, T, C, dt(dout),
                                   stream()), "se_bwd_x")


ACT_NONE, ACT_RELU, ACT_SIGMOID = 0, 1, 2


def skinny_linear_fwd(x, W, bias, y, act: int) -> None:
    _dev(x, W, bias, y)
    assert x.dtype == W.dtype == y.dtype == torch.float32 and x.is_contiguous() and W.is_contiguous() and y.is_contiguous()
    B, K = x.shape
    N = W.shape[0]
    assert W.numel() == N * K and y.shape == (B, N)
    _lib.check(lib().w2v2_skinny_linear_fwd(x.data_ptr(), W.data_ptr(), _p(bias), y.data_ptr(), B, N, K, act, stream()),
               "skinny_linear_fwd")


def skinny_linear_bwd_x(dy, y, W, dx, act: int) -> None:
    _dev(dy, y, W, dx)
    B, N = dy.shape
    K = dx.shape[1]
    assert W.numel() == N * K and dx.shape == (B, K) and dx.is_contiguous() and dy.is_contiguous()
    _lib.check(lib().w2v2_skinny_linear_bwd_x(dy.data_ptr(), _p(y), W.data_ptr(), dx.data_ptr(), B, N, K, act, stream()),
               "skinny_linear_bwd_x")


def skinny_linear_bwd_w(dy, y, x, dW, dbias, act: int, accumulate: bool) -> None:
    _dev(dy, y, x, dW, dbias)
    B, N = dy.shape
    K = x.shape[1]
    assert dW.numel() == N * K and x.shape == (B, K) and x.is_contiguous() and dy.is_contiguous()
    _lib.check(lib().w2v2_skinny_linear_bwd_w(dy.data_ptr(), _p(y), x.data_ptr(), dW.data_ptr(), _p(dbias), B, N, K, act,
                                              int(accumulate), stream()), "skinny_linear_bwd_w")


def act_fwd(x, y, mode: int) -> None:
    _dev(x, y)
    _lib.check(lib().w2v2_act_fwd(x.data_ptr(), y.data_ptr(), x.numel(), mode, stream()), "act_fwd")


def act_bwd(dy, y, dx, mode: int) -> None:
    _dev(dy, y, dx)
    _lib.check(lib().w2v2_act_bwd(dy.data_ptr(), y.data_ptr(), dx.data_ptr(), dy.numel(), mode, stream()), "act_bwd")


def bce_head_fwd_bwd(emb, w, b, label, prob, loss_rows, dlogit, demb, dw, db, B: int, H: int, loss_scale=None) -> None:
    _dev(emb, w, b, label, prob, loss_rows, dlogit, demb, dw, db, loss_scale)
    _lib.check(lib().w2v2_bce_head_fwd_bwd(emb.data_ptr(), w.data_ptr(), b.data_ptr(), label.data_ptr(), prob.data_ptr(),
                                           loss_rows.data_ptr(), _p(dlogit), _p(demb), _p(dw), _p(db), B, H,
                                           _p(loss_scale), stream()), "bce_head")
```

Before: 6440 utterances/sec.

## Fuse AAM-softmax head into cosine, loss-mean, and batched dx kernels

Adds a fused path for the AAM-softmax head. One kernel computes row norms of weights and embeddings, casts the embedding to 16-bit, and produces the normalized cosine logits with MFMA. The softmax kernel now also reduces the mean loss through a last-block ticket, and the split dx GEMMs become one batched launch whose last entry takes a shorter K, followed by a fold kernel that produces demb. The goal is fewer small launches and host-side ops in a head that runs on only 66 rows. The cost is more custom code and atomic ticket logic in place of library GEMMs.

```diff
diff --git a/include/w2v2_hip.h b/include/w2v2_hip.h
--- a/include/w2v2_hip.h
+++ b/include/w2v2_hip.h
@@ -53,7 +53,7 @@
   float alpha;
   int32_t split_k;
   int32_t accumulate;
-  int32_t _pad;
+  int32_t k_last;
   int32_t k_ext, n_ext_from;
   int64_t b_lo_offset;
 } w2v2_gemm_desc;
@@ -263,6 +263,15 @@
                        void* stream);
 int w2v2_aam_dw(const void* dcos_x, int64_t ldc, const void* emb, const float* colprod, const float* W,
                 const float* inv_w, float* dW, int B, int C, int E, int dtype, void* stream);
+int w2v2_aam_cos(const float* W, const float* emb, float* logits, int64_t ldc, float* inv_x, float* inv_w,
+                 void* emb_lp, int B, int C, int E, int dtype, void* stream);
+int w2v2_aam_softmax_fwd_bwd_mean(const float* cos, const int64_t* label, float* softmax, float* loss_rows,
+                                  void* dcos_w, void* dcos_x, const float* inv_x, const float* inv_w,
+                                  float* rowdot, float* colprod, int B, int C, int64_t ldc, float margin,
+                                  float scale, const float* loss_scale, float* correct_rows, int easy_margin,
+                                  float* loss_mean, unsigned* ticket, int dtype, void* stream);
+int w2v2_aam_fold_demb(const float* parts, int nparts, const float* emb, const float* inv_x, const float* rowdot,
+                       float* demb, int B, int E, void* stream);
 
 int w2v2_adam_step(float* p, const float* g, float* m, float* v, void* pb, int pb_dtype, int64_t n, float lr,
                    float beta1, float beta2, float eps, float bias_corr1, float bias_corr2,
diff --git a/w2v2_speaker_amd/_lib.py b/w2v2_speaker_amd/_lib.py
--- a/w2v2_speaker_amd/_lib.py
+++ b/w2v2_speaker_amd/_lib.py
@@ -24,7 +24,7 @@
                 ("C", c_vp), ("ldc", c_i64), ("c_stride0", c_i64), ("c_stride1", c_i64),
                 ("aux", c_vp), ("ldaux", c_i64), ("aux_stride0", c_i64), ("aux_stride1", c_i64),
                 ("bias", c_vp), ("bias_stride1", c_i64), ("row_scale", c_vp), ("col_scale", c_vp),
-                ("alpha", c_f32), ("split_k", c_i32), ("accumulate", c_i32), ("_pad", c_i32),
+                ("alpha", c_f32), ("split_k", c_i32), ("accumulate", c_i32), ("k_last", c_i32),
                 ("k_ext", c_i32), ("n_ext_from", c_i32), ("b_lo_offset", c_i64)]
 
 
@@ -150,6 +150,10 @@
     "w2v2_aam_softmax_fwd_bwd": (c_i32, [c_vp, c_vp, c_vp, c_vp, c_vp, c_vp, c_vp, c_vp, c_vp, c_vp, c_i32,
                                          c_i32, c_i64, c_f32, c_f32, c_vp, c_vp, c_i32, c_i32, c_vp]),
     "w2v2_aam_dw": (c_i32, [c_vp, c_i64, c_vp, c_vp, c_vp, c_vp, c_vp, c_i32, c_i32, c_i32, c_i32, c_vp]),
+    "w2v2_aam_cos": (c_i32, [c_vp, c_vp, c_vp, c_i64, c_vp, c_vp, c_vp, c_i32, c_i32, c_i32, c_i32, c_vp]),
+    "w2v2_aam_softmax_fwd_bwd_mean": (c_i32, [c_vp, c_vp, c_vp, c_vp, c_vp, c_vp, c_vp, c_vp, c_vp, c_vp, c_i32,
+                                              c_i32, c_i64, c_f32, c_f32, c_vp, c_vp, c_i32, c_vp, c_vp, c_i32, c_vp]),
+    "w2v2_aam_fold_demb": (c_i32, [c_vp, c_i32, c_vp, c_vp, c_vp, c_vp, c_i32, c_i32, c_vp]),
     "w2v2_normalize_bwd": (c_i32, [c_vp, c_vp, c_i64, c_vp, c_vp, c_vp, c_i32, c_i32, c_i32, c_i32, c_vp]),
     "w2v2_adam_step": (c_i32, [c_vp, c_vp, c_vp, c_vp, c_vp, c_i32, c_i64, c_f32, c_f32, c_f32, c_f32, c_f32,
                                c_f32, c_f32, c_vp, c_i32, c_i32, c_vp]),
diff --git a/w2v2_speaker_amd/csrc/gemm.hip b/w2v2_speaker_amd/csrc/gemm.hip
--- a/w2v2_speaker_amd/csrc/gemm.hip
+++ b/w2v2_speaker_amd/csrc/gemm.hip
@@ -108,7 +108,8 @@
   const int z0 = z / g.batch_inner, z1 = z - z0 * g.batch_inner;
   const int split = blockIdx.y;
   const int kbeg = split * g.k_per_split;
-  const int kend = min(g.K, kbeg + g.k_per_split);
+  const int Kz = (g.k_last > 0 && z == (int)gridDim.z - 1) ? g.k_last : g.K;
+  const int kend = min(Kz, kbeg + g.k_per_split);
 
   const bf16_t* Ab = reinterpret_cast<const bf16_t*>(g.A.ptr) + z0 * g.a_s0 + z1 * g.a_s1;
   const bf16_t* Bb = reinterpret_cast<const bf16_t*>(g.B.ptr) + z0 * g.b_s0 + z1 * g.b_s1;
@@ -393,6 +394,7 @@
   a.late_dma = 0;
   a.xcd_tiles = 0;
   a.dbg_bits = 0;
+  a.k_last = d->k_last;
   const int cal = d->dtype_c == W2V2_F32 ? 4 : 8;
   a.c_vec_ok = aligned16(d->C) && (d->ldc % cal == 0) && (d->c_stride0 % cal == 0) && (d->c_stride1 % cal == 0);
   a.aux_vec_ok = d->aux && aligned16(d->aux) && (d->ldaux % cal == 0) && (d->aux_stride0 % cal == 0) &&
@@ -403,6 +405,7 @@
   a.k_per_split = (int)(cdiv(cdiv(d->K, split), bk) * bk);
   if (a.k_per_split == 0) a.k_per_split = bk;
   if (f32) {
+    W2V2_REQUIRE(d->k_last == 0, "w2v2_gemm: k_last is for 16-bit operands");
     r.f32_rows = w2v2_gemm_f32_dma_rows(a, d->M, d->N, d->K, split, d->batch);
     r.family = r.f32_rows > 0 ? 10 : 9;
     return 0;
@@ -439,6 +442,10 @@
                  "w2v2_gemm: two-term weights (k_ext) need k_ext == K, n_ext_from %% 128 == 0 and K-contiguous 16-byte "
                  "aligned operands with K %% 64 == 0 (M=%d N=%d K=%d)", d->M, d->N, d->K);
   r.family = phased ? 4 : ring ? 2 : glds ? 1 : 3;
+  if (d->k_last != 0)
+    W2V2_REQUIRE(r.family == 3 && d->k_last > 0 && d->k_last < d->K && d->batch > 1 && split == 1 && !atomic,
+                 "w2v2_gemm: a shorter last batch entry (k_last=%d, K=%d, batch=%d) runs on the register-staged kernel "
+                 "only, unsplit and written", d->k_last, d->K, d->batch);
   a.wt_stores = sw.wt_stores;
   a.late_dma = sw.late_dma;
   if (r.family == 2)
diff --git a/w2v2_speaker_amd/csrc/gemm_common.h b/w2v2_speaker_amd/csrc/gemm_common.h
--- a/w2v2_speaker_amd/csrc/gemm_common.h
+++ b/w2v2_speaker_amd/csrc/gemm_common.h
@@ -39,6 +39,7 @@
   int64_t b_lo_off;
   int xcd_tiles;
   int dbg_bits;
+  int k_last;
 };
 
 __device__ __forceinline__ int64_t outer_off(const OpDev& o, int64_t idx) {
diff --git a/w2v2_speaker_amd/csrc/heads.hip b/w2v2_speaker_amd/csrc/heads.hip
--- a/w2v2_speaker_amd/csrc/heads.hip
+++ b/w2v2_speaker_amd/csrc/heads.hip
@@ -84,7 +84,8 @@
                                                       const float* __restrict__ inv_w, float* __restrict__ rowdot,
                                                       float* __restrict__ colprod, int B, int C, int64_t ldc,
                                                       float margin, float scale, const float* __restrict__ loss_scale,
-                                                      float* __restrict__ correct_rows, int easy_margin) {
+                                                      float* __restrict__ correct_rows, int easy_margin,
+                                                      float* __restrict__ loss_mean, unsigned* __restrict__ ticket) {
   constexpr int NT = AAM_ROW_THREADS, NW = NT / 64;
   __shared__ float sh[NW], sh2[NW];
   __shared__ int shi[NW];
@@ -144,7 +145,11 @@
   }
   block_reduce_sum2<NW>(sum, sum_off, sh, sh2);
   const float inv = 1.0f / sum;
-  if (threadIdx.x == 0) loss_rows[b] = bad_label ? __builtin_nanf("") : (mx + __logf(sum)) - zy;
+  if (threadIdx.x == 0) {
+    const float lr = bad_label ? __builtin_nanf("") : (mx + __logf(sum)) - zy;
+    if (loss_mean != nullptr) __hip_atomic_store(loss_rows + b, lr, __ATOMIC_RELAXED, __HIP_MEMORY_SCOPE_AGENT);
+    else loss_rows[b] = lr;
+  }
   const float invB = bad_label ? 0.f : (loss_scale ? loss_scale[0] : 1.0f) / (float)B;
   float rd = 0.f;
   for (int c = threadIdx.x; c < C; c += NT) {
@@ -169,6 +174,43 @@
     rd = block_reduce_n<NW>(rd, sh, false);
     if (threadIdx.x == 0) rowdot[b] = rd;
   }
+  if (loss_mean != nullptr && threadIdx.x < 64) {
+    unsigned t = 0;
+    if (threadIdx.x == 0) {
+      asm volatile("s_waitcnt vmcnt(0)" ::: "memory");
+      t = __hip_atomic_fetch_add(ticket, 1u, __ATOMIC_RELAXED, __HIP_MEMORY_SCOPE_AGENT);
+    }
+    t = __shfl(t, 0, 64);
+    if (t == gridDim.x - 1) {
+      float r[4];
+#pragma unroll
+      for (int w = 0; w < 4; ++w) {
+        float s = 0.f;
+        for (int i = 64 * w + (int)threadIdx.x; i < B; i += 256)
+          s += __hip_atomic_load(loss_rows + i, __ATOMIC_RELAXED, __HIP_MEMORY_SCOPE_AGENT);
+        r[w] = wave_sum(s);
+      }
+      if (threadIdx.x == 0) {
+        loss_mean[0] = (r[0] + r[1] + r[2] + r[3]) / (float)B;
+        __hip_atomic_store(ticket, 0u, __ATOMIC_RELAXED, __HIP_MEMORY_SCOPE_AGENT);
+      }
+    }
+  }
+}
+
+extern "C" int w2v2_aam_softmax_fwd_bwd_mean(const float* cos, const int64_t* label, float* softmax, float* loss_rows,
+                                             void* dcos_w, void* dcos_x, const float* inv_x, const float* inv_w,
+                                             float* rowdot, float* colprod, int B, int C, int64_t ldc, float margin,
+                                             float scale, const float* loss_scale, float* correct_rows, int easy_margin,
+                                             float* loss_mean, unsigned* ticket, int dtype, void* stream) {
+  W2V2_REQUIRE(cos && label && softmax && loss_rows && B > 0 && C > 0 && ldc >= C, "aam_softmax: bad arguments");
+  W2V2_REQUIRE((loss_mean == nullptr) == (ticket == nullptr), "aam_softmax: the mean and its ticket counter come together");
+  W2V2_DISPATCH_ACT(dtype, "aam_softmax",
+    hipLaunchKernelGGL(aam_row_kernel<AT>, dim3(B), dim3(AAM_ROW_THREADS), 0, as_stream(stream), cos, label, softmax,
+                       loss_rows, (AT*)dcos_w, (AT*)dcos_x, inv_x, inv_w, rowdot, colprod, B, C, ldc, margin,
+                       scale, loss_scale, correct_rows, easy_margin, loss_mean, ticket););
+  W2V2_CHECK_LAUNCH("aam_softmax");
+  return 0;
 }
 
 extern "C" int w2v2_aam_softmax_fwd_bwd(const float* cos, const int64_t* label, float* softmax, float* loss_rows,
@@ -176,13 +218,9 @@
                                         float* rowdot, float* colprod, int B, int C, int64_t ldc, float margin,
                                         float scale, const float* loss_scale, float* correct_rows, int easy_margin,
                                         int dtype, void* stream) {
-  W2V2_REQUIRE(cos && label && softmax && loss_rows && B > 0 && C > 0 && ldc >= C, "aam_softmax: bad arguments");
-  W2V2_DISPATCH_ACT(dtype, "aam_softmax",
-    hipLaunchKernelGGL(aam_row_kernel<AT>, dim3(B), dim3(AAM_ROW_THREADS), 0, as_stream(stream), cos, label, softmax,
-                       loss_rows, (AT*)dcos_w, (AT*)dcos_x, inv_x, inv_w, rowdot, colprod, B, C, ldc, margin,
-                       scale, loss_scale, correct_rows, easy_margin););
-  W2V2_CHECK_LAUNCH("aam_softmax");
-  return 0;
+  return w2v2_aam_softmax_fwd_bwd_mean(cos, label, softmax, loss_rows, dcos_w, dcos_x, inv_x, inv_w, rowdot, colprod, B, C,
+                                       ldc, margin, scale, loss_scale, correct_rows, easy_margin, nullptr, nullptr, dtype,
+                                       stream);
 }
 
 template <typename TX>
@@ -207,6 +245,226 @@
     hipLaunchKernelGGL(normalize_bwd_kernel<AT>, dim3(nb), dim3(256), 0, as_stream(stream), g, (const AT*)x,
                        ldx, inv, dot, dx, rows, cols, add););
   W2V2_CHECK_LAUNCH("normalize_bwd");
+  return 0;
+}
+
+constexpr int ACOS_CT = 32, ACOS_KT = 256, ACOS_PITCH = ACOS_KT + 8;
+template <int MT2> constexpr size_t acos_lds_bytes() {
+  return (size_t)(ACOS_CT + 32 * MT2) * ACOS_PITCH * 2 + (size_t)(ACOS_CT + 32 * MT2) * sizeof(float);
+}
+template <typename T, int MT2>
+__global__ __launch_bounds__(512) void aam_cos_kernel(const float* __restrict__ W, const float* __restrict__ emb,
+                                                      float* __restrict__ logits, int64_t ldc, float* __restrict__ inv_x,
+                                                      float* __restrict__ inv_w, T* __restrict__ emb_lp, int B, int C,
+                                                      int E) {
+  constexpr int RPW = 4 * MT2;
+  constexpr int NI = (2 * MT2 + 3) / 4;
+  extern __shared__ __attribute__((aligned(16))) char acos_raw[];
+  T* Ws = reinterpret_cast<T*>(acos_raw);
+  T* Xs = Ws + ACOS_CT * ACOS_PITCH;
+  float* s_invw = reinterpret_cast<float*>(Xs + 32 * MT2 * ACOS_PITCH);
+  float* s_invx = s_invw + ACOS_CT;
+  const int tid = threadIdx.x, lane = tid & 63;
+  const int wave = __builtin_amdgcn_readfirstlane(tid >> 6);
+  const int c0 = blockIdx.x * ACOS_CT;
+  const int nv = E >> 2;
+  const bool first = blockIdx.x == 0;
+  const float4* W4 = reinterpret_cast<const float4*>(W);
+  const float4* X4 = reinterpret_cast<const float4*>(emb);
+
+  int64_t wrow[4];
+#pragma unroll
+  for (int j = 0; j < 4; ++j) wrow[j] = (int64_t)min(c0 + wave * 4 + j, C - 1) * nv;
+  float ssw[4][4], ssx[RPW][4];
+#pragma unroll
+  for (int j = 0; j < 4; ++j)
+#pragma unroll
+    for (int e = 0; e < 4; ++e) ssw[j][e] = 0.f;
+#pragma unroll
+  for (int j = 0; j < RPW; ++j)
+#pragma unroll
+    for (int e = 0; e < 4; ++e) ssx[j][e] = 0.f;
+  f32x4_hw acc[NI];
+#pragma unroll
+  for (int i = 0; i < NI; ++i) acc[i] = f32x4_hw{0.f, 0.f, 0.f, 0.f};
+
+  constexpr bool XPRE = MT2 < 4;
+  constexpr int XH = XPRE ? RPW : RPW / 2;
+  float4 wv[4], xv[XH];
+  auto load_w = [&](int t) {
+    const int c = lane + 64 * t;
+#pragma unroll
+    for (int j = 0; j < 4; ++j) wv[j] = c < nv ? W4[wrow[j] + c] : make_float4(0.f, 0.f, 0.f, 0.f);
+  };
+  auto load_x = [&](int t, int jb) {
+    const int c = lane + 64 * t;
+#pragma unroll
+    for (int j = 0; j < XH; ++j) {
+      const int r = wave + 8 * (jb + j);
+      xv[j] = (c < nv && r < B) ? X4[(int64_t)r * nv + c] : make_float4(0.f, 0.f, 0.f, 0.f);
+    }
+  };
+  auto conv_x = [&](int t, int jb) {
+    const int c = lane + 64 * t;
+#pragma unroll
+    for (int j = 0; j < XH; ++j) {
+      const int r = wave + 8 * (jb + j);
+      float* ss = ssx[jb + j];
+      ss[0] = fmaf(xv[j].x, xv[j].x, ss[0]); ss[1] = fmaf(xv[j].y, xv[j].y, ss[1]);
+      ss[2] = fmaf(xv[j].z, xv[j].z, ss[2]); ss[3] = fmaf(xv[j].w, xv[j].w, ss[3]);
+      const uint2 p = make_uint2(pack2<T>(xv[j].x, xv[j].y), pack2<T>(xv[j].z, xv[j].w));
+      *reinterpret_cast<uint2*>(Xs + r * ACOS_PITCH + 4 * lane) = p;
+      if (first && emb_lp != nullptr && c < nv && r < B) *reinterpret_cast<uint2*>(emb_lp + (int64_t)r * E + 4 * c) = p;
+    }
+  };
+  const int cw = wave & 1, mg = wave >> 1;
+  const int frow = lane & 15, fk = lane >> 4;
+  const int nt = (E + ACOS_KT - 1) / ACOS_KT;
+  load_w(0);
+  if constexpr (XPRE) load_x(0, 0);
+  for (int t = 0; t < nt; ++t) {
+#pragma unroll
+    for (int j = 0; j < 4; ++j) {
+      ssw[j][0] = fmaf(wv[j].x, wv[j].x, ssw[j][0]); ssw[j][1] = fmaf(wv[j].y, wv[j].y, ssw[j][1]);
+      ssw[j][2] = fmaf(wv[j].z, wv[j].z, ssw[j][2]); ssw[j][3] = fmaf(wv[j].w, wv[j].w, ssw[j][3]);
+      *reinterpret_cast<uint2*>(Ws + (wave * 4 + j) * ACOS_PITCH + 4 * lane) =
+          make_uint2(pack2<T>(wv[j].x, wv[j].y), pack2<T>(wv[j].z, wv[j].w));
+    }
+    if constexpr (XPRE) {
+      conv_x(t, 0);
+    } else {
+      load_x(t, 0);
+      conv_x(t, 0);
+      load_x(t, XH);
+      conv_x(t, XH);
+    }
+    if (t + 1 < nt) {
+      load_w(t + 1);
+      if constexpr (XPRE) load_x(t + 1, 0);
+    }
+    __syncthreads();
+    const int nstep = (min(ACOS_KT, E - t * ACOS_KT) + 31) >> 5;
+#pragma unroll
+    for (int s = 0; s < ACOS_KT / 32; ++s) {
+      if (s < nstep) {
+        const frag8_t wf = *reinterpret_cast<const frag8_t*>(Ws + (cw * 16 + frow) * ACOS_PITCH + (s * 4 + fk) * 8);
+#pragma unroll
+        for (int i = 0; i < NI; ++i) {
+          const int mt = mg + 4 * i;
+          if (mt * 16 < B) {
+            const frag8_t xf = *reinterpret_cast<const frag8_t*>(Xs + (mt * 16 + frow) * ACOS_PITCH + (s * 4 + fk) * 8);
+            acc[i] = mfma16<T>(wf, xf, acc[i]);
+          }
+        }
+      }
+    }
+    __syncthreads();
+  }
+#pragma unroll
+  for (int j = 0; j < 4; ++j) {
+    const float s = wave_sum((ssw[j][0] + ssw[j][1]) + (ssw[j][2] + ssw[j][3]));
+    const float iv = 1.0f / fmaxf(sqrtf(s), 1e-12f);
+    if (lane == 0) {
+      s_invw[wave * 4 + j] = iv;
+      if (c0 + wave * 4 + j < C) inv_w[c0 + wave * 4 + j] = iv;
+    }
+  }
+#pragma unroll
+  for (int j = 0; j < RPW; ++j) {
+    const int r = wave + 8 * j;
+    const float s = wave_sum((ssx[j][0] + ssx[j][1]) + (ssx[j][2] + ssx[j][3]));
+    const float iv = 1.0f / fmaxf(sqrtf(s), 1e-12f);
+    if (lane == 0) {
+      s_invx[r] = iv;
+      if (first && r < B) inv_x[r] = iv;
+    }
+  }
+  __syncthreads();
+#pragma unroll
+  for (int i = 0; i < NI; ++i) {
+    const int m = (mg + 4 * i) * 16 + frow;
+    if (m >= B) continue;
+    const int nl = cw * 16 + 4 * fk, n = c0 + nl;
+    const float rs = s_invx[m];
+    float o[4];
+#pragma unroll
+    for (int e = 0; e < 4; ++e) o[e] = acc[i][e] * (rs * s_invw[nl + e]);
+    float* crow = logits + (int64_t)m * ldc;
+    if (n + 4 <= C && (ldc & 3) == 0) {
+      *reinterpret_cast<float4*>(crow + n) = make_float4(o[0], o[1], o[2], o[3]);
+    } else {
+#pragma unroll
+      for (int e = 0; e < 4; ++e)
+        if (n + e < C) crow[n + e] = o[e];
+    }
+  }
+}
+
+extern "C" int w2v2_aam_cos(const float* W, const float* emb, float* logits, int64_t ldc, float* inv_x, float* inv_w,
+                            void* emb_lp, int B, int C, int E, int dtype, void* stream) {
+  W2V2_REQUIRE(W && emb && logits && inv_x && inv_w && B > 0 && C > 0 && E > 0 && ldc >= C, "aam_cos: bad arguments");
+  W2V2_REQUIRE(B <= 128 && E % 8 == 0, "aam_cos: B = %d, E = %d: at most 128 rows and E a multiple of 8 (else: the GEMM path)", B, E);
+  W2V2_REQUIRE(((uintptr_t)W | (uintptr_t)emb | (uintptr_t)logits | (uintptr_t)emb_lp) % 16 == 0,
+               "aam_cos: operands must be 16-byte aligned");
+  const dim3 grid((unsigned)cdiv(C, ACOS_CT));
+  hipStream_t st = as_stream(stream);
+  const int mt2 = (int)cdiv(B, 32);
+#define W2V2_ACOS(N)                                                                                                  \
+  case N:                                                                                                            \
+    if (w2v2_launch_lds<&aam_cos_kernel<AT, N>>("aam_cos_kernel", grid, dim3(512), acos_lds_bytes<N>(), st, W, emb, logits, \
+                                                 ldc, inv_x, inv_w, (AT*)emb_lp, B, C, E) != 0)                     \
+      return -1;                                                                                                     \
+    break;
+  W2V2_DISPATCH_16(dtype, "aam_cos", switch (mt2) { W2V2_ACOS(1) W2V2_ACOS(2) W2V2_ACOS(3) W2V2_ACOS(4) default: break; });
+#undef W2V2_ACOS
+  W2V2_CHECK_LAUNCH("aam_cos");
+  return 0;
+}
+
+__global__ __launch_bounds__(256) void aam_fold_demb_kernel(const float* __restrict__ parts, int nparts,
+                                                            const float* __restrict__ emb, const float* __restrict__ inv_x,
+                                                            const float* __restrict__ rowdot, float* __restrict__ demb,
+                                                            int B, int E) {
+  const int64_t n4 = (int64_t)B * E / 4;
+  const int64_t i4 = blockIdx.x * (int64_t)blockDim.x + threadIdx.x;
+  if (i4 >= n4) return;
+  const float4* p4 = reinterpret_cast<const float4*>(parts);
+  float a[4][4];
+#pragma unroll
+  for (int y = 0; y < 4; ++y)
+#pragma unroll
+    for (int e = 0; e < 4; ++e) a[y][e] = 0.f;
+#pragma unroll 2
+  for (int m = 0; m < nparts; m += 4) {
+    float4 v[4];
+#pragma unroll
+    for (int y = 0; y < 4; ++y) v[y] = (m + y < nparts) ? p4[(int64_t)(m + y) * n4 + i4] : make_float4(0.f, 0.f, 0.f, 0.f);
+#pragma unroll
+    for (int y = 0; y < 4; ++y)
+      if (m + y < nparts) { a[y][0] += v[y].x; a[y][1] += v[y].y; a[y][2] += v[y].z; a[y][3] += v[y].w; }
+  }
+  const int r = (int)(i4 * 4 / E);
+  const float iv = inv_x[r], dot = rowdot[r];
+  const float4 x = reinterpret_cast<const float4*>(emb)[i4];
+  const float xs[4] = {x.x, x.y, x.z, x.w};
+  float o[4];
+#pragma unroll
+  for (int e = 0; e < 4; ++e) {
+    const float g = 0.f + (a[0][e] + a[1][e] + a[2][e] + a[3][e]);
+    o[e] = iv * (g - xs[e] * iv * dot);
+  }
+  reinterpret_cast<float4*>(demb)[i4] = make_float4(o[0], o[1], o[2], o[3]);
+}
+
+extern "C" int w2v2_aam_fold_demb(const float* parts, int nparts, const float* emb, const float* inv_x,
+                                  const float* rowdot, float* demb, int B, int E, void* stream) {
+  W2V2_REQUIRE(parts && emb && inv_x && rowdot && demb && nparts > 0 && B > 0 && E > 0, "aam_fold_demb: bad arguments");
+  W2V2_REQUIRE(nparts <= 256 && E % 4 == 0 && ((uintptr_t)parts | (uintptr_t)emb | (uintptr_t)demb) % 16 == 0,
+               "aam_fold_demb: at most 256 partials, E a multiple of 4, 16-byte aligned operands");
+  const int64_t n4 = (int64_t)B * E / 4;
+  hipLaunchKernelGGL(aam_fold_demb_kernel, dim3((unsigned)cdiv(n4, 256)), dim3(256), 0, as_stream(stream), parts, nparts,
+                     emb, inv_x, rowdot, demb, B, E);
+  W2V2_CHECK_LAUNCH("aam_fold_demb");
   return 0;
 }
 
diff --git a/w2v2_speaker_amd/heads.py b/w2v2_speaker_amd/heads.py
--- a/w2v2_speaker_amd/heads.py
+++ b/w2v2_speaker_amd/heads.py
@@ -28,6 +28,9 @@
         self.loss_rows = torch.empty(B, dtype=f32, device=dev)
         self.correct = torch.zeros(B, dtype=f32, device=dev)
         aam = kind == "aam"
+        self.fused = (aam and ops.is16(act_dtype) and batch <= 128 and embed_dim % 8 == 0
+                      and w_master.data_ptr() % 16 == 0 and emb.data_ptr() % 16 == 0)
+        self._ticket = torch.zeros(1, dtype=torch.int32, device=dev) if self.fused else None
         if aam:
             self.inv_x, self.inv_w = torch.empty(B, dtype=f32, device=dev), torch.empty(Cn, dtype=f32, device=dev)
             self.g_fwd = Gemm(B, Cn, E, self.emb_lp, w_operand, self.logits, lda=E, ldb=E, ldc=self.ldc,
@@ -54,6 +57,9 @@
             if rest:
                 self.g_dx.append(Gemm(B, E, rest, self.dcos_w.view(-1)[S * Kc:], w_operand.view(-1)[S * Kc * E:],
                                       self.dx_parts[S], lda=self.ldc, ldb=E, ldc=E, transB=True))
+            self.g_dx1 = self.g_dx[0] if not rest else Gemm(
+                B, E, Kc, self.dcos_w, w_operand, self.dx_parts, lda=self.ldc, ldb=E, ldc=E, transB=True, batch=S + 1,
+                batch_inner=S + 1, a_strides=(0, Kc), b_strides=(0, Kc * E), c_strides=(0, B * E), k_last=rest)
             self.fused_dw = aam and E % 8 == 0
             if aam and not self.fused_dw:
                 self.H1 = torch.empty(Cn, E, dtype=f32, device=dev)
@@ -67,6 +73,8 @@
         B, E, Cn = self.B, self.E, self.C
         assert label.dtype == torch.int64 and label.is_cuda and label.shape == (B,)
         aam, tr = self.kind == "aam", self.train
+        if self.fused:
+            return self._forward_backward_fused(label)
         if self.emb_lp is not self.emb:
             ops.cast(self.emb, self.emb_lp)
         if aam:
@@ -100,6 +108,20 @@
                 self.demb.copy_(self.G1)
                 self.g_dw()
                 ops.colsum(self.dcos_w, self.bias_grad, B, Cn, self.ldc)
+        return loss, self.softmax[:, :Cn]
+
+    def _forward_backward_fused(self, label: torch.Tensor):
+        B, E, Cn, tr = self.B, self.E, self.C, self.train
+        ops.aam_cos(self.w_master, self.emb, self.logits, self.inv_x, self.inv_w, self.emb_lp, B, Cn, E, self.ldc)
+        loss = torch.empty((), dtype=torch.float32, device=self.loss_rows.device)
+        ops.aam_softmax_fwd_bwd_mean(self.logits, label, self.softmax, self.loss_rows, self.dcos_w if tr else None,
+                                     self.dcos_x if tr else None, self.inv_x, self.inv_w, self.rowdot if tr else None,
+                                     self.colprod if tr else None, B, Cn, self.ldc, self.margin, self.scale,
+                                     self.loss_scale if tr else None, self.correct, self.easy_margin, loss, self._ticket)
+        if tr:
+            self.g_dx1()
+            ops.aam_fold_demb(self.dx_parts, self.emb, self.inv_x, self.rowdot, self.demb, B, E)
+            ops.aam_dw(self.dcos_x, self.emb_lp, self.colprod, self.w_master, self.inv_w, self.w_grad, B, Cn, E, self.ldc)
         return loss, self.softmax[:, :Cn]
 
 
diff --git a/w2v2_speaker_amd/ops.py b/w2v2_speaker_amd/ops.py
--- a/w2v2_speaker_amd/ops.py
+++ b/w2v2_speaker_amd/ops.py
@@ -58,7 +58,7 @@
                  aux: Optional[torch.Tensor] = None, ldaux: int = 0, aux_strides: Tuple[int, int] = (0, 0),
                  row_scale: Optional[torch.Tensor] = None, col_scale: Optional[torch.Tensor] = None,
                  alpha: float = 1.0, split_k: int = 1, accumulate: bool = False,
-                 b_lo: Optional[torch.Tensor] = None, n_ext_from: int = 0):
+                 b_lo: Optional[torch.Tensor] = None, n_ext_from: int = 0, k_last: int = 0):
         _dev(A, B, Cmat, bias, aux, row_scale, col_scale, b_lo)
         if dt(A) != dt(B):
             raise TypeError("GEMM operands must share a dtype")
@@ -85,6 +85,7 @@
         d.row_scale, d.col_scale = _p(row_scale), _p(col_scale)
         d.alpha, d.split_k, d.accumulate = alpha, split_k, int(accumulate)
         d.k_ext, d.n_ext_from, d.b_lo_offset = 0, 0, 0
+        d.k_last = k_last
         if b_lo is not None:
             assert b_lo.dtype == B.dtype and (b_lo.data_ptr() - B.data_ptr()) % B.element_size() == 0
             d.k_ext, d.n_ext_from = K, n_ext_from
@@ -93,7 +94,7 @@
         self._ref = C.byref(d)
         self._keep = (A, B, Cmat, bias, aux, row_scale, col_scale, b_lo)
         self._fn = lib().w2v2_gemm
-        self.flops = 2.0 * M * N * K * batch
+        self.flops = 2.0 * M * N * (K * batch - ((K - k_last) if k_last else 0))
         esz = A.element_size()
         self.bytes = float(batch) * ((M * K + N * K) * esz + M * N * Cmat.element_size() * (2 if aux is not None else 1))
         lp = dt(A) != F32
@@ -634,6 +635,36 @@
                "aam_softmax")
 
 
+def aam_softmax_fwd_bwd_mean(cos, label, softmax, loss_rows, dcos_w, dcos_x, inv_x, inv_w, rowdot, colprod, B: int,
+                             Cn: int, ldc: int, margin: float, scale: float, loss_scale, correct_rows,
+                             easy_margin: bool, loss_mean, ticket) -> None:
+    _dev(cos, label, softmax, loss_rows, dcos_w, dcos_x, inv_x, inv_w, rowdot, colprod, loss_scale, correct_rows,
+         loss_mean, ticket)
+    assert loss_mean.dtype == torch.float32 and ticket.dtype == torch.int32 and ticket.numel() == 1
+    dty = dt(dcos_w) if dcos_w is not None else F32
+    _lib.check(lib().w2v2_aam_softmax_fwd_bwd_mean(cos.data_ptr(), label.data_ptr(), softmax.data_ptr(),
+                                                   loss_rows.data_ptr(), _p(dcos_w), _p(dcos_x), _p(inv_x), _p(inv_w),
+                                                   _p(rowdot), _p(colprod), B, Cn, ldc, margin, scale, _p(loss_scale),
+                                                   _p(correct_rows), int(easy_margin), loss_mean.data_ptr(),
+                                                   ticket.data_ptr(), dty, stream()),
+               "aam_softmax")
+
+
+def aam_cos(w_master, emb, logits, inv_x, inv_w, emb_lp, B: int, Cn: int, E: int, ldc: int, act_dtype=None) -> None:
+    _dev(w_master, emb, logits, inv_x, inv_w, emb_lp)
+    assert w_master.dtype == torch.float32 and emb.dtype == torch.float32 and logits.dtype == torch.float32
+    dty = dt(emb_lp) if emb_lp is not None else {torch.bfloat16: BF16, torch.float16: F16}[act_dtype]
+    _lib.check(lib().w2v2_aam_cos(w_master.data_ptr(), emb.data_ptr(), logits.data_ptr(), ldc, inv_x.data_ptr(),
+                                  inv_w.data_ptr(), _p(emb_lp), B, Cn, E, dty, stream()), "aam_cos")
+
+
+def aam_fold_demb(parts, emb, inv_x, rowdot, demb, B: int, E: int) -> None:
+    _dev(parts, emb, inv_x, rowdot, demb)
+    assert parts.dtype == torch.float32 and emb.dtype == torch.float32 and demb.dtype == torch.float32
+    _lib.check(lib().w2v2_aam_fold_demb(parts.data_ptr(), parts.shape[0], emb.data_ptr(), inv_x.data_ptr(),
+                                        rowdot.data_ptr(), demb.data_ptr(), B, E, stream()), "aam_fold_demb")
+
+
 def normalize_bwd(g, x, inv, dot, dx, rows: int, cols: int, ldx: Optional[int] = None, add_to: bool = False) -> None:
     _dev(g, x, inv, dot, dx)
     _lib.check(lib().w2v2_normalize_bwd(g.data_ptr(), x.data_ptr(), ldx if ldx is not None else cols, inv.data_ptr(),
```

After: 6437 utterances/sec. About the same (-0.0%).
